# usamec/GAML

Measured on AMD Instinct MI355X. Metric: reads_per_sec_scored, higher is better.
Workload: dtype f64; 1 GPU; cfg3: 5 Mbp, 50x 2x150 paired, insert 300+-30; 833333 pairs in all, whole true genome as 1-2 walks, 8 rotating path sets, window cache warm; pairs_total=833333, pairs_per_gpu=833333, genome_bp=5000000, parallelism=reads sharded over 1 GPU(s)

## Files before the change

gaml_amd/api.py:

```python
from __future__ import annotations

import ctypes as C
import importlib.util
import os
import sys

import numpy as np

_HERE = os.path.dirname(os.path.abspath(__file__))
FLAVOUR = os.environ.get("GAML_HIP_FLAVOUR", "release")
LIB_PATH = os.environ.get("GAML_HIP_LIB") or os.path.join(_HERE, "libgaml_hip_dev.so" if FLAVOUR == "dev" else "libgaml_hip.so")

OK, EINVAL, ENODEVICE, EHIP, ESTATE = 0, -1, -2, -3, -4

_i32p = np.ctypeslib.ndpointer(np.int32, flags="C_CONTIGUOUS")
_i64p = np.ctypeslib.ndpointer(np.int64, flags="C_CONTIGUOUS")
_f64p = np.ctypeslib.ndpointer(np.float64, flags="C_CONTIGUOUS")
_u8p = np.ctypeslib.ndpointer(np.uint8, flags="C_CONTIGUOUS")

ALIGMENT = np.dtype([("position", np.int32), ("edit_dist", np.int32), ("read_id", np.int32), ("orientation", np.int32)])
PACBIO_ALIGMENT = np.dtype([("position", np.int32), ("position_end", np.int32), ("read_id", np.int32), ("pad_", np.int32),
                            ("logprob", np.float64)])


# ... 90 lines not shown
    L.gaml_hip_set_presharded.argtypes = [vp, C.c_int32]
    L.gaml_hip_put_window_records.argtypes = [vp, C.c_int, C.c_int, _i32p, C.c_int32, vp, C.c_int64]
    L.gaml_hip_put_pacbio_records.argtypes = [vp, C.c_int, _i32p, C.c_int32, vp, C.c_int64]
    L.gaml_hip_add_pacbio_reads.argtypes = [vp, C.POINTER(SingleCfg), C.c_int32, _u8p, _i64p, C.c_char_p]
    L.gaml_hip_pacbio_missing.argtypes = [vp, C.c_int, _i32p, C.c_int32, _i32p, C.c_int32]
    L.gaml_hip_pacbio_missing.restype = C.c_int32
    L.gaml_hip_pacbio_ingest_sam.argtypes = [vp, C.c_int, _i32p, C.c_int32, C.c_char_p, C.c_int64, C.POINTER(C.c_int64)]
    L.gaml_hip_pacbio_records.argtypes = [vp, C.c_int, _i32p, C.c_int32, vp, C.c_int64]
    L.gaml_hip_pacbio_records.restype = C.c_int64
    L.gaml_hip_pacbio_dp_stats.argtypes = [vp, C.c_int, _f64p]
    if hasattr(L, "gaml_hip_debug_sam_logprob"):
        L.gaml_hip_debug_sam_logprob.argtypes = [vp, C.c_char_p, C.c_int32, C.c_char_p, C.c_int32, C.c_char_p, C.c_int64, C.c_double, C.POINTER(C.c_double), vp, vp, C.c_int32]
    if hasattr(L, "gaml_hip_debug_sam_shape"):
        L.gaml_hip_debug_sam_shape.argtypes = [C.c_char_p, C.c_int64, C.c_int32, _i32p, C.c_void_p, C.c_int32]
    if hasattr(L, "gaml_hip_debug_sam_band"):
        L.gaml_hip_debug_sam_band.argtypes = [C.c_char_p, C.c_int64, C.c_int32, _i32p, _i32p, _i32p, _i32p, C.c_int32]
        L.gaml_hip_debug_sam_band.restype = C.c_int32
    L.gaml_hip_calc_prob.argtypes = [vp, _i32p, _i64p, C.c_int32, C.POINTER(C.c_double), _i32p, C.POINTER(C.c_int32)]
    L.gaml_hip_calc_prob_batch.argtypes = [vp, C.c_int32, _i32p, _i64p, _i32p, _f64p, vp, vp]
    L.gaml_hip_calc_partials.argtypes = [vp, _i32p, _i64p, C.c_int32, _f64p, C.POINTER(C.c_int32)]
    L.gaml_hip_combine_partials.argtypes = [vp, _f64p, C.c_int32, C.POINTER(C.c_double), _i32p]
    L.gaml_hip_calc_partials_async.argtypes = [vp, _i32p, _i64p, C.c_int32, vp, vp, C.POINTER(C.c_int32)]
    L.gaml_hip_eval_begin.argtypes = [vp, _i32p, _i64p, C.c_int32, C.POINTER(C.c_int64), C.POINTER(C.c_int32)]
    L.gaml_hip_eval_pending_maxpos.argtypes = [vp, vp, C.c_int64]
    L.gaml_hip_eval_pending_maxpos.restype = C.c_int64
    L.gaml_hip_eval_apply_maxpos.argtypes = [vp, _i32p, C.c_int64]
    L.gaml_hip_eval_finish.argtypes = [vp, _f64p]
    L.gaml_hip_eval_finish_async.argtypes = [vp, vp, vp]
    L.gaml_hip_sync.argtypes = [vp]
    L.gaml_hip_compact_tables.argtypes = [vp]
    L.gaml_hip_eval_score_async.argtypes = [vp, vp, vp]
    L.gaml_hip_eval_score_async.restype = C.c_int32
    L.gaml_hip_eval_coverage_export_async.argtypes = [vp, C.c_int32, vp, C.c_int64, C.POINTER(C.c_int64), vp]
    L.gaml_hip_eval_coverage_finish_async.argtypes = [vp, C.c_int32, vp, C.c_int32, C.c_int32, vp]
    L.gaml_hip_eval_pacbio_pending.argtypes = [vp]
    L.gaml_hip_eval_pacbio_pending.restype = C.c_int32
    L.gaml_hip_eval_pacbio_intervals.argtypes = [vp, C.c_int32]
    L.gaml_hip_eval_pacbio_intervals.restype = C.c_int64
    L.gaml_hip_eval_pacbio_export_async.argtypes = [vp, C.c_int32, vp, C.c_int64, vp]
    L.gaml_hip_eval_pacbio_finish_async.argtypes = [vp, C.c_int32, vp, C.c_int64, C.c_int32, vp]
    L.gaml_hip_num_readsets.argtypes = [vp]
    L.gaml_hip_readset_kind.argtypes = [vp, C.c_int]
    L.gaml_hip_readset_reads.argtypes = [vp, C.c_int]
    L.gaml_hip_readset_reads.restype = C.c_int64
    L.gaml_hip_num_nodes.argtypes = [vp]
    L.gaml_hip_node_len.argtypes = [vp, C.c_int32]
    L.gaml_hip_read_probs.argtypes = [vp, C.c_int, _f64p, C.c_int64]
    L.gaml_hip_bad_bases.argtypes = [vp, C.c_int, C.POINTER(C.c_int64)]
    L.gaml_hip_window_count.argtypes = [vp, C.c_int, C.c_int]
    L.gaml_hip_window_count.restype = C.c_int64
    L.gaml_hip_window_records.argtypes = [vp, C.c_int, C.c_int, _i32p, C.c_int32, vp, C.c_int64]
    L.gaml_hip_window_records.restype = C.c_int64
    L.gaml_hip_align_window.argtypes = [vp, C.c_int, C.c_int, _i32p, C.c_int32]
    L.gaml_hip_align_window.restype = C.c_int64
    if hasattr(L, "gaml_hip_debug_prepare"):
        L.gaml_hip_debug_prepare.argtypes = [vp, _i32p, _i64p, C.c_int32]
    if hasattr(L, "gaml_hip_debug_occurrences"):
        L.gaml_hip_debug_occurrences.argtypes = [vp, C.c_int, C.c_int, _i32p, C.c_int64]
    if hasattr(L, "gaml_hip_debug_occurrences"):
        L.gaml_hip_debug_occurrences.restype = C.c_int64
    if hasattr(L, "gaml_hip_debug_table_occurrences"):
        L.gaml_hip_debug_table_occurrences.argtypes = [vp, C.c_int, C.c_int, _i32p, C.c_int64, _i64p]
    if hasattr(L, "gaml_hip_debug_table_occurrences"):
        L.gaml_hip_debug_table_occurrences.restype = C.c_int64
    if hasattr(L, "gaml_hip_debug_window_walk"):
        L.gaml_hip_debug_window_walk.argtypes = [vp, C.c_int, C.c_int, C.c_int32, _i32p, C.c_int32]
    for new, old in (("gaml_hip_pair_classes", "gaml_hip_debug_class_counts"), ("gaml_hip_last_phases", "gaml_hip_debug_profile"),
                     ("gaml_hip_table_stats", "gaml_hip_debug_table_stats")):
        if not hasattr(L, new) and hasattr(L, old):
            setattr(L, new, getattr(L, old))
    L.gaml_hip_pair_classes.argtypes = [vp, C.c_int, _i64p]
    if hasattr(L, "gaml_hip_debug_fold_check"):
        L.gaml_hip_debug_fold_check.argtypes = [vp, C.c_int, _i64p]
    if hasattr(L, "gaml_hip_debug_radix_sort"):
        L.gaml_hip_debug_radix_sort.argtypes = [vp, C.c_void_p, C.c_void_p, C.c_int64, C.c_int, C.c_int, C.c_void_p]
    if hasattr(L, "gaml_hip_debug_tables_check"):
        L.gaml_hip_debug_tables_check.argtypes = [vp, C.c_int, _i64p]
    if hasattr(L, "gaml_hip_debug_static_check"):
        L.gaml_hip_debug_static_check.argtypes = [vp, C.c_int, _i64p]
    if hasattr(L, "gaml_hip_debug_set_knob"):
        L.gaml_hip_debug_set_knob.argtypes = [vp, C.c_int, C.c_int]
    if hasattr(L, "gaml_hip_debug_occ_route"):
        L.gaml_hip_debug_occ_route.argtypes = [vp, C.c_int, _i64p]
    if hasattr(L, "gaml_hip_debug_occ_check"):
        L.gaml_hip_debug_occ_check.argtypes = [vp, C.c_int, _i64p]
    if hasattr(L, "gaml_hip_shm_exchange_open"):
        L.gaml_hip_shm_exchange_open.argtypes = [vp, C.c_char_p, C.c_int32, C.c_int32, C.c_int32]
        L.gaml_hip_shm_allreduce_sum.argtypes = [vp, C.c_void_p, C.c_int32]
        L.gaml_hip_shm_exchange_close.argtypes = [vp, C.c_int32]
    if hasattr(L, "gaml_hip_fetch_async"):
        L.gaml_hip_fetch_async.argtypes = [vp, C.c_void_p, C.c_int32, C.c_void_p]
        L.gaml_hip_fetch_wait.argtypes = [vp, C.c_void_p, C.c_int32]
    if hasattr(L, "gaml_hip_advice_build"):
        L.gaml_hip_advice_build.argtypes = [vp, C.c_int, C.c_int32]
        L.gaml_hip_advice_index.argtypes = [vp, C.c_int, C.c_void_p, C.c_void_p, C.c_int64]
        L.gaml_hip_advice_index.restype = C.c_int64
        L.gaml_hip_advice_candidates.argtypes = [vp, C.c_int, _i32p, C.c_int32, _i32p, C.c_int32, C.c_int32, C.c_void_p, C.c_int64]
        L.gaml_hip_advice_candidates.restype = C.c_int64
    if hasattr(L, "gaml_hip_debug_timeline"):
        L.gaml_hip_debug_timeline.argtypes = [vp, C.c_int, C.c_void_p, C.c_int64]
    L.gaml_hip_last_phases.argtypes = [vp, _f64p]
    L.gaml_hip_table_stats.argtypes = [vp, C.c_int, _i64p]
    L.gaml_hip_aligner_stats.argtypes = [vp, C.POINTER(C.c_int64), C.POINTER(C.c_int64), C.POINTER(C.c_double)]
    L.gaml_hip_aligner_stages.argtypes = [vp, _f64p]
    L.gaml_hip_last_timing.argtypes = [vp, _f64p]
    L.gaml_hip_set_event_timing.argtypes = [vp, C.c_int]
    L.gaml_hip_kernel_stats.argtypes = [vp, C.c_int, C.POINTER(C.c_int64), C.POINTER(C.c_double), C.POINTER(C.c_double)]
    return L


_lib = _load()

def lib():
    return _lib


def version() -> str:
    return _lib.gaml_hip_version().decode()


class FlatPaths:

    def __init__(self, paths):
        self.flat, self.offs = _flat(paths)
        self.n = len(paths)
        self.flat_ptr, self.offs_ptr = self.flat.ctypes.data, self.offs.ctypes.data

    def __len__(self):
        return self.n


def _flat(paths):
    if isinstance(paths, FlatPaths):
        return paths.flat, paths.offs
    flat = np.array([x for p in paths for x in p], dtype=np.int32)
    if flat.size == 0:
        flat = np.zeros(1, np.int32)
    offs = np.zeros(len(paths) + 1, dtype=np.int64)
    offs[1:] = np.cumsum([len(p) for p in paths])
    return flat, offs


def comm_unique_id() -> bytes:
    buf = C.create_string_buffer(128)
    rc = _lib.gaml_hip_comm_unique_id(C.cast(buf, C.c_void_p))
    if rc != OK:
        raise GamlHipError(rc, "gaml_hip_comm_unique_id failed (RCCL not loadable?)")
    return buf.raw


class Context:

    def __init__(self, device: int = 0, rank: int = 0, world: int = 1, presharded: int = 1, devices=None):
        self._h = C.c_void_p()
        if devices is not None:
            devs = np.ascontiguousarray(devices, np.int32)
            rc = _lib.gaml_hip_create_multi(C.byref(self._h), devs, len(devs))
            if rc != OK:
                raise GamlHipError(rc, f"gaml_hip_create_multi(devices={list(devs)}) failed")
            device = int(devs[0])
        else:
            rc = _lib.gaml_hip_create(C.byref(self._h), device)
            if rc != OK:
                raise GamlHipError(rc, f"gaml_hip_create(device={device}) failed")
        self.device = device
        if world != 1:
# ... 365 lines not shown
        if n > len(out):
            out = self._adv_buf = np.zeros(n, np.int32)
            n = self._check(_lib.gaml_hip_advice_candidates(self._h, rs, path, len(path), reach, len(reach), flags, out.ctypes.data, len(out)))
        return out[:n].copy()

    def debug_prepare(self, paths):
        flat, offs = _flat(paths)
        self._check(_lib.gaml_hip_debug_prepare(self._h, flat, offs, len(paths)))

    def debug_occurrences(self, rs, mate=0) -> np.ndarray:
        n = _lib.gaml_hip_debug_occurrences(self._h, rs, mate, np.zeros(5, np.int32), 0)
        out = np.zeros(5 * max(1, n), np.int32)
        _lib.gaml_hip_debug_occurrences(self._h, rs, mate, out, n)
        return out.reshape(-1, 5)[:n]

    def debug_table_occurrences(self, rs, mate=0):
        info = np.zeros(3, np.int64)
        n = _lib.gaml_hip_debug_table_occurrences(self._h, rs, mate, np.zeros(5, np.int32), 0, info)
        out = np.zeros(5 * max(1, n), np.int32)
        _lib.gaml_hip_debug_table_occurrences(self._h, rs, mate, out, n, info)
        return out.reshape(-1, 5)[:n], {"incremental": bool(info[0]), "incremental_calls": int(info[1]), "full_calls": int(info[2])}

    def debug_window_walk(self, rs, mate, wid) -> list:
        buf = np.zeros(64, np.int32)
        n = _lib.gaml_hip_debug_window_walk(self._h, rs, mate, wid, buf, 64)
        if n > 64:
            buf = np.zeros(n, np.int32)
            _lib.gaml_hip_debug_window_walk(self._h, rs, mate, wid, buf, n)
        return [int(x) for x in buf[:n]]

    def table_stats(self, rs):
        out = np.zeros(10, np.int64)
        self._check(_lib.gaml_hip_table_stats(self._h, rs, out))
        return {"full_rebuilds": int(out[0]), "delta_updates": int(out[1]), "dirty_pairs": int(out[2]), "worker_rebuilds": int(out[3]), "side_stream_rebuilds": int(out[3]),
                "batches_patched": int(out[4]), "batches_full": int(out[5]), "records_left_out": [int(out[6]), int(out[7])], "delta_records_left_out": int(out[8]),
                "static_index_pairs": int(out[9])}

    def aligner_stats(self):
        w, k, us = C.c_int64(), C.c_int64(), C.c_double()
        _lib.gaml_hip_aligner_stats(self._h, C.byref(w), C.byref(k), C.byref(us))
        return {"windows": w.value, "candidates": k.value, "us": us.value}

    def aligner_stages(self):
        out = np.zeros(6, np.float64)
        self._check(_lib.gaml_hip_aligner_stages(self._h, out))
        return {"strings_upload": out[0], "spans_candidates": out[1], "extension": out[2], "hits_d2h": out[3], "sort_file": out[4], "batches": int(out[5])}

    def last_phases(self):
        out = np.zeros(8, np.float64)
        _lib.gaml_hip_last_phases(self._h, out)
        return out

    def debug_timeline(self, rs: int, cap_waves: int = 1 << 16) -> np.ndarray:
        out = np.zeros((cap_waves, 8), np.uint64)
        n = self._check(_lib.gaml_hip_debug_timeline(self._h, rs, out.ctypes.data, cap_waves))
        return out[:n]

    def debug_set_knob(self, knob, value):
        self._check(_lib.gaml_hip_debug_set_knob(self._h, knob, value))

    def debug_fold_check(self, rs):
        out = np.zeros(6, np.int64)
        self._check(_lib.gaml_hip_debug_fold_check(self._h, rs, out))
        return {"records_left_out": [int(out[0]), int(out[1])], "compact_pairs": [int(out[2]), int(out[3])], "records_checked": int(out[4]),
                "violations": int(out[5])}

    def debug_radix_sort(self, keys, vals=None, begin_bit=0, end_bit=64, running_max=False):
        k = np.ascontiguousarray(keys, np.uint64).copy()
        v = None if vals is None else np.ascontiguousarray(vals, np.uint64).copy()
        m = np.zeros(len(k), np.uint64) if running_max else None
        self._check(_lib.gaml_hip_debug_radix_sort(self._h, k.ctypes.data, None if v is None else v.ctypes.data, len(k), begin_bit, end_bit,
                                                   None if m is None else m.ctypes.data))
        return k, v, m

    def debug_static_check(self, rs):
        out = np.zeros(8, np.int64)
        self._check(_lib.gaml_hip_debug_static_check(self._h, rs, out))
        return {"static_pairs": int(out[0]), "other_pairs": int(out[1]), "violations": int(out[2]), "no_record": int(out[3]),
                "different_windows": int(out[4]), "orientation": int(out[5]), "distance": int(out[6]), "edits_or_code": int(out[7])}

    def debug_occ_route(self, rs):
        out = np.zeros(6, np.int64)
        self._check(_lib.gaml_hip_debug_occ_route(self._h, rs, out))
        return {"device": int(out[0]), "host": int(out[1]), "fallbacks": int(out[2]), "compactions": int(out[3]),
                "pool_entries": int(out[4]), "shared_combinations": int(out[5])}

    def debug_occ_check(self, rs):
        out = np.zeros(4, np.int64)
        rc = _lib.gaml_hip_debug_occ_check(self._h, rs, out)
        res = {"compared": int(out[0]), "present": int(out[1]), "mismatches": int(out[2]), "lists": int(out[3])}
        if rc != 0 and res["compared"] == 0:
            self._check(rc)
        return res

    def debug_tables_check(self, rs):
        out = np.zeros(8, np.int64)
        rc = _lib.gaml_hip_debug_tables_check(self._h, rs, out)
        res = {"pairs": int(out[0]), "compact": int(out[1]), "static": int(out[2]), "two": int(out[3]), "four": int(out[4]), "more": int(out[5]),
               "compared": int(out[6]), "mismatches": int(out[7])}
        if rc != 0 and res["compared"] == 0:
            self._check(rc)
        return res

    def debug_block_partials(self, rs, set_index=0):
        sums, zeros, lay = np.zeros(8192, np.float64), np.zeros(8192, np.int32), np.zeros(8, np.int32)
        _lib.gaml_hip_debug_block_partials.argtypes = [C.c_void_p, C.c_int, C.c_int32, _f64p, _i32p, C.c_int32, _i32p]
        n = _lib.gaml_hip_debug_block_partials(self._h, rs, set_index, sums, zeros, 8192, lay)
        return sums[:max(n, 0)].copy(), zeros[:max(n, 0)].copy(), lay.tolist()

    def pair_classes(self, rs):
        out = np.zeros(4, np.int64)
        self._check(_lib.gaml_hip_pair_classes(self._h, rs, out))
        return out

    debug_table_stats, debug_profile, debug_class_counts = table_stats, last_phases, pair_classes

    def last_timing(self):
        out = np.zeros(3, np.float64)
        _lib.gaml_hip_last_timing(self._h, out)
        return {"host_us": out[0], "device_wall_us": out[1], "kernel_us": out[2]}

    def set_event_timing(self, on):
        _lib.gaml_hip_set_event_timing(self._h, int(on))

    def kernel_stats(self, reset=False):
        n, us, b = C.c_int64(), C.c_double(), C.c_double()
        _lib.gaml_hip_kernel_stats(self._h, 1 if reset else 0, C.byref(n), C.byref(us), C.byref(b))
        return {"launches": n.value, "device_us": us.value, "algo_bytes": b.value}


def debug_sam_band(sam_line: str, total_len: int):
    raw = sam_line.encode()
    f = np.zeros(10, np.int32); r0 = np.zeros(1, np.int32)
    n = _lib.gaml_hip_debug_sam_band(raw, len(raw), total_len, f, r0, np.zeros(1, np.int32), np.zeros(1, np.int32), 0)
    if n < 0:
        raise GamlHipError(n, "malformed SAM line")
    lo = np.zeros(n, np.int32); hi = np.zeros(n, np.int32)
    _lib.gaml_hip_debug_sam_band(raw, len(raw), total_len, f, r0, lo, hi, n)
    keys = ["flags", "len", "posstart", "posend", "sstart", "send", "slen", "tstart", "tend", "edit_dist"]
    return dict(zip(keys, (int(x) for x in f))), int(r0[0]), lo, hi


def debug_sam_shape(sam_line: str, total_len: int):
    raw = sam_line.encode()
    f = np.zeros(6, np.int32)
    n = _lib.gaml_hip_debug_sam_shape(raw, len(raw), total_len, f, None, 0)
    if n < 0:
        raise GamlHipError(n, "malformed SAM line")
    ops = np.zeros(max(1, n), np.uint32)
    _lib.gaml_hip_debug_sam_shape(raw, len(raw), total_len, f, ops.ctypes.data, n)
    keys = ["n_ops", "row_f", "col_f", "bl", "el", "max_width"]
    return dict(zip(keys, (int(x) for x in f))), [(int(o) >> 2, "MID"[int(o) & 3]) for o in ops[:n]]
```

gaml_amd/csrc/ctx.hip.h:

```cpp
#pragma once
#include <hip/hip_runtime.h>
#include <hip/hip_ext.h>
#include "radix_sort.hip.h"

#include <algorithm>
#include <atomic>
#include <fcntl.h>
#include <sys/mman.h>
#include <unistd.h>
#include <chrono>
#include <climits>
#include <limits>
#include <cmath>
#include <cstdio>
#include <cstdlib>
#include <cstring>
#include <immintrin.h>
#include <memory>
#include <set>
#include <string>
#include <thread>
#include <vector>

#include "aligner.hip.h"
// ... 200 lines not shown
  int64_t class_count[4] = {0, 0, 0, 0};
  int64_t n0a = 0;
  std::vector<uint32_t> len_combo;
  int64_t dropped_records[2] = {0, 0};
};

struct AdviceDev {
  bool built = false;
  int32_t threshold = 0;
  int64_t n_ent = 0, queries = 0;
  std::vector<int64_t> h_offs;
  std::vector<int32_t> h_ent;
  DevBuf offs, ent;
  DevBuf scratch;
  DevBuf first, last, cnt, at, tiles;
  DevBuf in, mask, out;
  PinBuf h_in, h_out;
  uint32_t serial = 0;
  std::vector<AdviceStep> steps;
  std::vector<int32_t> list;
  void release() {
    offs.release(); ent.release(); scratch.release(); first.release(); last.release(); cnt.release(); at.release(); tiles.release();
    in.release(); mask.release(); out.release(); h_in.release(); h_out.release();
  }
};

struct PairedSet {
  gaml_paired_cfg cfg;
  ShortMate mate[2];
  PairInfo pt;
  MateDev dev[2];
  TableDev tab;
  TableRebuild rebuild;
  BuildScratch scratch;
  BuildPlan build_plan;
  int64_t async_rebuilds = 0, retired_windows = 0, eval_count = 0;
  DevBuf lcode, len_combo_dev, combo_tabs, memo;
  int memo_codes = 0;
  bool statics_uploaded = false, kernels_warm = false, prereserved = false;
  DevBuf dl_slot, dl_spill, dl_rec[2], sp_rng[2], sp_rec[2], sp_slot, dstate;
  DevBuf dl_bins, dl_bin_count, dl_blk_tot, dl_wlist, dl_stamps;
  PinBuf h_dstate;
  size_t delta_cap = 0, cap_spill = 0, cap_sprec = 0;
  int64_t nd_est = 0, ns_est = 0;
  bool spill_may_grow = false;
  int dl_seq = 0;
  int64_t full_rebuilds = 0, delta_updates = 0;
  int quiet_calls = 0;
  int64_t delta_left_out = 0, delta_left_out_base = 0;
  bool compact_requested = false;
  PinBuf h_timeline; int timeline_waves = 0;
  PinBuf h_part_sum, h_part_zero;
  size_t host_part_stride = 0;
  int last_total_blocks = 0, last_sets = 1;
  int last_blocks[8] = {0, 0, 0, 0, 0, 0, 0, 0};
  bool last_host_partials = false;
  DevBuf probs, tabs, cov_bits, bad;
  Arena arena;
  struct Persist {
    void* dev = nullptr; size_t bytes = 0;
    size_t cap_w[2] = {0, 0}, cap_lo[2] = {0, 0}, cap_m[2] = {0, 0};
    size_t off_tfloor = 0, off_occ[2] = {0, 0}, off_lo[2] = {0, 0}, off_m[2] = {0, 0};
    bool valid = false;
    void release() { if (dev) (void)hipFree(dev); dev = nullptr; bytes = 0; valid = false; }
  } persist;
  struct OccDev {
    DevBuf pool[2];
    size_t pool_cap[2] = {0, 0}, pool_used[2] = {0, 0};
    uint32_t pool_gen = 1;
    PinBuf stage;
    DevBuf tab[2][2], list[2][2];
    DevBuf stamp[2];
    size_t cap_w = 0, cap_list = 0;
    int32_t list_n[2][2] = {{0, 0}, {0, 0}};
    uint32_t serial = 0;
    PinBuf dup;
    bool taken = false;
    bool check_dup = false;
    bool image_stale = false;
    std::vector<std::vector<uint64_t>> shared;
    size_t shared_next = 0;
    std::vector<uint64_t> key;
    int64_t dev_calls = 0, host_calls = 0, fallbacks = 0, compactions = 0;
    void release() {
      for (int mt = 0; mt < 2; mt++) {
        pool[mt].release(); stamp[mt].release();
        for (int k = 0; k < 2; k++) { tab[mt][k].release(); list[mt][k].release(); }
      }
      stage.release(); dup.release();
    }
  } occdev;
  int64_t batches_patched = 0, batches_full = 0;
  size_t batch_slack = 0;
  hipEvent_t ev_tables = nullptr, ev_ovf = nullptr;
  PairedPlanner planner;
  OccImage image[2];
  std::vector<Occ> scratch_occ[2];
  Reducer red;
  Staging stage_pool;
  std::vector<double> ins_tab, floor_tab, logfloor_tab, covthr_tab;
  bool floor_positive = true;
  bool tabs_uploaded = false;
  int64_t last_bad_bases = 0;
  AdviceDev adv;
};

struct SingleSet {
  gaml_single_cfg cfg;
  ShortMate mate;
  ReadMajor rm;
  MateDev dev;
  DevBuf lens, probs, tabs, occ_arena;
  std::vector<Occ> last_occ;
  Reducer red;
  std::vector<double> floor_tab, logfloor_tab;
  bool tabs_uploaded = false;
  Staging stage;
};

struct DpDev {
  DevBuf path, jobs, ops, scratch, out, dbg;
  void release() { path.release(); jobs.release(); ops.release(); scratch.release(); out.release(); dbg.release(); }
};

struct PbSweepDev {
  DevBuf iv_off, iv;
  std::vector<int32_t> iv_off_host;
  uint64_t generation = ~0ull;
  DevBuf in, all;
  DevBuf key_begin, key_end, pos, key_begin_s, key_end_s, pos_s, end_max, tmp, bad;
  Staging stage;
  void release() {
    iv_off.release(); iv.release(); in.release(); all.release(); key_begin.release(); key_end.release(); pos.release();
    key_begin_s.release(); key_end_s.release(); pos_s.release(); end_max.release(); tmp.release(); bad.release();
    for (int k = 0; k < kRing; k++) { stage.host[k].release(); if (stage.done[k]) (void)hipEventDestroy(stage.done[k]); stage.done[k] = nullptr; stage.armed[k] = false; }
  }
};

struct PacbioSet {
  gaml_single_cfg cfg;
  int64_t n_global = 0, lo = 0, hi = 0;
  std::vector<int32_t> lens;
  double log_match = 0, log_mismatch = 0;
  std::unordered_map<Walk, int32_t, WalkHasher> walk_id;
  std::vector<std::vector<gaml_pacbio_aligment>> recs;
  uint64_t generation = 0, uploaded_generation = ~0ull;
  int32_t max_len = 0;
  int64_t misses = 0;
  DevBuf d_lens, rec_off, rec_walk, rec_logp, walk_count, logprobs;
  Reducer red;
  int64_t last_bad_bases = 0;
  Staging stage;
  PbSweepDev sweep;
  bool have_reads = false;
  std::string bases;
  std::vector<int64_t> base_off;
  std::unordered_map<std::string, int32_t> name_id;
  DevBuf d_bases;
  DpDev dp;
  bool bases_uploaded = false;
  double dp_stats[8] = {0, 0, 0, 0, 0, 0, 0, 0};
};

struct PairedPrep {
  int64_t assembled_records = 0;
  std::vector<int32_t> path_base, start_off, starts;
  int32_t total_bits = 0, n_paths = 0;
  bool general = false;
};
// ... 76 lines not shown
```

gaml_amd/csrc/debug_api.hip.h:

```cpp
#pragma once

int gaml_hip_debug_prepare(gaml_hip_ctx* c, const int32_t* flat, const int64_t* offs, int32_t n_paths) {
  if (!c || n_paths < 0 || (n_paths > 0 && (!flat || !offs))) return fail(c, GAML_HIP_EINVAL, "bad arguments");
  if (c->multi) {
    for (int k = 0; k < gaml::multi_num_shards(c->multi); k++)
      if (int e = gaml_hip_debug_prepare(gaml::multi_shard(c->multi, k), flat, offs, n_paths)) return fail(c, e, gaml_hip_last_error(gaml::multi_shard(c->multi, k)));
    return GAML_HIP_OK;
  }
  if (!c->have_graph) return fail(c, GAML_HIP_ESTATE, "no graph set");
  std::vector<Walk> paths = unflatten(flat, offs, n_paths);
  for (auto& h : scoring_order(c)) {
    if (h.kind == 0) { std::vector<Occ> occs; prepare_single_host(c, *c->singles[h.idx], paths, occs); }
    else if (h.kind == 1) {
      PairedPrep p;
      PairedSet& ps = *c->paireds[h.idx];
      if (int e = prepare_paired_structure(c, ps, flat, offs, n_paths)) return e;
      if (int e = align_pending_pair(c, ps)) return e;
      if (int e = prepare_paired_tables_host(c, ps, p)) return e;
    }
  }
  if (c->peers == 1) {
    for (ShortMate* m : filter_mates(c)) m->unsynced.clear();
  }
  return GAML_HIP_OK;
// ... 205 lines not shown
  }
  return n;
}



int gaml_hip_debug_tables_check(gaml_hip_ctx* c, int rs, int64_t* out8) {
  MULTI_SHARD0(c);
  if (!c || rs < 0 || rs >= (int)c->handles.size() || c->handles[rs].kind != 1 || !out8) return fail(c, GAML_HIP_EINVAL, "bad arguments");
  if (c->device < 0) return fail(c, GAML_HIP_ENODEVICE, "host-only context");
  PairedSet& s = *c->paireds[c->handles[rs].idx];
  HIP_TRY(c, hipSetDevice(c->device));
  if (s.rebuild.active) { if (int e = paired_build_continue(c, s, true)) return e; HIP_TRY(c, hipEventSynchronize(s.rebuild.done)); s.rebuild.active = false; s.rebuild.after.clear(); }
  if (int e = prepare_paired_tables(c, s)) return e;
  if (int e = pool_mirror(c, s, c->stream)) return e;
  if (int e = paired_upload_statics(c, s, c->stream)) return e;
  TableDev T;
  if (int e = paired_build_enqueue(c, s, T, c->stream)) return e;
  HIP_TRY(c, hipStreamSynchronize(c->stream));
  if (int e = paired_build_collect(c, s, T)) { T.release(); return e; }
  ShortMate hm[2];
  for (int mt = 0; mt < 2; mt++) {
    const ShortMate& m = s.mate[mt];
    hm[mt].n_global = m.n_global; hm[mt].lo = m.lo; hm[mt].hi = m.hi; hm[mt].lens = m.lens;
    hm[mt].wins = m.wins;
    std::vector<int4> dp((size_t)s.dev[mt].pool_n);
    if (!dp.empty()) HIP_TRY(c, hipMemcpy(dp.data(), s.dev[mt].pool.p, dp.size() * sizeof(int4), hipMemcpyDeviceToHost));
    hm[mt].pool.resize(dp.size());
    for (size_t k = 0; k < dp.size(); k++) hm[mt].pool[k] = gaml_aligment{dp[k].y, dp[k].z & 0xff, dp[k].w, (dp[k].z >> 8) & 1};
    for (Window& w : hm[mt].wins) w.first = w.dfirst < 0 ? 0 : w.dfirst;
    for (Window& w : hm[mt].wins) if (w.dfirst < 0) { w.count = 0; }
  }
  PairTables pt;
  build_pair_tables(hm[0], hm[1], pt, KNOB(c, 16) != 1, paired_static_ins_n(c, s));
  const int64_t n = s.mate[0].n_local();
  int64_t compared = 0, bad = 0;
  auto fetch = [&](const DevBuf& d, size_t bytes, std::vector<char>& out) -> int {
    out.resize(bytes);
    if (bytes) HIP_TRY(c, hipMemcpy(out.data(), d.p, bytes, hipMemcpyDeviceToHost));
    return 0;
  };
  auto cmp = [&](const DevBuf& d, const void* host, size_t bytes, size_t elem, const char* what) -> int {
    std::vector<char> v;
    if (int e = fetch(d, bytes, v)) return e;
    int64_t b0 = bad;
    for (size_t k = 0; k < bytes / elem; k++) { compared++; if (memcmp(v.data() + k * elem, (const char*)host + k * elem, elem) != 0) bad++; }
    if (bad != b0 && getenv("GAML_HIP_TRACE_HOST")) fprintf(stderr, "tables_check: %s differs in %lld of %zu entries\n", what, (long long)(bad - b0), bytes / elem);
    return 0;
  };
  for (int k = 0; k < 4; k++) { compared++; bad += T.class_count[k] != pt.class_count[k]; }
  compared++; bad += T.n0a != pt.n0a;
  if (bad == 0) {
    const int64_t n0 = pt.class_count[0], n16 = n - n0;
    if (int e = cmp(T.slot_of_read, pt.slot_of_read.data(), (size_t)n * 4, 4, "slot_of_read")) return e;
    if (int e = cmp(T.read_of_slot, pt.read_of_slot.data(), (size_t)n * 4, 4, "read_of_slot")) return e;
    for (int mt = 0; mt < 2; mt++) {
      if (int e = cmp(T.rec8[mt], pt.rec8[mt].data(), (size_t)n0 * 8, 8, "rec8")) return e;
      if (int e = cmp(T.first[mt], pt.rm[mt].first.data(), (size_t)n16 * 16, 16, "first")) return e;
      if (int e = cmp(T.extra[mt], pt.rm[mt].extra.data(), pt.rm[mt].extra.size() * 16, 16, "extra")) return e;
      if (int e = cmp(T.inl[mt], pt.inl[mt].data(), pt.inl[mt].size() * 16, 16, "inl")) return e;
      compared++; bad += T.extras[mt] != (int64_t)pt.rm[mt].extra.size();
      compared++; bad += T.dropped[mt] != pt.dropped_records[mt];
    }
    if (int e = cmp(T.len_code, pt.len_code.data(), (size_t)n0, 1, "len_code")) return e;
    if (int e = cmp(T.static_idx, pt.static_idx.data(), (size_t)pt.n0a * 4, 4, "static_idx")) return e;
    if (int e = cmp(T.len12, pt.len12.data(), (size_t)n16 * 4, 4, "len12")) return e;
    compared++; bad += pt.len_combo != s.pt.len_combo;
  }
  out8[0] = n; out8[1] = T.class_count[0]; out8[2] = T.n0a; out8[3] = T.class_count[1]; out8[4] = T.class_count[2]; out8[5] = T.class_count[3];
  out8[6] = compared; out8[7] = bad;
  T.release();
  return bad ? fail(c, GAML_HIP_ESTATE, "record tables: the device build differs from the host restatement") : GAML_HIP_OK;
}

int gaml_hip_debug_occ_route(gaml_hip_ctx* c, int rs, int64_t* out6) {
  MULTI_SHARD0(c);
  if (!c || !out6 || rs < 0 || rs >= (int)c->handles.size() || c->handles[rs].kind != 1) return fail(c, GAML_HIP_EINVAL, "bad arguments");
  const PairedSet::OccDev& D = c->paireds[c->handles[rs].idx]->occdev;
  out6[0] = D.dev_calls; out6[1] = D.host_calls; out6[2] = D.fallbacks; out6[3] = D.compactions;
  out6[4] = (int64_t)(D.pool_used[0] + D.pool_used[1]); out6[5] = (int64_t)D.shared.size();
  return GAML_HIP_OK;
}

int gaml_hip_debug_occ_check(gaml_hip_ctx* c, int rs, int64_t* out4) {
  MULTI_SHARD0(c);
  if (!c || !out4 || rs < 0 || rs >= (int)c->handles.size() || c->handles[rs].kind != 1) return fail(c, GAML_HIP_EINVAL, "bad arguments");
  PairedSet& ps = *c->paireds[c->handles[rs].idx];
  const PairedSet::OccDev& D = ps.occdev;
  out4[0] = out4[1] = out4[2] = out4[3] = 0;
  if (!D.image_stale) return GAML_HIP_OK;
  HIP_TRY(c, hipSetDevice(c->device));
  HIP_TRY(c, hipStreamSynchronize(c->stream));
  const PlanView& v = ps.planner.view();
  for (int mt = 0; mt < 2; mt++) {
    OccImage im;
    im.build(ps.mate[mt].wins.size(), v, mt);
    const size_t n = im.occ12.size();
    std::vector<Occ12> dev(n);
    if (n) HIP_TRY(c, hipMemcpy(dev.data(), occdev_table(ps, mt), n * sizeof(Occ12), hipMemcpyDeviceToHost));
    for (size_t w = 0; w < n; w++) {
      const Occ12& h = im.occ12[w];
      const Occ12& d = dev[w];
      const bool absent = h.lo == ~0u && h.hi == ~0u;
      out4[0]++;
      if (!absent) out4[1]++;
      if (absent ? (d.lo != ~0u || d.hi != ~0u) : (d.lo != h.lo || d.hi != h.hi || d.rank != h.rank)) out4[2]++;
    }
    if (!im.general_wids.empty()) out4[3]++;
  }
  if (out4[2] || out4[3]) return fail(c, GAML_HIP_ESTATE, "device occurrence tables differ from the host image");
  return GAML_HIP_OK;
}
```

gaml_amd/csrc/host_model.cc:

```cpp
#include "host_model.h"

#include <algorithm>
#include <chrono>
#include <cmath>
#include <cstdlib>
#include <cstring>
#include <fstream>
#include <thread>

namespace gaml {

void GraphStore::finish() {
  norm.resize(n());
  std::unordered_map<std::string, int32_t> tiny;
  for (int32_t i = 0; i < n(); i++) {
    norm[i] = i;
    if (len(i) > 3) continue;
    std::string s(seq(i), len(i));
    auto it = tiny.find(s);
    if (it == tiny.end()) tiny.emplace(s, i);
    else norm[i] = it->second;
  }
}

// ... 865 lines not shown
    }
    is_new_.assign((size_t)n_paths, 0);
    for (const Edit& e : edits_) for (int32_t k = e.c0; k < e.c1; k++) is_new_[k] = 1;
    for (const Edit& e : edits_) {
      int32_t chain_end = e.c1;
      while (chain_end < n_paths) { const bool has_node = memos_[cur_ids_[chain_end]]->final_last_end != -2; chain_end++; if (has_node) break; }
      registration_chain(g, mate, e.c0, chain_end);
    }
    std::vector<char>& redo = redo_;
    redo.assign(memos_.size(), 0);
    for (int32_t id : in_ids) redo[id] = 1;
    for (int32_t id : stale_) if (id < (int32_t)memos_.size() && memos_[id]->use_count > 0 && (!memos_[id]->valid[0] || !memos_[id]->valid[1] || !memos_[id]->occ_valid[0] || !memos_[id]->occ_valid[1])) redo[id] = 2;
    stale_.clear();
    drain(mate);
    size_t seen = stale_.size();
    for (int32_t k = 0; k < n_paths; k++) {
      const int32_t id = cur_ids_[k];
      if (!redo[id]) continue;
      PathMemo& pm = *memos_[id];
      bool built = false;
      for (int mt = 0; mt < 2; mt++)
        if (!pm.valid[mt]) { build_placements(g, mate[mt], mt, pm, id); built = true; }
      if (!built) continue;
      drain(mate);
      for (; seen < stale_.size(); seen++) {
        const int32_t sid = stale_[seen];
        if (sid >= (int32_t)redo.size() || redo[sid]) continue;
        for (int32_t q = k + 1; q < n_paths; q++) if (cur_ids_[q] == sid) { redo[sid] = 2; break; }
      }
    }
    for (int32_t k = 0; k < n_paths; k++) {
      const int32_t id = cur_ids_[k];
      if (!redo[id]) continue;
      if (!is_new_[k]) {
        const PathMemo& pm = *memos_[id];
        removed_.push_back(Removed{cur_slots_[k], {pm.assembled[0], pm.assembled[1]}, {pm.occ[0], pm.occ[1]}});
      }
      work_.push_back(k);
    }
    std::vector<int32_t> keep;
    for (int32_t sid : stale_) if (sid < (int32_t)memos_.size() && memos_[sid]->use_count > 0 && (!memos_[sid]->valid[0] || !memos_[sid]->valid[1])) keep.push_back(sid);
    stale_.swap(keep);
  }
  const int64_t total = n_paths > 0 ? offs[n_paths] - base : 0;
  prev_flat_.assign(flat + base, flat + base + total);
  prev_offs_.resize((size_t)n_paths + 1);
  for (int32_t k = 0; k <= n_paths; k++) prev_offs_[k] = (n_paths > 0 ? offs[k] : 0) - base;
  have_prev_ = true;
  return true;
}

static void occ_prepack(const std::vector<Occ>& occ, std::vector<OccPre>& pre) {
  pre.resize(occ.size());
  for (size_t k = 0; k < occ.size(); k++) {
    const Occ& o = occ[k];
    const int32_t mp = o.min_pos < -32768 ? -32768 : o.min_pos;
    pre[k] = OccPre{o.min_pos <= 32767 ? o.wid : ~o.wid, (uint32_t)o.shift, (uint32_t)(uint16_t)(int16_t)mp, o.rank};
  }
}

static bool occ_pre_plain(const std::vector<OccPre>& pre) {
  std::vector<int32_t> w(pre.size());
  for (size_t k = 0; k < pre.size(); k++) { if (pre[k].wid < 0) return false; w[k] = pre[k].wid; }
  std::sort(w.begin(), w.end());
  return std::adjacent_find(w.begin(), w.end()) == w.end();
}

void PairedPlanner::invalidate_thresholds() {
  for (auto& pm : memos_) pm->occ_valid[0] = pm->occ_valid[1] = false;
  have_prev_ = false;
}

void PairedPlanner::finish(ShortMate mate[2]) {
  auto redo_occ = [&](PathMemo& pm) {
    for (int mt = 0; mt < 2; mt++) {
      if (pm.occ_valid[mt]) continue;
      pm.occ[mt].clear();
      occurrences_from_placements(mate[mt], pm.pl[mt], pm.occ[mt]);
      pm.assembled[mt] = 0;
      for (const Occ& o : pm.occ[mt]) pm.assembled[mt] += mate[mt].wins[o.wid].count;
      occ_prepack(pm.occ[mt], pm.pre[mt]);
      pm.pre_plain[mt] = occ_pre_plain(pm.pre[mt]);
      pm.dev_off[mt] = -1;
      pm.occ_valid[mt] = true;
    }
  };
  if (!incremental_) {
    for (int32_t id : cur_ids_) redo_occ(*memos_[id]);
    assembled_[0] = assembled_[1] = 0;
    for (int32_t id : cur_ids_) { assembled_[0] += memos_[id]->assembled[0]; assembled_[1] += memos_[id]->assembled[1]; }
  } else {
    for (int32_t k : work_) redo_occ(*memos_[cur_ids_[k]]);
  }
}

const PlanView& PairedPlanner::view() {
  if (!view_valid_) {
    view_.paths.clear();
    for (int32_t id : cur_ids_) view_.paths.push_back(memos_[id].get());
    view_valid_ = true;
  }
  return view_;
}

void PairedPlanner::apply(ShortMate mate[2], OccImage image[2], bool build_image, bool image_stale) {
  if (!incremental_) {
    const PlanView& v = view();
    for (int32_t id : cur_ids_) {
      PathMemo& pm = *memos_[id];
      if (pm.touched_serial == retire_serial_) continue;
      for (int mt = 0; mt < 2; mt++) for (const Occ& o : pm.occ[mt]) mate[mt].touch(o.wid);
      pm.touched_serial = retire_serial_;
    }
    if (build_image) for (int mt = 0; mt < 2; mt++) image[mt].build(mate[mt].wins.size(), v, mt);
    return;
  }
  if (image_stale) {
    for (int mt = 0; mt < 2; mt++) {
      for (const Removed& r : removed_) assembled_[mt] -= r.assembled[mt];
      for (int32_t k : work_) assembled_[mt] += memos_[cur_ids_[k]]->assembled[mt];
    }
    for (int32_t id : cur_ids_) {
      PathMemo& pm = *memos_[id];
      if (pm.touched_serial == retire_serial_) continue;
      for (int mt = 0; mt < 2; mt++) for (const Occ& o : pm.occ[mt]) mate[mt].touch(o.wid);
      pm.touched_serial = retire_serial_;
    }
    rebuild_images(mate, image);
    return;
  }
  for (int32_t k : work_) {
    PathMemo& pm = *memos_[cur_ids_[k]];
    if (pm.touched_serial == retire_serial_) continue;
    for (int mt = 0; mt < 2; mt++) for (const Occ& o : pm.occ[mt]) mate[mt].touch(o.wid);
    pm.touched_serial = retire_serial_;
  }
  if ((int32_t)pos_of_slot_.size() < next_slot_) pos_of_slot_.resize((size_t)next_slot_ + 64, 0);
  for (int32_t k = 0; k < (int32_t)cur_slots_.size(); k++) pos_of_slot_[cur_slots_[k]] = k;
  for (int mt = 0; mt < 2; mt++) {
    OccImage& im = image[mt];
    for (const Removed& r : removed_) { im.remove_path(r.occ[mt], r.slot); assembled_[mt] -= r.assembled[mt]; }
    for (int32_t k : work_) {
      const PathMemo& pm = *memos_[cur_ids_[k]];
      im.add_path(mate[mt].wins.size(), pm.occ[mt], cur_slots_[k]);
      assembled_[mt] += pm.assembled[mt];
    }
    im.finalize(pos_of_slot_);
  }
}

void PairedPlanner::rebuild_images(ShortMate mate[2], OccImage image[2]) {
  if ((int32_t)pos_of_slot_.size() < next_slot_) pos_of_slot_.resize((size_t)next_slot_ + 64, 0);
  for (int32_t k = 0; k < (int32_t)cur_slots_.size(); k++) pos_of_slot_[cur_slots_[k]] = k;
  const PlanView& v = view();
  for (int mt = 0; mt < 2; mt++) image[mt].build(mate[mt].wins.size(), v, mt, &cur_slots_, &pos_of_slot_);
}

void PairedPlanner::mark_used(ShortMate mate[2], const OccImage image[2]) {
  for (int mt = 0; mt < 2; mt++) image[mt].for_each_present([&](int32_t w) { mate[mt].touch(w); });
  for (auto& pm : memos_)
    if (pm->last_used > rebuild_clock_ || pm->use_count > 0)
      for (int mt = 0; mt < 2; mt++) for (const Occ& o : pm->occ[mt]) if (o.wid < (int32_t)mate[mt].wins.size()) mate[mt].touch(o.wid);
}

void PairedPlanner::flat_occurrences(int mate, std::vector<Occ>& out) {
  out.clear();
// ... 646 lines not shown
```

gaml_amd/csrc/host_model.h:

```cpp
#pragma once
#include <climits>
#include <cstdint>
#include <memory>
#include <string>
#include <unordered_map>
#include <vector>

#include "../../include/gaml_hip.h"

namespace gaml {

constexpr int kTail = 300;
constexpr int kSeed = 15;

struct GraphStore {
  std::string bases;
  std::vector<int64_t> off;
  std::vector<int32_t> norm;
  int32_t n() const { return (int32_t)off.size() - 1; }
  int32_t len(int32_t node) const { return (int32_t)(off[node + 1] - off[node]); }
  const char* seq(int32_t node) const { return bases.data() + off[node]; }
  void finish();
  bool load_lastgraph(const std::string& file, std::string* err);
};
// ... 127 lines not shown
#ifndef GAML_FOLD_CLASS2_BELOW
#define GAML_FOLD_CLASS2_BELOW 1024
#endif
constexpr int64_t kFoldClass2Below = GAML_FOLD_CLASS2_BELOW;
constexpr int kMemoCodes = 4;
constexpr int32_t kStaticZero = -2;
constexpr size_t kMemoMaxEntries = (size_t)1 << 24;
#ifdef GAML_HIP_DEV
struct PairTables {
  std::vector<int32_t> slot_of_read, read_of_slot;
  int64_t class_count[4] = {0, 0, 0, 0};
  int64_t n0a = 0;
  std::vector<int32_t> static_idx;
  std::vector<uint64_t> rec8[2];
  std::vector<uint8_t> len_code;
  std::vector<uint32_t> len_combo;
  std::vector<uint32_t> len12;
  ReadMajor rm[2];
  std::vector<RecQuad> inl[2];
  int64_t dropped_records[2] = {0, 0};
};
void build_pair_tables(const ShortMate& a, const ShortMate& b, PairTables& out, bool fold = true, int ins_n = 0);
#endif
void link_mate_windows(ShortMate& a, ShortMate& b);
#ifdef GAML_HIP_DEV
int64_t undominated_records(const ShortMate& m, int32_t wid, std::vector<uint8_t>& keep);
#endif


struct OccQuad { int32_t shift, min_pos, path, rank; };
struct OccTable {
  std::vector<OccQuad> direct;
  std::vector<int32_t> multi_off;
  std::vector<OccQuad> multi;
};
void build_occ_table(size_t n_windows, const std::vector<Occ>& occs, OccTable& out);

void split_contigs(const Walk& path, std::vector<std::pair<int32_t, int32_t>>& ctg_ranges, std::vector<int32_t>& gaps);

struct PlanView;
struct Occ12 { uint32_t lo, hi; int32_t rank; };
struct OccImage {
  std::vector<Occ12> occ12;
  std::vector<int32_t> multi_off;
  std::vector<OccQuad> multi;
  std::vector<int32_t> general_wids;
  void build(size_t n_windows, const PlanView& view, int mate, const std::vector<int32_t>* slots = nullptr,
             const std::vector<int32_t>* pos_of_slot = nullptr);
  void add_path(size_t n_windows, const std::vector<Occ>& occ, int32_t slot);
  void remove_path(const std::vector<Occ>& occ, int32_t slot);
  void finalize(const std::vector<int32_t>& pos_of_slot);
  std::vector<int32_t> changed;
  bool changed_all = true, lists_changed = true;
  void dump(std::vector<Occ>& out) const;
  template <class F> void for_each_present(F f) const { for (int32_t w : touched_) if (cnt_[w] > 0) f(w); }
  void take_changed() { changed.clear(); changed_all = false; lists_changed = false; if (++mark_serial_ == 0) { std::fill(mark_.begin(), mark_.end(), 0); mark_serial_ = 1; } }
 private:
  void grow(size_t n_windows);
  void mark(int32_t w) { if (mark_[w] != mark_serial_) { mark_[w] = mark_serial_; changed.push_back(w); } }
  void set_direct(int32_t w, const OccQuad& q);
  std::vector<int32_t> touched_, stale_, cnt_, list_of_;
  std::vector<uint32_t> stamp_, mark_;
  uint32_t serial_ = 0, mark_serial_ = 1;
  struct Pending { int32_t wid; OccQuad q; };
  std::vector<Pending> pending_;
  std::unordered_map<int32_t, std::vector<OccQuad>> gen_;
  bool lists_dirty_ = false;
};

struct OccPre { int32_t wid; uint32_t lo, hi; int32_t rank; };

struct PathMemo {
  Walk path;
  bool registered[2] = {false, false};
  bool first_pending[2] = {false, false};
  bool valid[2] = {false, false};
  bool occ_valid[2] = {false, false};
  std::vector<Placement> pl[2];
  std::vector<Occ> occ[2];
  std::vector<OccPre> pre[2];
  bool pre_plain[2] = {false, false};
  int64_t dev_off[2] = {-1, -1};
  uint32_t dev_gen[2] = {0, 0};
  int64_t assembled[2] = {0, 0};
  std::vector<int32_t> starts;
  int32_t length = 0;
  int32_t first_idx = -1, first_end = -1;
  int32_t final_last_end = -2;
  int32_t use_count = 0;
  uint32_t touched_serial = 0;
  uint64_t last_used = 0;
  uint32_t serial = 0;
};

struct PlanView {
  std::vector<const PathMemo*> paths;
};

class PairedPlanner {
 public:
  bool begin(const GraphStore& g, ShortMate mate[2], const int32_t* flat, const int64_t* offs, int32_t n_paths,
             bool allow_incremental, std::string* err);
  void finish(ShortMate mate[2]);
  void apply(ShortMate mate[2], OccImage image[2], bool build_image = true, bool image_stale = false);
  void rebuild_images(ShortMate mate[2], OccImage image[2]);
  const std::vector<int32_t>& ids() const { return cur_ids_; }
  PathMemo& memo(int32_t id) { return *memos_[id]; }
  void mark_used(ShortMate mate[2], const OccImage image[2]);
  void note_rebuild(bool retired_some) { rebuild_clock_ = clock_; if (retired_some) retire_serial_++; }
  void invalidate_thresholds();
  void forget_previous() { have_prev_ = false; }
  const PlanView& view();
  void flat_occurrences(int mate, std::vector<Occ>& out);
  size_t memo_count() const { return memos_.size(); }
  int32_t total_len() const { return total_len_; }
  int64_t assembled(int mate) const { return assembled_[mate]; }
  int32_t n_paths() const { return (int32_t)cur_ids_.size(); }
  bool last_was_incremental() const { return incremental_; }
  const std::vector<int32_t>& slots() const { return cur_slots_; }
  uint64_t hits = 0, misses = 0, incremental_calls = 0, full_calls = 0;
 private:
  int32_t lookup_or_create(const GraphStore& g, const int32_t* p, int32_t len, std::string* err);
  void drain(ShortMate mate[2]);
  void build_placements(const GraphStore& g, ShortMate& m, int mt, PathMemo& pm, int32_t id);
  void registration_chain(const GraphStore& g, ShortMate mate[2], int32_t from, int32_t to);
  std::vector<std::unique_ptr<PathMemo>> memos_;
  std::unordered_map<Walk, int32_t, WalkHasher> by_path_;
  std::unordered_map<Walk, std::vector<std::pair<int32_t, uint32_t>>, WalkHasher> missed_[2];
  PlanView view_;
  bool view_valid_ = false;
  std::vector<int32_t> cur_ids_;
  std::vector<int32_t> cur_slots_;
  std::vector<int32_t> free_slots_, pos_of_slot_;
  int32_t next_slot_ = 0;
  std::vector<int32_t> prev_flat_;
  std::vector<int64_t> prev_offs_;
  bool have_prev_ = false;
  bool incremental_ = false;
  struct Removed { int32_t slot; int64_t assembled[2]; std::vector<Occ> occ[2]; };
  std::vector<Removed> removed_;
  std::vector<int32_t> work_;
  std::vector<int32_t> stale_;
  std::vector<char> redo_;
  struct Edit { int32_t p0, p1, c0, c1; };
  std::vector<Edit> edits_;
  std::vector<char> is_new_;
  int32_t total_len_ = 0;
  int64_t assembled_[2] = {0, 0};
  uint64_t clock_ = 0, rebuild_clock_ = 0;
  uint32_t retire_serial_ = 0;
  static constexpr size_t kMaxMemos = 2048;
};
int32_t walk_length(const GraphStore& g, const Walk& w);

bool read_fastq(const std::string& file, std::string& bases, std::vector<int64_t>& offs, std::string* err,
                std::vector<std::string>* names = nullptr);

struct SamRecord {
  std::string name;
  int32_t flags = 0, len = 0, posstart = 0, posend = 0, sstart = 0, send = 0, slen = 0, tstart = 0, tend = 0, edit_dist = 0;
  std::vector<std::pair<int32_t, char>> cigar;
};
bool parse_sam_record(const char* begin, const char* end, int32_t total_len, SamRecord& out);

struct DpBand {
  int32_t row0 = 0, max_width = 0;
// ... 11 lines not shown
```

gaml_amd/csrc/kernels.hip.h:

```cpp
#pragma once
#include <hip/hip_runtime.h>
#include <stdint.h>

namespace gaml {

constexpr int kBlock = 256;
constexpr int kMaxBlocks = 2048;
enum { kDsDirty = 0, kDsSpill = 1, kDsTop0 = 2, kDsTop1 = 3, kDsOverflow = 4, kDsSeq = 5, kDsInts = 8 };

__device__ __forceinline__ unsigned long long occ8_of(const Occ12* t, unsigned w) { const Occ12* e = t + w; return (unsigned long long)e->lo | ((unsigned long long)e->hi << 32); }

struct MateView {
  const int4* first;
  const int4* extra;
  const int4* occ;
  const Occ12* occ12;
  const int* multi_off;
  const int4* multi;
  const double* mism_pow;
  const double* match_pow;
};

struct PairedArgs {
  int total_blocks, blocks0a, n0a, n_codes;
  int blocks0;
  int blocks01, blocks012;
  int main_blocks;
  const double2* memo;
  uint32_t* cov_bits;
  const unsigned long long* rec8[2];
  const double2* static_val;
  const Occ12* occ12[2];
  double* probs;
  double* part_sum;
  int* part_zero;
  double log_two_T;
  double tfloor0, logfloor0;
  uint32_t len_combo0; int pad0_;
  MateView m[2];
  const uint32_t* len12;
  const double* ins_tab;
  int ins_n;
  const double* floor_tab;
  const double* logfloor_tab;
  const double* covthr_tab;
  double two_T;
  int n;
  const int* path_base;
  const unsigned char* len_code;
  const uint32_t* len_combo;
  const double* pe[2];
  const double* floor_c;
  const double* logfloor_c;
  const double* covthr_c;
  int lt_codes;
  const double* tfloor_c;
  const int4* inl[2];
  int n0;
  const int* static_idx;
  int n01;
  int n_main;
  unsigned long long* timeline;
  const int* dstate;
  const int* dirty_slots;
  const int4* dirty_recs[2];
  const int* dirty_spill;
  const int2* spill_rng[2];
  const int4* spill_recs[2];
  const int* spill_slot;
  unsigned* ticket;
  double* out;
  double n_reads;
  double* status_out;
  double status_a, status_b;
};

struct Cand { int path, pos, edit, orient, rank, k; bool valid; };

__device__ __forceinline__ int4 occ_from_compact(unsigned long long o, int rk) {
  const int4 e = make_int4((int)(unsigned)o, (int)(short)(o >> 32), (int)((o >> 48) & 0x7fff), rk);
  return o == ~0ull ? make_int4(0, 0, -1, 0) : e;
}
__device__ __forceinline__ int4 mate_occ(const MateView& v, int w) {
  if (v.occ) return v.occ[w];
  const Occ12 e = v.occ12[w];
  return occ_from_compact((unsigned long long)e.lo | ((unsigned long long)e.hi << 32), e.rank);
}

__device__ __forceinline__ Cand make_cand(const int4& r, const int4& o, int k) {
  Cand c;
  c.path = o.z; c.pos = r.y + o.x; c.edit = r.z & 0xff; c.orient = (r.z >> 8) & 1;
  c.rank = o.w; c.k = k; c.valid = r.y >= o.y;
  return c;
}

struct TableSrc {
  const MateView* v;
  int4 r0;
  __device__ __forceinline__ int count() const { return r0.x < 0 ? 0 : 1 + (int)((unsigned)r0.z >> 9); }
  __device__ __forceinline__ int4 get(int k) const { return k == 0 ? r0 : v->extra[r0.w + k - 1]; }
};
struct ListSrc {
  const int4* recs;
  int cnt;
  __device__ __forceinline__ int count() const { return cnt; }
  __device__ __forceinline__ int4 get(int k) const { return recs[k]; }
};

template <class Src, class F>
__device__ __forceinline__ void for_each_cand_src(const MateView& v, const Src& src, F f) {
  const int cnt = src.count();
  for (int k = 0; k < cnt; k++) {
    int4 r = src.get(k);
    if (r.x < 0) continue;
    int4 o = mate_occ(v, r.x);
    if (o.z < 0) continue;
    if (o.w >= 0) {
      f(make_cand(r, o, k));
    } else {
      const int s = -o.w - 1;
      for (int q = v.multi_off[s]; q < v.multi_off[s + 1]; q++) f(make_cand(r, v.multi[q], k));
    }
  }
}
template <class F>
__device__ __forceinline__ void for_each_cand(const MateView& v, const int4& r0, F f) {
  for_each_cand_src(v, TableSrc{&v, r0}, f);
}

template <class Src>
__device__ __forceinline__ bool is_live_src(const MateView& v, const Src& src, const Cand& c) {
  if (!c.valid) return false;
  bool live = true;
  for_each_cand_src(v, src, [&](const Cand& d) {
    if (d.valid && d.path == c.path && d.pos == c.pos && (d.rank > c.rank || (d.rank == c.rank && d.k > c.k))) live = false;
  });
  return live;
}
__device__ __forceinline__ bool is_live(const MateView& v, const int4& r0, const Cand& c) {
  return is_live_src(v, TableSrc{&v, r0}, c);
}

__device__ __forceinline__ void mark_bit(uint32_t* bits, int bit) {
  atomicOr(&bits[bit >> 5], 1u << (bit & 31));
}

__device__ __forceinline__ double pair_term(const PairedArgs& a, const Cand& x, const Cand& y, int L1, int L2) {
  if (x.orient == y.orient) return 0.0;
  int dist;
  if (x.pos < y.pos) {
    if (x.orient != 0 || y.orient != 1) return 0.0;
    dist = y.pos - x.pos + L2;
  } else {
    if (x.orient != 1 || y.orient != 0) return 0.0;
    dist = x.pos - y.pos + L1;
  }
  if ((unsigned)dist >= (unsigned)a.ins_n) return 0.0;
  double p1 = a.m[0].mism_pow[x.edit] * a.m[0].match_pow[L1 - x.edit];
  double p2 = a.m[1].mism_pow[y.edit] * a.m[1].match_pow[L2 - y.edit];
  double ip = a.ins_tab[dist];
  double t = p1 * p2 * ip;
  if (a.cov_bits && t > a.covthr_tab[L2]) {
    int base = a.path_base[x.path];
    mark_bit(a.cov_bits, base + max(x.pos, y.pos));
    mark_bit(a.cov_bits, base + min(x.pos, y.pos));
  }
  return t;
}

template <class Src>
__device__ __forceinline__ double paired_general_src_slow(const PairedArgs& a, const Src& s1, const Src& s2, int L1, int L2) {
  double acc = 0.0;
  for_each_cand_src(a.m[0], s1, [&](const Cand& x) {
    if (!is_live_src(a.m[0], s1, x)) return;
    for_each_cand_src(a.m[1], s2, [&](const Cand& y) {
      if (y.path != x.path) return;
      if (!is_live_src(a.m[1], s2, y)) return;
      acc += pair_term(a, x, y, L1, L2);
    });
  });
  return acc;
}
template <class Src>
__device__ __forceinline__ bool live_mask_src(const MateView& v, const Src& src, unsigned long long& mask) {
  mask = 0;
  int n = 0;
  for_each_cand_src(v, src, [&](const Cand& c) {
    if (n < 64 && is_live_src(v, src, c)) mask |= 1ull << n;
    n++;
  });
  return n <= 64;
}
template <class Src>
__device__ __forceinline__ double paired_general_src_masks(const PairedArgs& a, const Src& s1, const Src& s2, int L1, int L2) {
  unsigned long long live1, live2;
  if (!live_mask_src(a.m[0], s1, live1) || !live_mask_src(a.m[1], s2, live2)) return paired_general_src_slow(a, s1, s2, L1, L2);
  double acc = 0.0;
  if (!live1 || !live2) return acc;
  int ix = 0;
  for_each_cand_src(a.m[0], s1, [&](const Cand& x) {
    const bool lx = (live1 >> ix) & 1ull;
    ix++;
    if (!lx) return;
    int iy = 0;
    for_each_cand_src(a.m[1], s2, [&](const Cand& y) {
      const bool ly = (live2 >> iy) & 1ull;
      iy++;
      if (!ly || y.path != x.path) return;
      acc += pair_term(a, x, y, L1, L2);
    });
  });
  return acc;
}
template <class Src>
__device__ __forceinline__ double paired_general_src(const PairedArgs& a, const Src& s1, const Src& s2, int L1, int L2) {
  return paired_general_src_slow(a, s1, s2, L1, L2);
}
__device__ __forceinline__ double paired_general(const PairedArgs& a, const int4& r1, const int4& r2, int L1, int L2) {
  return paired_general_src_masks(a, TableSrc{&a.m[0], r1}, TableSrc{&a.m[1], r2}, L1, L2);
}

__device__ __forceinline__ void block_reduce(double& s, int& z, double* sh_s, int* sh_z) {
  for (int off = 32; off > 0; off >>= 1) {
    s += __shfl_down(s, off, 64);
    z += __shfl_down(z, off, 64);
  }
  const int lane = threadIdx.x & 63, wave = threadIdx.x >> 6;
  if (lane == 0) { sh_s[wave] = s; sh_z[wave] = z; }
  __syncthreads();
  if (threadIdx.x == 0) {
    double ts = 0; int tz = 0;
    for (int w = 0; w < kBlock / 64; w++) { ts += sh_s[w]; tz += sh_z[w]; }
    s = ts; z = tz;
  }
}

constexpr int kTicketWords = 17;
__device__ __forceinline__ void grid_finish(double s, int z, int my_slot, int n_partials, double* part_sum, int* part_zero,
                                            unsigned* ticket, double* out, double bad_bases, double n_reads, double* sh_s, int* sh_z,
                                            double* status_out = nullptr, double status_a = 0.0, double status_b = 0.0) {
  __shared__ bool is_last;
  if (threadIdx.x == 0) {
    __hip_atomic_store(&part_sum[my_slot], s, __ATOMIC_RELAXED, __HIP_MEMORY_SCOPE_AGENT);
    __hip_atomic_store(&part_zero[my_slot], z, __ATOMIC_RELAXED, __HIP_MEMORY_SCOPE_AGENT);
    asm volatile("s_waitcnt vmcnt(0)" ::: "memory");
    const int g = my_slot & 15;
    const unsigned in_group = (unsigned)((n_partials - g + 15) >> 4), groups = (unsigned)min(16, n_partials);
    bool last = false;
    if (__hip_atomic_fetch_add(&ticket[1 + g], 1u, __ATOMIC_RELAXED, __HIP_MEMORY_SCOPE_AGENT) == in_group - 1)
      last = __hip_atomic_fetch_add(&ticket[0], 1u, __ATOMIC_RELAXED, __HIP_MEMORY_SCOPE_AGENT) == groups - 1;
    is_last = last;
  }
  __syncthreads();
  if (!is_last) return;
  double ts = 0; int tz = 0;
  for (int b = threadIdx.x; b < n_partials; b += kBlock) {
    ts += __hip_atomic_load(&part_sum[b], __ATOMIC_RELAXED, __HIP_MEMORY_SCOPE_AGENT);
    tz += __hip_atomic_load(&part_zero[b], __ATOMIC_RELAXED, __HIP_MEMORY_SCOPE_AGENT);
  }
  __syncthreads();
  block_reduce(ts, tz, sh_s, sh_z);
  if (threadIdx.x < kTicketWords) __hip_atomic_store(&ticket[threadIdx.x], 0u, __ATOMIC_RELAXED, __HIP_MEMORY_SCOPE_AGENT);
  if (threadIdx.x == 0) {
    out[0] = ts;
    out[1] = (double)tz;
    if (bad_bases >= 0) out[2] = bad_bases;
    out[3] = n_reads;
    if (status_out) { status_out[0] = status_a; status_out[1] = status_b; }
  }
}

struct PairVal { double t, logt; int key, kind; };

__device__ __forceinline__ void finish_read(const PairedArgs& a, int i, double acc, int L1, int L2, double& lsum, int& zeros, PairVal* cap = nullptr) {
  if (cap) *cap = PairVal{acc, 0.0, L1 + L2, 3};
  a.probs[i] = acc;
  const double p = acc / a.two_T;
  const int s = L1 + L2;
  if (p < a.floor_tab[s]) { zeros++; lsum += a.logfloor_tab[s]; }
  else lsum += log(p);
}

template <int K>
struct RegCands {
  int path[K], pos[K], ef[K], rank[K];
  bool valid[K], live[K];
};

template <int K>
__device__ __forceinline__ bool cands_from_records(const MateView& v, const int4 (&r)[K], RegCands<K>& c) {
  int4 o[K];
  bool multi = false;
  Occ12 e[K];
#pragma unroll
  for (int k = 0; k < K; k++) e[k] = v.occ12[r[k].x >= 0 ? r[k].x : 0];
#pragma unroll
  for (int k = 0; k < K; k++) o[k] = occ_from_compact((unsigned long long)e[k].lo | ((unsigned long long)e[k].hi << 32), e[k].rank);
#pragma unroll
  for (int k = 0; k < K; k++) if (r[k].x < 0) o[k] = make_int4(0, 0, -1, 0);
#pragma unroll
  for (int k = 0; k < K; k++) {
    multi |= (o[k].z >= 0 && o[k].w < 0);
    c.path[k] = o[k].z; c.pos[k] = r[k].y + o[k].x; c.ef[k] = r[k].z & 0x1ff; c.rank[k] = o[k].w;
    c.valid[k] = r[k].x >= 0 && o[k].z >= 0 && r[k].y >= o[k].y;
  }
#pragma unroll
  for (int i = 0; i < K; i++) {
    bool lv = c.valid[i];
#pragma unroll
    for (int j = 0; j < K; j++)
      if (j != i) lv = lv && !(c.valid[j] && c.path[j] == c.path[i] && c.pos[j] == c.pos[i] &&
                               (c.rank[j] > c.rank[i] || (c.rank[j] == c.rank[i] && j > i)));
    c.live[i] = lv;
  }
  return multi;
}
template <int K>
__device__ __forceinline__ bool load_cands_inline(const MateView& v, const int4* rec, RegCands<K>& c) {
  int4 r[K];
#pragma unroll
  for (int k = 0; k < K; k++) r[k] = rec[k];
  return cands_from_records<K>(v, r, c);
}

template <int K>
__device__ __forceinline__ double score_regs(const PairedArgs& a, const RegCands<K>& c1, const RegCands<K>& c2, int L1, int L2) {
  int n1 = 0, n2 = 0;
  Cand x, y;
  x.path = -1; x.pos = 0; x.edit = 0; x.orient = 0; y = x;
#pragma unroll
  for (int i = 0; i < K; i++) {
    if (c1.live[i]) { n1++; x.path = c1.path[i]; x.pos = c1.pos[i]; x.edit = c1.ef[i] & 0xff; x.orient = c1.ef[i] >> 8; }
    if (c2.live[i]) { n2++; y.path = c2.path[i]; y.pos = c2.pos[i]; y.edit = c2.ef[i] & 0xff; y.orient = c2.ef[i] >> 8; }
  }
  if (n1 == 0 || n2 == 0) return 0.0;
  if (n1 == 1 && n2 == 1) return x.path == y.path ? pair_term(a, x, y, L1, L2) : 0.0;
  double acc = 0.0;
#pragma unroll
  for (int i = 0; i < K; i++) {
#pragma unroll
    for (int j = 0; j < K; j++) {
      if (c1.live[i] && c2.live[j] && c1.path[i] == c2.path[j]) {
        Cand x, y;
        x.path = c1.path[i]; x.pos = c1.pos[i]; x.edit = c1.ef[i] & 0xff; x.orient = c1.ef[i] >> 8;
        y.path = c2.path[j]; y.pos = c2.pos[j]; y.edit = c2.ef[j] & 0xff; y.orient = c2.ef[j] >> 8;
        acc += pair_term(a, x, y, L1, L2);
      }
    }
  }
  return acc;
}

constexpr unsigned long long kNone8 = ~0ull;
constexpr unsigned long long kDirty8 = ~0ull - 1;
constexpr int kDirtyWid = -2;

__device__ __forceinline__ int4 rec8_to_quad(unsigned long long r) {
  if (r == kNone8 || r == kDirty8) return make_int4(r == kDirty8 ? kDirtyWid : -1, 0, 0, 0);
  return make_int4((int)(r & 0xffffff), (int)((r >> 24) & 0xfffffff), (int)((r >> 52) & 63) | ((int)((r >> 58) & 1) << 8), 0);
}

struct Compact1 {
  unsigned long long r1, r2, o1, o2;
  int L1, L2, lc;
};

__global__ __launch_bounds__(kBlock) void logterm_kernel(const double* pe0, const double* pe1, const double* ins_tab, int ins_n, int codes,
                                                        double2* memo) {
  const int total = codes * 49 * ins_n;
  for (int idx = blockIdx.x * kBlock + threadIdx.x; idx < total; idx += gridDim.x * kBlock) {
    const int dist = idx % ins_n;
    const int q = idx / ins_n;
    const int e2 = q % 7, e1 = (q / 7) % 7, code = q / 49;
    const double t = pe0[code * 64 + e1] * pe1[code * 64 + e2] * ins_tab[dist];
    memo[idx] = make_double2(t, log(t));
  }
}

// ... 82 lines not shown
      for (int q = 0; q < K; q++) {
        const Cand y = make_cand(r2, e2[q], 0);
        if (q >= l2.n || !y.valid || y.path != x.path) continue;
        acc += pair_term(a, x, y, L1, L2);
      }
    }
  } else {
    for (int p = 0; p < l1.n; p++) {
      const Cand x = make_cand(r1, l1.e[p], 0);
      if (!x.valid) continue;
      for (int q = 0; q < l2.n; q++) {
        const Cand y = make_cand(r2, l2.e[q], 0);
        if (!y.valid || y.path != x.path) continue;
        acc += pair_term(a, x, y, L1, L2);
      }
    }
  }
  finish_read_compact(a, i, acc, lc, lsum, zeros);
}

struct GenOut { double add; int zeros; };
__device__ GenOut compact_general_call(unsigned long long kernargs, int i, int set);
__device__ GenOut general_pair_call(unsigned long long kernargs, int i, int dj, int set, int4* lds);
__device__ __forceinline__ unsigned long long kernel_args_address() {
#if defined(__HIP_DEVICE_COMPILE__)
  return (unsigned long long)__builtin_amdgcn_kernarg_segment_ptr();
#else
  return 0;
#endif
}

__device__ __forceinline__ void compact_finish(const PairedArgs& a, int i, const Compact1& c, const CompactPrep& q, double2 m,
                                               double& lsum, int& zeros, PairVal* cap = nullptr) {
  if (q.memo_idx >= 0) {
    const double t = m.x;
    if (cap) *cap = PairVal{t, m.y, c.lc, 1};
    compact_cover(a, c, q, t);
    __builtin_nontemporal_store(t, &a.probs[i]);
    const bool floored = t < a.tfloor_c[c.lc];
    lsum += floored ? a.logfloor_c[c.lc] : m.y - a.log_two_T;
    zeros += (int)floored;
    return;
  }
  double t = 0.0;
  if (q.scores) { t = compact_term_tables(a, c, q); compact_cover(a, c, q, t); }
  finish_read_compact(a, i, t, c.lc, lsum, zeros, cap);
}

__device__ __forceinline__ void finish_val(const PairedArgs& a, int i, const PairVal& v, bool store, double& lsum, int& zeros) {
  if (v.kind == 0) return;
  if (store) __builtin_nontemporal_store(v.t, &a.probs[i]);
  if (v.kind == 1) {
    const bool floored = v.t < a.tfloor_c[v.key];
    lsum += floored ? a.logfloor_c[v.key] : v.logt - a.log_two_T;
    zeros += (int)floored;
  } else if (v.kind == 2) {
    if (v.t == 0.0 && a.floor_c[v.key] > 0.0) { zeros++; lsum += a.logfloor_c[v.key]; return; }
    const double p = v.t / a.two_T;
    if (p < a.floor_c[v.key]) { zeros++; lsum += a.logfloor_c[v.key]; }
    else lsum += log(p);
  } else {
    const double p = v.t / a.two_T;
    if (p < a.floor_tab[v.key]) { zeros++; lsum += a.logfloor_tab[v.key]; }
    else lsum += log(p);
  }
}

__device__ __forceinline__ void compact_load(const PairedArgs& a, int i, bool ok, Compact1& c) {
  c.r1 = ok ? a.rec8[0][i] : kNone8;
  c.r2 = ok ? a.rec8[1][i] : kNone8;
  c.lc = ok ? a.len_code[i] : 0;
}

#if defined(GAML_HIP_DEV) && defined(GAML_GEN_X)
#define GAML_GEN_OFF(bit) ((GAML_GEN_X) & (bit))
#else
#define GAML_GEN_OFF(bit) 0
#endif
struct SlotRange { int lo, hi, lb, blocks; };
__device__ __forceinline__ SlotRange compact_range(const PairedArgs& a, int lb) {
  return lb < a.blocks0a ? SlotRange{0, a.n0a, lb, a.blocks0a} : SlotRange{a.n0a, a.n0, lb - a.blocks0a, a.blocks0 - a.blocks0a};
}

template <bool GEN>
__device__ __forceinline__ void paired_compact_body(const PairedArgs& a, const SlotRange rg, double& lsum, int& zeros) {
  const int stride = rg.blocks * kBlock, hi = rg.hi;
  int i0 = rg.lo + rg.lb * kBlock + threadIdx.x;
  if (i0 >= hi) return;
  Compact1 c0, c1;
  compact_load(a, i0, true, c0);
  compact_load(a, i0 + stride, i0 + stride < hi, c1);
  while (true) {
    const int i1 = i0 + stride;
    const bool two = i1 < hi;
    const int j0 = i0 + 2 * stride;
    const bool more = j0 < hi;
    Compact1 n0v, n1v;
    compact_load(a, j0, more, n0v);
    compact_load(a, j0 + stride, j0 + stride < hi, n1v);
    const uint32_t l0 = a.len_combo[c0.lc], l1 = a.len_combo[c1.lc];
    c0.L1 = l0 & 0xffff; c0.L2 = l0 >> 16; c1.L1 = l1 & 0xffff; c1.L2 = l1 >> 16;
    const bool d0 = c0.r1 == kDirty8, d1 = c1.r1 == kDirty8;
    if (d0) { c0.r1 = kNone8; c0.r2 = kNone8; }
    if (d1) { c1.r1 = kNone8; c1.r2 = kNone8; }
    c0.o1 = c0.r1 != kNone8 ? occ8_of(a.occ12[0], (unsigned)(c0.r1 & 0xffffff)) : kNone8;
    c0.o2 = c0.r2 != kNone8 ? occ8_of(a.occ12[1], (unsigned)(c0.r2 & 0xffffff)) : kNone8;
    c1.o1 = c1.r1 != kNone8 ? occ8_of(a.occ12[0], (unsigned)(c1.r1 & 0xffffff)) : kNone8;
    c1.o2 = c1.r2 != kNone8 ? occ8_of(a.occ12[1], (unsigned)(c1.r2 & 0xffffff)) : kNone8;
    CompactPrep q0, q1;
    compact_prep(a, c0, q0);
    compact_prep(a, c1, q1);
    const double2 m0 = q0.memo_idx >= 0 ? a.memo[q0.memo_idx] : make_double2(0.0, 0.0);
    const double2 m1 = q1.memo_idx >= 0 ? a.memo[q1.memo_idx] : make_double2(0.0, 0.0);
    if (!d0 && !q0.skip) compact_finish(a, i0, c0, q0, m0, lsum, zeros);
    else if (GEN && q0.skip) { const GenOut o = compact_general_call(kernel_args_address(), i0, -1); lsum += o.add; zeros += o.zeros; }
    if (two && !d1 && !q1.skip) compact_finish(a, i1, c1, q1, m1, lsum, zeros);
    else if (GEN && two && q1.skip) { const GenOut o = compact_general_call(kernel_args_address(), i1, -1); lsum += o.add; zeros += o.zeros; }
    if (!more) break;
    c0 = n0v; c1 = n1v;
    i0 = j0;
  }
}

constexpr int kPairZero = -1, kPairOther = -(1 << 20);
__device__ __forceinline__ int compact_state(const PairedArgs& a, uint2 r1, uint2 r2, uint2 o1, uint2 o2, unsigned lc, uint32_t l12,
                                             bool in_range, bool& skip) {
  const bool v1 = r1.y != ~0u, v2 = r2.y != ~0u;
  const bool w1 = v1 & (o1.y != ~0u), w2 = v2 & (o2.y != ~0u);
  const bool here = in_range & !(r1.y == ~0u && r1.x == 0xfffffffeu);
  skip = here & ((w1 & ((int)o1.y < 0)) | (w2 & ((int)o2.y < 0)));
  const int L1 = l12 & 0xffff, L2 = l12 >> 16;
  const int p1 = (int)(__funnelshift_r(r1.x, r1.y, 24) & 0xfffffffu), p2 = (int)(__funnelshift_r(r2.x, r2.y, 24) & 0xfffffffu);
  const int x = p1 + (int)o1.x, y = p2 + (int)o2.x;
  const unsigned or1 = (r1.y >> 26) & 1u, or2 = (r2.y >> 26) & 1u;
  const bool fwd = x < y;
  const int dist = fwd ? y - x + L2 : x - y + L1;
  const bool scores = w1 & w2 & !skip & (((o1.y ^ o2.y) >> 16) == 0)
                      & (p1 >= (int)(short)(o1.y & 0xffffu)) & (p2 >= (int)(short)(o2.y & 0xffffu))
                      & (or1 != or2) & (or1 == (fwd ? 0u : 1u));
  const unsigned e1 = (r1.y >> 20) & 63u, e2 = (r2.y >> 20) & 63u;
  const bool in_memo = scores & ((unsigned)dist < (unsigned)a.ins_n) & (lc < (unsigned)a.lt_codes) & (e1 < 7u) & (e2 < 7u);
  const int idx = (int)((lc * 7u + e1) * 7u + e2) * a.ins_n + dist;
  int state = in_memo ? idx : ((skip | scores) ? kPairOther : kPairZero - (int)lc);
  if (!here) state = kPairOther - 1;
  return state;
}

template <bool GEN, bool TL = false, bool ONE = false>
__device__ __forceinline__ void paired_compact4_body(const PairedArgs& a, const SlotRange rg, double& lsum, int& zeros) {
  const unsigned stride = (unsigned)rg.blocks * kBlock, n0 = (unsigned)rg.hi;
  unsigned long long* tl = TL ? a.timeline + ((size_t)blockIdx.x * (kBlock / 64) + (threadIdx.x >> 6)) * 8 : nullptr;
#define GAML_STAMP(slot, dep) if (TL) { asm volatile("s_waitcnt vmcnt(0)" ::: "memory"); if ((threadIdx.x & 63) == 0) tl[slot] = (unsigned long long)wall_clock64() + ((dep) == 0x12345u ? 1 : 0); }
  const char* const rec0 = (const char*)a.rec8[0];
  const char* const rec1 = (const char*)a.rec8[1];
  const char* const occ0 = (const char*)a.occ12[0];
  const char* const occ1 = (const char*)a.occ12[1];
  const char* const memo = (const char*)a.memo;
  char* const probs = (char*)a.probs;
  const uint32_t l12_one = ONE ? a.len_combo[0] : 0u;
  const double logfloor_one = ONE ? a.logfloor_c[0] : 0.0, tfloor_one = ONE ? a.tfloor_c[0] : 0.0, log2T = a.log_two_T;
  for (unsigned base = (unsigned)rg.lo + (unsigned)rg.lb * kBlock + threadIdx.x; base < n0; base += 4 * stride) {
    uint2 r1[4], r2[4], o1[4], o2[4];
    unsigned lc[4];
#pragma unroll
    for (int k = 0; k < 4; k++) {
      const unsigned ic = base + k * stride < n0 ? base + k * stride : base;
      r1[k] = *(const uint2*)(rec0 + ic * 8u); r2[k] = *(const uint2*)(rec1 + ic * 8u); lc[k] = ONE ? 0u : (unsigned)a.len_code[ic];
    }
    GAML_STAMP(2, r1[0].x ^ r1[1].x ^ r1[2].x ^ r1[3].x ^ r2[0].x ^ r2[3].x)
#pragma unroll
    for (int k = 0; k < 4; k++) {
      const Occ12* e1 = (const Occ12*)(occ0 + (r1[k].y != ~0u ? (r1[k].x & 0xffffffu) : 0u) * 12u);
      const Occ12* e2 = (const Occ12*)(occ1 + (r2[k].y != ~0u ? (r2[k].x & 0xffffffu) : 0u) * 12u);
      o1[k] = make_uint2(e1->lo, e1->hi); o2[k] = make_uint2(e2->lo, e2->hi);
    }
    GAML_STAMP(3, o1[0].x ^ o1[1].x ^ o1[2].x ^ o1[3].x ^ o2[0].x ^ o2[3].x)
    int state[4];
    unsigned skip_bits = 0;
#pragma unroll
    for (int k = 0; k < 4; k++) {
      bool skip;
      state[k] = compact_state(a, r1[k], r2[k], o1[k], o2[k], lc[k], ONE ? l12_one : a.len_combo[lc[k]], base + k * stride < n0, skip);
      skip_bits |= (unsigned)skip << k;
    }
    double2 m[4];
#pragma unroll
    for (int k = 0; k < 4; k++) m[k] = *(const double2*)(memo + (unsigned)max(state[k], 0) * 16u);
    GAML_STAMP(4, (unsigned)(__double2loint(m[0].x) ^ __double2loint(m[1].x) ^ __double2loint(m[2].x) ^ __double2loint(m[3].x)))
    bool other = false;
#pragma unroll
    for (int k = 0; k < 4; k++) {
      double* const out = (double*)(probs + (base + k * stride) * 8u);
      if (state[k] >= 0) {
        __builtin_nontemporal_store(m[k].x, out);
        const bool floored = m[k].x < (ONE ? tfloor_one : a.tfloor_c[lc[k]]);
        lsum += floored ? (ONE ? logfloor_one : a.logfloor_c[lc[k]]) : m[k].y - log2T;
        zeros += (int)floored;
      } else if (state[k] > kPairOther) {
        __builtin_nontemporal_store(0.0, out);
        zeros++;
        lsum += ONE ? logfloor_one : a.logfloor_c[kPairZero - state[k]];
      } else other |= state[k] == kPairOther && !((skip_bits >> k) & 1u);
    }
    GAML_STAMP(5, 0u)
    if (__any(other)) {
#pragma unroll 1
      for (int k = 0; k < 4; k++) {
        if (state[k] != kPairOther || ((skip_bits >> k) & 1u)) continue;
        const int i = (int)(base + k * stride);
        Compact1 d;
        compact_load(a, i, true, d);
        d.o1 = d.r1 != kNone8 ? occ8_of(a.occ12[0], (unsigned)(d.r1 & 0xffffff)) : kNone8;
        d.o2 = d.r2 != kNone8 ? occ8_of(a.occ12[1], (unsigned)(d.r2 & 0xffffff)) : kNone8;
        const uint32_t l = a.len_combo[d.lc];
        d.L1 = l & 0xffff; d.L2 = l >> 16;
        CompactPrep q;
        compact_prep(a, d, q);
        compact_finish(a, i, d, q, make_double2(0.0, 0.0), lsum, zeros);
      }
    }
    if (GEN && !GAML_GEN_OFF(8) && __any(skip_bits != 0)) {
#pragma unroll 1
      for (int k = 0; k < 4; k++)
        if ((skip_bits >> k) & 1u) { const GenOut o = compact_general_call(kernel_args_address(), (int)(base + k * stride), -1); lsum += o.add; zeros += o.zeros; }
    }
  }
#undef GAML_STAMP
}

#ifndef GAML_LEAN_ENTRY
#define GAML_LEAN_ENTRY 1
#endif
#if GAML_LEAN_ENTRY && defined(__HIP_DEVICE_COMPILE__)
#define GAML_FRESH_ARGS(name, fallback)                                                                                   \
  const __attribute__((address_space(4))) PairedArgs* name##_p =                                                          \
      (const __attribute__((address_space(4))) PairedArgs*)__builtin_amdgcn_kernarg_segment_ptr();                        \
  asm volatile("" : "+s"(name##_p));                                                                                      \
  const PairedArgs name = *name##_p;
#else
#define GAML_FRESH_ARGS(name, fallback) const PairedArgs& name = fallback;
#endif
#ifndef GAML_STATIC_P
#define GAML_STATIC_P 4
#endif
#ifndef GAML_STATIC_PIPE
#define GAML_STATIC_PIPE 0
#endif
#if defined(GAML_HIP_DEV) && defined(GAML_STATIC_X)
#define GAML_TIMING_X(bit) ((GAML_STATIC_X) & (bit))
#else
#define GAML_TIMING_X(bit) 0
#endif
__global__ __launch_bounds__(kBlock) void static_values_kernel(const int* static_idx, int n0a, const double2* memo, double2* static_val) {
  for (int i = blockIdx.x * kBlock + threadIdx.x; i < n0a; i += gridDim.x * kBlock) {
    const int mi = static_idx[i];
    static_val[i] = mi >= 0 ? memo[mi] : make_double2(0.0, 0.0);
  }
}

template <bool GEN, bool TL = false, bool ONE = false>
__device__ __forceinline__ void paired_static4_body(const PairedArgs& a, const SlotRange rg, double& lsum, int& zeros) {
  constexpr int P = GAML_STATIC_P;
  const unsigned stride = (unsigned)rg.blocks * kBlock, n0 = (unsigned)rg.hi;
  unsigned long long* tl = TL ? a.timeline + ((size_t)blockIdx.x * (kBlock / 64) + (threadIdx.x >> 6)) * 8 : nullptr;
#define GAML_STAMP(slot, dep) if (TL && first_round) { asm volatile("s_waitcnt vmcnt(0)" ::: "memory"); if ((threadIdx.x & 63) == 0) tl[slot] = (unsigned long long)wall_clock64() + ((dep) == 0x12345u ? 1 : 0); }
  const char* const rec0 = (const char*)a.rec8[0];
  const char* const rec1 = (const char*)a.rec8[1];
  const char* const sval = (const char*)a.static_val;
  const char* const occ0 = (const char*)a.occ12[0];
  const char* const occ1 = (const char*)a.occ12[1];
  char* const probs = (char*)a.probs;
  const double logfloor_one = ONE ? a.logfloor0 : 0.0, tfloor_one = ONE ? a.tfloor0 : 0.0, log2T = a.log_two_T;
  unsigned base = (unsigned)rg.lo + (unsigned)rg.lb * kBlock + threadIdx.x;
  if (base >= n0) return;
  uint2 r1[P], r2[P];
  double2 m[P];
  unsigned lc[P];
#pragma unroll
  for (int k = 0; k < P; k++) {
    const unsigned ic = base + k * stride < n0 ? base + k * stride : base;
    r1[k] = *(const uint2*)(rec0 + ic * 8u); r2[k] = *(const uint2*)(rec1 + ic * 8u); m[k] = GAML_TIMING_X(4) ? make_double2(1e-9 * (double)ic, -20.0) : *(const double2*)(sval + ic * 16u);
    lc[k] = ONE ? 0u : (unsigned)a.len_code[ic];
  }
  bool first_round = true;
  while (true) {
    GAML_STAMP(2, r1[0].x ^ r2[0].x ^ (unsigned)__double2loint(m[0].x))
    uint2 o1[P], o2[P];
#pragma unroll
    for (int k = 0; k < P; k++) {
      const unsigned w1 = (r1[k].x & 0xffffffu) & (0u - (unsigned)(r1[k].y != ~0u)), w2 = (r2[k].x & 0xffffffu) & (0u - (unsigned)(r2[k].y != ~0u));
      const Occ12* e1 = (const Occ12*)(occ0 + w1 * 12u);
      const Occ12* e2 = (const Occ12*)(occ1 + w2 * 12u);
      o1[k] = make_uint2(e1->lo, e1->hi); o2[k] = make_uint2(e2->lo, e2->hi);
      if (GAML_TIMING_X(1)) { o1[k] = make_uint2(r1[k].x >> 8, 0u); o2[k] = make_uint2(r1[k].x >> 8, 0u); }
    }
    const unsigned nbase = base + P * stride;
    const bool more = nbase < n0;
    uint2 nr1[P], nr2[P];
    double2 nm[P];
    unsigned nlc[P];
    if (GAML_STATIC_PIPE && __any(more)) {
#pragma unroll
      for (int k = 0; k < P; k++) {
        const unsigned ic = nbase + k * stride < n0 ? nbase + k * stride : base;
        nr1[k] = *(const uint2*)(rec0 + ic * 8u); nr2[k] = *(const uint2*)(rec1 + ic * 8u); nm[k] = *(const double2*)(sval + ic * 16u);
        nlc[k] = ONE ? 0u : (unsigned)a.len_code[ic];
      }
    }
    GAML_STAMP(3, o1[0].x ^ o2[0].x)
    GAML_STAMP(4, 0u)
    unsigned skip_bits = 0;
#pragma unroll
    for (int k = 0; k < P; k++) {
      const bool none1 = r1[k].y == ~0u, none2 = r2[k].y == ~0u;
      const bool here = (base + k * stride < n0) & !(none1 & (r1[k].x == 0xfffffffeu));
      const bool w1 = !none1 & (o1[k].y != ~0u), w2 = !none2 & (o2[k].y != ~0u);
      const bool gen = here & ((w1 & ((int)o1[k].y < 0)) | (w2 & ((int)o2[k].y < 0)));
      const bool same = (o1[k].x == o2[k].x) & (((o1[k].y ^ o2[k].y) >> 16) == 0);
      const int p1 = (int)(__funnelshift_r(r1[k].x, r1[k].y, 24) & 0xfffffffu), p2 = (int)(__funnelshift_r(r2[k].x, r2[k].y, 24) & 0xfffffffu);
      const bool kept = (p1 >= (int)(short)(o1[k].y & 0xffffu)) & (p2 >= (int)(short)(o2[k].y & 0xffffu));
      const bool both = here & !gen & w1 & w2;
      const bool scores = both & same & kept;
      const bool poison = both & !same;
      const bool counted = here & !gen;
      skip_bits |= (unsigned)gen << k;
      const double t = scores ? m[k].x : 0.0;
      const bool floored = counted & (!scores | (t < (ONE ? tfloor_one : a.tfloor_c[lc[k]])));
      const double lf = ONE ? logfloor_one : a.logfloor_c[lc[k]];
      double add = floored ? lf : m[k].y - log2T;
      add = counted ? add : 0.0;
      add = poison ? __builtin_nan("") : add;
      lsum += add;
      zeros += (int)floored;
      if (counted && !GAML_TIMING_X(2)) __builtin_nontemporal_store(t, (double*)(probs + (base + k * stride) * 8u));
    }
    if (GEN && !GAML_GEN_OFF(1) && __any(skip_bits != 0)) {
#pragma unroll 1
      for (int k = 0; k < P; k++)
        if ((skip_bits >> k) & 1u) { const GenOut o = compact_general_call(kernel_args_address(), (int)(base + k * stride), -1); lsum += o.add; zeros += o.zeros; }
    }
    GAML_STAMP(5, 0u)
    first_round = false;
    if (!more) break;
    base = nbase;
    if (GAML_STATIC_PIPE) {
#pragma unroll
      for (int k = 0; k < P; k++) { r1[k] = nr1[k]; r2[k] = nr2[k]; m[k] = nm[k]; lc[k] = nlc[k]; }
    } else {
#pragma unroll
      for (int k = 0; k < P; k++) {
        const unsigned ic = base + k * stride < n0 ? base + k * stride : base;
        r1[k] = *(const uint2*)(rec0 + ic * 8u); r2[k] = *(const uint2*)(rec1 + ic * 8u); m[k] = GAML_TIMING_X(4) ? make_double2(1e-9 * (double)ic, -20.0) : *(const double2*)(sval + ic * 16u);
        lc[k] = ONE ? 0u : (unsigned)a.len_code[ic];
      }
    }
  }
#undef GAML_STAMP
}

#ifndef GAML_GEN_CANDS
#define GAML_GEN_CANDS 32
#endif
constexpr int kGenCands = GAML_GEN_CANDS;
#ifdef GAML_GEN_STAMPS
__device__ unsigned long long g_gen_stamp[32];
#define GEN_STAMP(k) do { asm volatile("s_waitcnt vmcnt(0) lgkmcnt(0)" ::: "memory"); const unsigned long long now_ = wall_clock64(); \
  if (__ffsll((long long)__ballot(1)) - 1 == (int)(threadIdx.x & 63)) atomicAdd(&g_gen_stamp[k], now_ - gen_t_); atomicMax(&g_gen_stamp[16 + k], now_ - gen_t_); if (now_ - gen_t_ > 1000) atomicAdd(&g_gen_stamp[24 + k], 1ull); gen_t_ = now_; } while (0)
#define GEN_STAMP_BEGIN unsigned long long gen_t_ = wall_clock64(); const unsigned long long gen_t0_ = gen_t_; if (__ffsll((long long)__ballot(1)) - 1 == (int)(threadIdx.x & 63)) atomicAdd(&g_gen_stamp[15], 1ull);
#else
#define GEN_STAMP(k) do { } while (0)
#define GEN_STAMP_BEGIN
#endif
constexpr int kGenListBatch = 8;
template <int K>
__device__ __forceinline__ bool general_pair_staged(const PairedArgs& a, const int4 (&r1)[K], const int4 (&r2)[K], int L1, int L2, double& acc_out, int4* cand) {
  int n[2] = {0, 0};
  unsigned live[2] = {0, 0};
  Occ12 e[2][K];
  int lb[2][K], le[2][K];
  GEN_STAMP_BEGIN
#pragma unroll
  for (int m = 0; m < 2; m++)
#pragma unroll
    for (int k = 0; k < K; k++) { const int4& r = m == 0 ? r1[k] : r2[k]; e[m][k] = a.m[m].occ12[r.x >= 0 ? r.x : 0]; }
  GEN_STAMP(0);
#pragma unroll
  for (int m = 0; m < 2; m++)
#pragma unroll
    for (int k = 0; k < K; k++) {
      const int4& r = m == 0 ? r1[k] : r2[k];
      const bool occurs = r.x >= 0 && !(e[m][k].lo == ~0u && e[m][k].hi == ~0u);
      const bool list = occurs && e[m][k].rank < 0;
      lb[m][k] = le[m][k] = 0;
      if (list) { const int s = -e[m][k].rank - 1; lb[m][k] = a.m[m].multi_off[s]; le[m][k] = a.m[m].multi_off[s + 1]; }
      else if (occurs) le[m][k] = -1;
    }
  GEN_STAMP(1);
  bool fits = true;
#pragma unroll
  for (int m = 0; m < 2; m++) {
    int4* const cm = cand + m * kGenCands;
#pragma unroll
    for (int k = 0; k < K; k++) {
      const int4& r = m == 0 ? r1[k] : r2[k];
      const bool single = le[m][k] == -1;
      const int cnt = single ? 1 : le[m][k] - lb[m][k];
      if (!__any(cnt > 0)) continue;
      if (n[m] + cnt > kGenCands) fits = false;
      const int4 one = occ_from_compact((unsigned long long)e[m][k].lo | ((unsigned long long)e[m][k].hi << 32), e[m][k].rank);
      const int n_before = n[m];
      for (int c0 = 0; __any(fits && c0 < cnt); c0 += kGenListBatch) {
        const int left = fits ? cnt - c0 : 0;
        int4 t[kGenListBatch];
#pragma unroll
        for (int q = 0; q < kGenListBatch; q++) t[q] = (!single && left > 0) ? a.m[m].multi[lb[m][k] + c0 + min(q, left - 1)] : one;
        unsigned nl = 0;
        int pos[kGenListBatch];
#pragma unroll
// ... 11 lines not shown
          if (q < left) cm[n[m] + q] = make_int4(t[q].z, pos[q], (r.z & 0x1ff) | (((valid >> q) & 1u) ? 0x200 : 0) | (k << 10), t[q].w);
        if (left > 0) { live[m] |= nl << n[m]; n[m] += min(left, kGenListBatch); }
      }
    }
  }
  GEN_STAMP(2);
#ifdef GAML_GEN_STAMPS
  if (!fits) atomicAdd(&g_gen_stamp[12], 1ull);
#endif
  if (!fits) return false;
  GEN_STAMP(3);
  double acc = 0.0;
  for (int x = 0; x < n[0]; x++) {
    if (!((live[0] >> x) & 1u)) continue;
    const int4 cx = cand[x];
    Cand X; X.path = cx.x; X.pos = cx.y; X.edit = cx.z & 0xff; X.orient = (cx.z >> 8) & 1;
    for (int y = 0; y < n[1]; y++) {
      if (!((live[1] >> y) & 1u)) continue;
      const int4 cy = cand[kGenCands + y];
      if (cy.x != cx.x) continue;
      Cand Y; Y.path = cy.x; Y.pos = cy.y; Y.edit = cy.z & 0xff; Y.orient = (cy.z >> 8) & 1;
      acc += pair_term(a, X, Y, L1, L2);
    }
  }
  GEN_STAMP(4);
#ifdef GAML_GEN_STAMPS
  if (__ffsll((long long)__ballot(1)) - 1 == (int)(threadIdx.x & 63)) { atomicAdd(&g_gen_stamp[8], (unsigned long long)n[0]); atomicAdd(&g_gen_stamp[9], (unsigned long long)n[1]); atomicAdd(&g_gen_stamp[10], (unsigned long long)__popc(live[0])); atomicAdd(&g_gen_stamp[11], (unsigned long long)__popcll(__ballot(1))); }
  atomicMax(&g_gen_stamp[13], wall_clock64() - gen_t0_); atomicMax(&g_gen_stamp[14], (unsigned long long)(n[0] * 1000 + n[1])); atomicMax(&g_gen_stamp[7], (unsigned long long)(__popc(live[0]) * 1000 + __popc(live[1])));
#endif
  acc_out = acc;
  return true;
}
constexpr int kOvfCap = 128;
constexpr int kGenWaveSlots = 2 * kOvfCap / (2 * kGenCands);
__device__ __forceinline__ int4* gen_wave_slot(int4* wave_lds, bool mine) {
  const unsigned long long m = __ballot(mine);
  const int rank = __popcll(m & ((1ull << (threadIdx.x & 63)) - 1ull));
  return (wave_lds && mine && rank < kGenWaveSlots) ? wave_lds + rank * 2 * kGenCands : nullptr;
}

template <int K>
__device__ __forceinline__ void score_cands_and_finish(const PairedArgs& a, int i, uint32_t l12, const RegCands<K>& x, const RegCands<K>& y,
                                                       double& lsum, int& zeros, PairVal* cap = nullptr) {
  const int L1 = l12 & 0xffff, L2 = l12 >> 16;
    if (a.memo) {
      int n1 = 0, n2 = 0;
      Compact1 c;
      CompactPrep q;
      q.x.path = -1; q.x.pos = 0; q.x.edit = 0; q.x.orient = 0; q.y = q.x;
#pragma unroll
      for (int k = 0; k < K; k++) {
        if (x.live[k]) { n1++; q.x.path = x.path[k]; q.x.pos = x.pos[k]; q.x.edit = x.ef[k] & 0xff; q.x.orient = x.ef[k] >> 8; }
        if (y.live[k]) { n2++; q.y.path = y.path[k]; q.y.pos = y.pos[k]; q.y.edit = y.ef[k] & 0xff; q.y.orient = y.ef[k] >> 8; }
      }
      int code = (a.lt_codes > 0 && l12 == a.len_combo0) ? 0 : -1;
      if (code < 0 && a.n_codes > 1) {
#pragma unroll
        for (int k = 3; k >= 1; k--) if (k < a.lt_codes && a.len_combo[k] == l12) code = k;
      }
      if (n1 == 1 && n2 == 1 && q.x.path == q.y.path && code >= 0 && q.x.orient != q.y.orient && q.x.edit < 7 && q.y.edit < 7) {
        const bool fwd = q.x.pos < q.y.pos;
        const bool ok = fwd ? (q.x.orient == 0) : (q.x.orient == 1);
        const int dist = fwd ? q.y.pos - q.x.pos + L2 : q.x.pos - q.y.pos + L1;
        if (ok && dist >= 0 && dist < a.ins_n) {
          c.lc = code; c.L1 = L1; c.L2 = L2;
          q.dist = dist; q.scores = true; q.skip = false;
          q.memo_idx = ((code * 7 + q.x.edit) * 7 + q.y.edit) * a.ins_n + dist;
          const double tfl = code == 0 ? a.tfloor0 : a.tfloor_c[code], lfl = code == 0 ? a.logfloor0 : a.logfloor_c[code];
          const double2 m = a.memo[q.memo_idx];
          if (cap) *cap = PairVal{m.x, m.y, code, 1};
          compact_cover(a, c, q, m.x);
          __builtin_nontemporal_store(m.x, &a.probs[i]);
          const bool floored = m.x < tfl;
          lsum += floored ? lfl : m.y - a.log_two_T;
          zeros += (int)floored;
          return;
        }
      }
    }
    const double acc = score_regs<K>(a, x, y, L1, L2);
    finish_read(a, i, acc, L1, L2, lsum, zeros, cap);
}

template <int K, bool GEN>
__device__ __forceinline__ void paired_regs_body(const PairedArgs& a, int lb, int slot_lo, int slot_hi, int block_lo, int block_hi,
                                                 double& lsum, int& zeros, unsigned long long* tl = nullptr, int4* wave_lds = nullptr) {
  bool first_pair = true;
#ifdef GAML_GEN_STAMPS
  const unsigned long long tb_ = wall_clock64();
#endif
  for (int i = slot_lo + (lb - block_lo) * kBlock + threadIdx.x; i < slot_hi; i += (block_hi - block_lo) * kBlock) {
    const int t = i - a.n0;
    const uint32_t l12 = a.len12[t];
    const size_t at = K == 2 ? (size_t)2 * (i - a.n0) : (size_t)2 * (a.n01 - a.n0) + (size_t)4 * (i - a.n01);
    int4 r1[K], r2[K];
#pragma unroll
    for (int k = 0; k < K; k++) { r1[k] = a.inl[0][at + k]; r2[k] = a.inl[1][at + k]; }
    if (tl && first_pair) { asm volatile("s_waitcnt vmcnt(0)" ::: "memory"); if ((threadIdx.x & 63) == 0) tl[2] = (unsigned long long)wall_clock64() + (r1[0].x == 0x12345 ? 1 : 0); }
    RegCands<K> x, y;
    const bool m1 = cands_from_records<K>(a.m[0], r1, x), m2 = cands_from_records<K>(a.m[1], r2, y);
    if (tl && first_pair) { asm volatile("s_waitcnt vmcnt(0)" ::: "memory"); if ((threadIdx.x & 63) == 0) tl[3] = (unsigned long long)wall_clock64() + (x.pos[0] == 0x12345 ? 1 : 0); }
    const bool dirty = r1[0].x == kDirtyWid;
    const bool general = !dirty && (m1 || m2);
    if (!dirty && !general) score_cands_and_finish<K>(a, i, l12, x, y, lsum, zeros);
    if (tl && first_pair) { asm volatile("s_waitcnt vmcnt(0)" ::: "memory"); if ((threadIdx.x & 63) == 0) tl[5] = (unsigned long long)wall_clock64() + (lsum == 0.12345 ? 1 : 0); }
    first_pair = false;
    if (GEN && !GAML_GEN_OFF(2) && __any(general)) {
      int4* const slot = gen_wave_slot(wave_lds, general);
#ifdef GAML_GEN_STAMPS
      const unsigned long long tc0_ = wall_clock64();
#endif
      if (general) {
        double acc;
        const int L1 = l12 & 0xffff, L2 = l12 >> 16;
        int4 priv[K == 2 ? 2 * kGenCands : 1];
        if (K == 2 && general_pair_staged<K>(a, r1, r2, L1, L2, acc, slot ? slot : priv)) finish_read(a, i, acc, L1, L2, lsum, zeros);
        else { const GenOut o = general_pair_call(kernel_args_address(), i, -1, -1, slot); lsum += o.add; zeros += o.zeros; }
      }
#ifdef GAML_GEN_STAMPS
      if (general) { asm volatile("s_waitcnt vmcnt(0) lgkmcnt(0)" ::: "memory"); const unsigned long long tc1_ = wall_clock64(); atomicAdd(&g_gen_stamp[5], tc1_ - tc0_); atomicAdd(&g_gen_stamp[6], 1ull); atomicAdd(&g_gen_stamp[21], tc0_ - tb_); }
#endif
    }
  }
}

template <bool GEN>
__device__ __forceinline__ void paired_delta_body(const PairedArgs& a, int db, int delta_blocks, double& lsum, int& zeros, int4* wave_lds = nullptr) {
  for (int dj = db * kBlock + threadIdx.x; dj < a.dstate[kDsDirty]; dj += delta_blocks * kBlock) {
    const int i = a.dirty_slots[dj];
    const int sp = a.dirty_spill[dj];
    int4 r0[4], r1[4];
#pragma unroll
    for (int k = 0; k < 2; k++) { r0[k] = a.dirty_recs[0][4 * (size_t)dj + k]; r1[k] = a.dirty_recs[1][4 * (size_t)dj + k]; }
    const uint32_t l12 = (uint32_t)r0[0].w;
    const int c0 = r1[0].w & 0xff, c1 = (r1[0].w >> 8) & 0xff;
    bool general = false;
    if (__all(sp >= 0 || (c0 <= 2 && c1 <= 2))) {
      if (sp < 0) {
        RegCands<2> x, y;
        const int4 q0[2] = {r0[0], r0[1]}, q1[2] = {r1[0], r1[1]};
        const bool m0 = cands_from_records<2>(a.m[0], q0, x), m1 = cands_from_records<2>(a.m[1], q1, y);
        general = m0 || m1;
        if (!general) score_cands_and_finish<2>(a, i, l12, x, y, lsum, zeros);
      }
    } else if (sp < 0) {
#pragma unroll
      for (int k = 2; k < 4; k++) { r0[k] = a.dirty_recs[0][4 * (size_t)dj + k]; r1[k] = a.dirty_recs[1][4 * (size_t)dj + k]; }
      RegCands<4> x, y;
      const bool m0 = cands_from_records<4>(a.m[0], r0, x), m1 = cands_from_records<4>(a.m[1], r1, y);
      general = m0 || m1;
      if (!general) score_cands_and_finish<4>(a, i, l12, x, y, lsum, zeros);
    }
    if (GEN) {
      if (!GAML_GEN_OFF(4) && __any(general)) {
        int4* const slot = gen_wave_slot(wave_lds, general);
        if (general) { const GenOut o = general_pair_call(kernel_args_address(), i, dj, -1, slot); lsum += o.add; zeros += o.zeros; }
      }
    } else if (general) {
      lsum += __builtin_nan("");
    }
  }
}

struct DeltaPatch { int dj, slot, spill, pad; int4 rec[2][4]; };
struct DeltaPatch2 { int dj, slot, spill, pad; int4 rec[2][2]; };
__device__ __forceinline__ void mark_dirty_slot(int s, unsigned long long* rec8_0, int n0, int4* inl_0, int n01, int n_main, int4* first_0) {
  if (s < n0) rec8_0[s] = ~0ull - 1;
  else {
    if (s < n01) inl_0[(size_t)2 * (s - n0)].x = -2;
    else if (s < n_main) inl_0[(size_t)2 * (n01 - n0) + (size_t)4 * (s - n01)].x = -2;
    first_0[s - n0].x = -2;
  }
}
template <class Patch, int K>
__global__ __launch_bounds__(kBlock) void apply_delta_patch_kernel(const Patch* patch, int n, int* slots, int* spill, int4* rec0, int4* rec1, int mark_from,
                                                                   unsigned long long* rec8_0, int n0, int4* inl_0, int n01, int n_main, int4* first_0) {
  for (int t = blockIdx.x * kBlock + threadIdx.x; t < n; t += gridDim.x * kBlock) {
    const Patch p = patch[t];
    slots[p.dj] = p.slot;
    spill[p.dj] = p.spill;
#pragma unroll
    for (int k = 0; k < 4; k++) {
      rec0[4 * (size_t)p.dj + k] = k < K ? p.rec[0][k < K ? k : 0] : make_int4(-1, 0, 0, 0);
      rec1[4 * (size_t)p.dj + k] = k < K ? p.rec[1][k < K ? k : 0] : make_int4(-1, 0, 0, 0);
    }
    if (mark_from >= 0 && p.dj >= mark_from) mark_dirty_slot(p.slot, rec8_0, n0, inl_0, n01, n_main, first_0);
  }
}

template <bool TICKET, bool GEN, bool TL>
__device__ __forceinline__ void paired_main_body(const PairedArgs& a, int lb, double* sh_s, int* sh_z, int4* gen_lds) {
  double lsum = 0.0;
  int zeros = 0;
  unsigned long long* tl = TL ? a.timeline + ((size_t)blockIdx.x * (kBlock / 64) + (threadIdx.x >> 6)) * 8 : nullptr;
  if (TL && (threadIdx.x & 63) == 0) { tl[0] = wall_clock64(); tl[7] = lb < a.blocks0 ? 0 : (lb < a.blocks01 ? 1 : 2); }
  if (GAML_TIMING_X(8) && lb >= a.blocks0a) {
  } else if (GAML_TIMING_X(16) && lb < a.blocks0a) {
  } else if (lb < a.blocks0) {
    GAML_FRESH_ARGS(c, a)
    const bool wide = c.memo && !c.cov_bits;
    const SlotRange rg = compact_range(c, lb);
    const bool stat = wide && lb < c.blocks0a;
    if (!TL && wide && c.n_codes == 1) {
      if (stat) paired_static4_body<GEN, false, true>(c, rg, lsum, zeros);
      else paired_compact4_body<GEN, false, true>(c, rg, lsum, zeros);
    } else {
      __shared__ uint32_t sh_combo[256];
      __shared__ double sh_floor[256], sh_logfloor[256], sh_tfloor[256];
      for (int k = threadIdx.x; k < c.n_codes; k += kBlock) { sh_combo[k] = c.len_combo[k]; sh_floor[k] = c.floor_c[k]; sh_logfloor[k] = c.logfloor_c[k]; sh_tfloor[k] = c.tfloor_c ? c.tfloor_c[k] : 0.0; }
      __syncthreads();
      PairedArgs b = c;
      b.len_combo = sh_combo; b.floor_c = sh_floor; b.logfloor_c = sh_logfloor; b.tfloor_c = sh_tfloor;
      if (TL && (threadIdx.x & 63) == 0) tl[1] = wall_clock64();
      if (stat) paired_static4_body<GEN, TL>(b, rg, lsum, zeros);
      else if (wide) paired_compact4_body<GEN, TL>(b, rg, lsum, zeros);
      else paired_compact_body<GEN>(b, rg, lsum, zeros);
    }
  } else {
    int4* const wave_lds = GEN ? gen_lds + (threadIdx.x >> 6) * 2 * kOvfCap : nullptr;
    if (lb < a.blocks01) {
      GAML_FRESH_ARGS(c, a)
      paired_regs_body<2, GEN>(c, lb, c.n0, c.n01, c.blocks0, c.blocks01, lsum, zeros, tl, wave_lds);
    } else if (lb < a.blocks012) {
      GAML_FRESH_ARGS(c, a)
      paired_regs_body<4, GEN>(c, lb, c.n01, c.n_main, c.blocks01, c.blocks012, lsum, zeros, nullptr, wave_lds);
    } else {
      GAML_FRESH_ARGS(c, a)
      paired_delta_body<GEN>(c, lb - c.blocks012, c.main_blocks - c.blocks012, lsum, zeros, wave_lds);
    }
  }
  block_reduce(lsum, zeros, sh_s, sh_z);
  if (TL && (threadIdx.x & 63) == 0) tl[6] = wall_clock64();
  if (TICKET) {
    GAML_FRESH_ARGS(c, a)
    grid_finish(lsum, zeros, lb, c.total_blocks, c.part_sum, c.part_zero, c.ticket, c.out,
                c.cov_bits ? -1.0 : 0.0, c.n_reads, sh_s, sh_z, c.status_out, c.status_a, c.status_b);
  } else if (threadIdx.x == 0) {
    a.part_sum[lb] = lsum;
    a.part_zero[lb] = zeros;
  }
}

__global__ __launch_bounds__(kBlock) void finish_partials_kernel(const double* part_sum, const int* part_zero, int n_partials,
                                                                 double* out, double bad_bases, double n_reads,
                                                                 double* status_out = nullptr, double status_a = 0.0, double status_b = 0.0) {
  __shared__ double sh_s[kBlock / 64];
  __shared__ int sh_z[kBlock / 64];
  double ts = 0; int tz = 0;
  for (int b = threadIdx.x; b < n_partials; b += kBlock) { ts += part_sum[b]; tz += part_zero[b]; }
  block_reduce(ts, tz, sh_s, sh_z);
  if (threadIdx.x == 0) {
    out[0] = ts; out[1] = (double)tz; if (bad_bases >= 0) out[2] = bad_bases; out[3] = n_reads;
    if (status_out) { status_out[0] = status_a; status_out[1] = status_b; }
  }
}

constexpr int kOvfMaxBlocks = 1024;

template <class Src>
__device__ __forceinline__ int wave_gather(const MateView& v, const Src& src, int4* lds, int lane) {
  const int cnt = src.count();
  int total = 0;
  for (int base = 0; base < cnt; base += 64) {
    const int k = base + lane;
    int mine = 0;
    int4 r = make_int4(-1, 0, 0, 0), o = make_int4(0, 0, -1, 0);
    if (k < cnt) {
      r = src.get(k);
      if (r.x >= 0) { const Occ12 e = v.occ12[r.x]; o = occ_from_compact((unsigned long long)e.lo | ((unsigned long long)e.hi << 32), e.rank); }
      if (o.z >= 0) mine = o.w >= 0 ? 1 : v.multi_off[-o.w] - v.multi_off[-o.w - 1];
    }
    int incl = mine;
    for (int d = 1; d < 64; d <<= 1) { int t = __shfl_up(incl, d, 64); if (lane >= d) incl += t; }
    const int wave_total = __shfl(incl, 63, 64);
    const int at = total + incl - mine;
    if (total + wave_total > kOvfCap) return -1;
    if (mine == 1 && o.w >= 0) {
      lds[at] = make_int4(o.z, r.y + o.x, (r.z & 0x1ff) | ((r.y >= o.y) ? 0x200 : 0), o.w);
    } else if (mine > 0) {
      const int s = -o.w - 1;
      for (int q = 0; q < mine; q++) {
        const int4 oo = v.multi[v.multi_off[s] + q];
        lds[at + q] = make_int4(oo.z, r.y + oo.x, (r.z & 0x1ff) | ((r.y >= oo.y) ? 0x200 : 0), oo.w);
      }
    }
    total += wave_total;
  }
  return total;
}

template <class Src>
__device__ __forceinline__ double wave_score_pair(const PairedArgs& a, const Src& s1, const Src& s2, int L1, int L2, int4* c1, int4* c2, int lane) {
  const int n1 = wave_gather(a.m[0], s1, c1, lane);
  const int n2 = wave_gather(a.m[1], s2, c2, lane);
  double acc = 0.0;
  if (n1 < 0 || n2 < 0) {
    if (lane == 0) acc = paired_general_src(a, s1, s2, L1, L2);
    return acc;
  }
  __builtin_amdgcn_wave_barrier();
  for (int m = 0; m < 2; m++) {
    int4* c = m == 0 ? c1 : c2;
    const int n = m == 0 ? n1 : n2;
    for (int x = lane; x < n; x += 64) {
      int4 me = c[x];
      bool live = (me.z & 0x200) != 0;
      for (int y = 0; y < n && live; y++) {
        const int4 ot = c[y];
        if (y != x && (ot.z & 0x200) && ot.x == me.x && ot.y == me.y && (ot.w > me.w || (ot.w == me.w && y > x))) live = false;
      }
      if (live) me.z |= 0x400;
      c[x].z = me.z;
    }
  }
  __builtin_amdgcn_wave_barrier();
  const int pairs = n1 * n2;
  for (int idx = lane; idx < pairs; idx += 64) {
    const int4 xr = c1[idx / n2];
    const int4 yr = c2[idx % n2];
    if ((xr.z & 0x400) && (yr.z & 0x400) && xr.x == yr.x) {
      Cand x, y;
      x.path = xr.x; x.pos = xr.y; x.edit = xr.z & 0xff; x.orient = (xr.z >> 8) & 1;
      y.path = yr.x; y.pos = yr.y; y.edit = yr.z & 0xff; y.orient = (yr.z >> 8) & 1;
      acc += pair_term(a, x, y, L1, L2);
    }
  }
  for (int off = 32; off > 0; off >>= 1) acc += __shfl_xor(acc, off, 64);
  __builtin_amdgcn_wave_barrier();
  return acc;
}

template <bool TICKET>
__device__ __forceinline__ void paired_overflow_body(const PairedArgs& a, int ovf_block, int ovf_blocks, double* sh_s, int* sh_z,
                                                     int4 (*cand)[2][kOvfCap]) {
  const int lane = threadIdx.x & 63, wave = threadIdx.x >> 6;
  const int wave_global = ovf_block * (kBlock / 64) + wave;
  const int n_waves = ovf_blocks * (kBlock / 64);
  const int n_table = a.n - a.n_main;
  const int n_items = n_table + a.dstate[kDsSpill];
  double lsum = 0.0;
  int zeros = 0;
  int4* c1 = cand[wave][0];
  int4* c2 = cand[wave][1];
  for (int item = wave_global; item < n_items; item += n_waves) {
    if (item < n_table) {
      const int i = a.n_main + item;
      const int4 r1 = a.m[0].first[i - a.n0], r2 = a.m[1].first[i - a.n0];
      const uint32_t l12 = a.len12[i - a.n0];
      if (r1.x == kDirtyWid) continue;
      const int L1 = l12 & 0xffff, L2 = l12 >> 16;
      const double acc = wave_score_pair(a, TableSrc{&a.m[0], r1}, TableSrc{&a.m[1], r2}, L1, L2, c1, c2, lane);
      if (lane == 0) finish_read(a, i, acc, L1, L2, lsum, zeros);
    } else {
      const int sp = item - n_table;
      const int i = a.spill_slot[sp];
      const uint32_t l12 = i < a.n0 ? a.len_combo[a.len_code[i]] : a.len12[i - a.n0];
      const int L1 = l12 & 0xffff, L2 = l12 >> 16;
      const int2 g0 = a.spill_rng[0][sp], g1 = a.spill_rng[1][sp];
      const double acc = wave_score_pair(a, ListSrc{a.spill_recs[0] + g0.x, g0.y}, ListSrc{a.spill_recs[1] + g1.x, g1.y}, L1, L2, c1, c2, lane);
      if (lane == 0) finish_read(a, i, acc, L1, L2, lsum, zeros);
    }
  }
  block_reduce(lsum, zeros, sh_s, sh_z);
  if (TICKET) {
    grid_finish(lsum, zeros, a.main_blocks + ovf_block, a.total_blocks, a.part_sum, a.part_zero, a.ticket, a.out,
                a.cov_bits ? -1.0 : 0.0, a.n_reads, sh_s, sh_z, a.status_out, a.status_a, a.status_b);
  } else if (threadIdx.x == 0) {
    a.part_sum[a.main_blocks + ovf_block] = lsum;
    a.part_zero[a.main_blocks + ovf_block] = zeros;
  }
}

#ifndef GAML_GEN_WAVES
#define GAML_GEN_WAVES 4
#endif
template <bool TICKET, bool GEN = false, bool TL = false>
__global__ __launch_bounds__(kBlock, GEN ? GAML_GEN_WAVES : 5) void paired_score_kernel(PairedArgs a) {
  __shared__ double sh_s[kBlock / 64];
  __shared__ int sh_z[kBlock / 64];
  __shared__ int4 cand[kBlock / 64][2][kOvfCap];
  const int lb = a.total_blocks - 1 - (int)blockIdx.x;
#if GAML_LEAN_ENTRY && defined(__HIP_DEVICE_COMPILE__)
  if (!TL && lb < a.blocks0a && a.memo && !a.cov_bits && a.n_codes == 1) {
    double lsum = 0.0;
    int zeros = 0;
    if (!GAML_TIMING_X(16))
    paired_static4_body<GEN, false, true>(a, SlotRange{0, a.n0a, lb, a.blocks0a}, lsum, zeros);
    block_reduce(lsum, zeros, sh_s, sh_z);
    if (TICKET) grid_finish(lsum, zeros, lb, a.total_blocks, a.part_sum, a.part_zero, a.ticket, a.out, 0.0, a.n_reads, sh_s, sh_z, a.status_out, a.status_a, a.status_b);
    else if (threadIdx.x == 0) { a.part_sum[lb] = lsum; a.part_zero[lb] = zeros; }
    return;
  }
  if (lb < a.main_blocks) paired_main_body<TICKET, GEN, TL>(a, lb, sh_s, sh_z, &cand[0][0][0]);
  else if (GAML_GEN_OFF(16)) { if (threadIdx.x == 0) { a.part_sum[lb] = 0.0; a.part_zero[lb] = 0; } }
  else {
    GAML_FRESH_ARGS(c, a)
    paired_overflow_body<TICKET>(c, lb - c.main_blocks, c.total_blocks - c.main_blocks, sh_s, sh_z, cand);
  }
#else
  if (lb < a.main_blocks) paired_main_body<TICKET, GEN, TL>(a, lb, sh_s, sh_z, &cand[0][0][0]);
  else paired_overflow_body<TICKET>(a, lb - a.main_blocks, a.total_blocks - a.main_blocks, sh_s, sh_z, cand);
#endif
}

constexpr int kMaxSets = 8;
struct SetDev {
  const Occ12* occ12[2];
  const int* multi_off[2];
  const int4* multi[2];
  const double* tfloor_c;
  double tfloor0;
  double two_T, log_two_T;
  double* part_sum;
  int* part_zero;
};
struct MultiSets { int n; int pad_; const unsigned char* chg[2]; SetDev set[kMaxSets]; };

constexpr int kTfCodes = 16;
__device__ __forceinline__ PairedArgs with_set(const PairedArgs& a, const SetDev& sd, const double* tfloor_lds = nullptr) {
  PairedArgs b = a;
#pragma unroll
  for (int mt = 0; mt < 2; mt++) { b.m[mt].occ12 = sd.occ12[mt]; b.occ12[mt] = sd.occ12[mt]; b.m[mt].multi_off = sd.multi_off[mt]; b.m[mt].multi = sd.multi[mt]; }
  b.tfloor_c = tfloor_lds ? tfloor_lds : sd.tfloor_c; b.tfloor0 = sd.tfloor0; b.two_T = sd.two_T; b.log_two_T = sd.log_two_T;
  b.part_sum = sd.part_sum; b.part_zero = sd.part_zero;
  return b;
}

struct MultiKernArgs { PairedArgs a; MultiSets ms; };
#if defined(__HIP_DEVICE_COMPILE__)
#define GAML_CALLEE_ARGS(name, set)                                                                                                  \
  const unsigned long long name##_u = ((unsigned long long)(unsigned)__builtin_amdgcn_readfirstlane((int)(kernargs >> 32)) << 32) |  \
                                      (unsigned)__builtin_amdgcn_readfirstlane((int)kernargs);          \
  const __attribute__((address_space(4))) MultiKernArgs* name##_p = (const __attribute__((address_space(4))) MultiKernArgs*)name##_u; \
  const PairedArgs name##_0 = name##_p->a;                                                                                           \
  const PairedArgs name = (set) >= 0 ? with_set(name##_0, name##_p->ms.set[set]) : name##_0;
#else
#define GAML_CALLEE_ARGS(name, set) const PairedArgs& name = *(const PairedArgs*)nullptr;
#endif
__device__ __noinline__ GenOut compact_general_call(unsigned long long kernargs, int i, int set) {
  GAML_CALLEE_ARGS(a, set)
  GenOut o{0.0, 0};
  compact_general(a, i, o.add, o.zeros);
  return o;
}
__device__ __noinline__ GenOut general_pair_call(unsigned long long kernargs, int i, int dj, int set, int4* lds) {
  GAML_CALLEE_ARGS(a, set)
  GenOut o{0.0, 0};
  int4 priv[2 * kGenCands];
  int4* const cand = lds ? lds : priv;
  const int4 none = make_int4(-1, 0, 0, 0);
  int4 r1[4], r2[4];
  double acc;
  if (dj < 0) {
    const bool four = i >= a.n01;
    const size_t at = four ? (size_t)2 * (a.n01 - a.n0) + (size_t)4 * (i - a.n01) : (size_t)2 * (i - a.n0);
#pragma unroll
    for (int k = 0; k < 4; k++) { const bool has = four || k < 2; r1[k] = has ? a.inl[0][at + (has ? k : 0)] : none; r2[k] = has ? a.inl[1][at + (has ? k : 0)] : none; }
    const uint32_t l12 = a.len12[i - a.n0];
    const int L1 = l12 & 0xffff, L2 = l12 >> 16;
    if (!general_pair_staged<4>(a, r1, r2, L1, L2, acc, cand)) acc = paired_general(a, a.m[0].first[i - a.n0], a.m[1].first[i - a.n0], L1, L2);
    finish_read(a, i, acc, L1, L2, o.add, o.zeros);
  } else {
#pragma unroll
    for (int k = 0; k < 4; k++) { r1[k] = a.dirty_recs[0][4 * (size_t)dj + k]; r2[k] = a.dirty_recs[1][4 * (size_t)dj + k]; }
    const uint32_t l12 = (uint32_t)r1[0].w;
    const int L1 = l12 & 0xffff, L2 = l12 >> 16;
    const int c0 = r2[0].w & 0xff, c1 = (r2[0].w >> 8) & 0xff;
    if (!general_pair_staged<4>(a, r1, r2, L1, L2, acc, cand))
      acc = paired_general_src_masks(a, ListSrc{a.dirty_recs[0] + 4 * (size_t)dj, c0}, ListSrc{a.dirty_recs[1] + 4 * (size_t)dj, c1}, L1, L2);
    finish_read(a, i, acc, L1, L2, o.add, o.zeros);
  }
  return o;
}

template <bool GEN, bool ONE>
__device__ __forceinline__ void paired_compact4_multi_body(const PairedArgs& a, const MultiSets& ms, const SlotRange rg, double* acc_s, int* acc_z, const double* tf) {
  const unsigned stride = (unsigned)rg.blocks * kBlock, n0 = (unsigned)rg.hi;
  const char* const rec0 = (const char*)a.rec8[0];
  const char* const rec1 = (const char*)a.rec8[1];
  const char* const memo = (const char*)a.memo;
  char* const probs = (char*)a.probs;
  const uint32_t l12_one = ONE ? a.len_combo[0] : 0u;
  const double logfloor_one = ONE ? a.logfloor_c[0] : 0.0;
  for (unsigned base = (unsigned)rg.lo + (unsigned)rg.lb * kBlock + threadIdx.x; base < n0; base += 4 * stride) {
// ... 571 lines not shown
```

gaml_amd/csrc/occ_device.hip.h:

```cpp
#pragma once

namespace {

constexpr int kOccMaxDesc = 32;

struct OccDesc { long long off; int slot, start; };
struct OccScatterArgs {
  const OccPre* pool[2];
  Occ12* dst[2];
  int* dst_list[2];
  Occ12* clr[2];
  const int* clr_list[2];
  unsigned* stamp[2];
  int* dup;
  int n_desc, total[2], n_clr[2];
  unsigned serial;
  OccDesc desc[2][kOccMaxDesc];
};

__global__ void __launch_bounds__(kBlock) occ_scatter_kernel(const OccScatterArgs a) {
  const int t0 = a.total[0], t01 = t0 + a.total[1], c0 = t01 + a.n_clr[0], n = c0 + a.n_clr[1];
  for (int i = blockIdx.x * blockDim.x + threadIdx.x; i < n; i += gridDim.x * blockDim.x) {
    if (i < t01) {
      const int mt = i < t0 ? 0 : 1;
      const int j = mt ? i - t0 : i;
      int d = 0;
      while (d + 1 < a.n_desc && a.desc[mt][d + 1].start <= j) d++;
      const OccDesc& D = a.desc[mt][d];
      const OccPre e = a.pool[mt][D.off + (j - D.start)];
      Occ12* o = a.dst[mt] + e.wid;
      o->lo = e.lo; o->hi = e.hi | ((unsigned)D.slot << 16); o->rank = e.rank;
      a.dst_list[mt][j] = e.wid;
      if (atomicExch(a.stamp[mt] + e.wid, a.serial) == a.serial) *(volatile int*)a.dup = 1;
    } else {
      const int mt = i < c0 ? 0 : 1;
      const int j = mt ? i - c0 : i - t01;
      Occ12* o = a.clr[mt] + a.clr_list[mt][j];
      o->lo = ~0u; o->hi = ~0u; o->rank = -1;
    }
  }
}

bool paired_resident_route(const gaml_hip_ctx* c, const PairedSet& s) {
  return c->host_results && c->direct_write && KNOB(c, 8) == 0 && KNOB(c, 13) == 0 && !(s.cfg.penalty_constant > 0);
}

bool occdev_route_ok(const gaml_hip_ctx* c, PairedSet& s) {
  PairedSet::OccDev& D = s.occdev;
  if (!c->occ_route || KNOB(c, 17) != 0 || !paired_resident_route(c, s) || !s.persist.valid) return false;
  if (s.planner.last_was_incremental()) return false;
  const std::vector<int32_t>& ids = s.planner.ids();
  if (ids.empty() || ids.size() > (size_t)kOccMaxDesc) return false;
  D.key.clear();
  for (int32_t id : ids) {
    const PathMemo& pm = s.planner.memo(id);
    if (!pm.pre_plain[0] || !pm.pre_plain[1]) return false;
    D.key.push_back((uint64_t)(uint32_t)id << 32 | pm.serial);
  }
  for (const auto& k : D.shared) if (k == D.key) return false;
  return true;
}

void occdev_note_shared(PairedSet::OccDev& D) {
  constexpr size_t kShared = 16;
  if (D.shared.size() < kShared) D.shared.push_back(D.key);
  else { D.shared[D.shared_next] = D.key; D.shared_next = (D.shared_next + 1) % kShared; }
}

int occdev_reserve(gaml_hip_ctx* c, PairedSet& s, size_t n_windows, size_t n_occ, hipStream_t st) {
  PairedSet::OccDev& D = s.occdev;
  if (D.cap_w > 0 && n_windows <= D.cap_w && n_occ <= D.cap_list) return 0;
  HIP_TRY(c, hipStreamSynchronize(st));
  D.cap_w = std::max(std::max<size_t>(4 * n_windows, (size_t)1 << 18), D.cap_w);
  D.cap_list = std::max(std::max<size_t>(2 * n_occ, (size_t)1 << 16), D.cap_list);
  for (int mt = 0; mt < 2; mt++) {
    for (int k = 0; k < 2; k++) {
      HIP_TRY(c, D.tab[mt][k].reserve(D.cap_w * sizeof(Occ12)));
      HIP_TRY(c, hipMemsetAsync(D.tab[mt][k].p, 0xff, D.cap_w * sizeof(Occ12), st));
      HIP_TRY(c, D.list[mt][k].reserve(D.cap_list * sizeof(int32_t)));
      D.list_n[mt][k] = 0;
    }
    HIP_TRY(c, D.stamp[mt].reserve(D.cap_w * sizeof(uint32_t)));
    HIP_TRY(c, hipMemsetAsync(D.stamp[mt].p, 0, D.cap_w * sizeof(uint32_t), st));
  }
  D.serial = 0;
  return 0;
}

int occdev_upload(gaml_hip_ctx* c, PairedSet& s, hipStream_t st, size_t* bytes) {
  PairedSet::OccDev& D = s.occdev;
  const std::vector<int32_t>& ids = s.planner.ids();
  auto missing = [&](const PathMemo& pm, int mt) { return pm.dev_off[mt] < 0 || pm.dev_gen[mt] != D.pool_gen; };
  size_t need[2] = {0, 0}, whole[2] = {0, 0};
  for (int32_t id : ids)
    for (int mt = 0; mt < 2; mt++) { const PathMemo& pm = s.planner.memo(id); whole[mt] += pm.pre[mt].size(); if (missing(pm, mt)) need[mt] += pm.pre[mt].size(); }
  if (D.pool_used[0] + need[0] > D.pool_cap[0] || D.pool_used[1] + need[1] > D.pool_cap[1]) {
    HIP_TRY(c, hipStreamSynchronize(st));
    for (int mt = 0; mt < 2; mt++) {
      if (2 * whole[mt] > D.pool_cap[mt]) {
        D.pool_cap[mt] = std::max<size_t>(8 * whole[mt], 2 * D.pool_cap[mt]);
        HIP_TRY(c, D.pool[mt].reserve(D.pool_cap[mt] * sizeof(OccPre)));
      }
      D.pool_used[mt] = 0;
      need[mt] = whole[mt];
    }
    D.pool_gen++;
    D.compactions++;
  }
  *bytes = (need[0] + need[1]) * sizeof(OccPre);
  if (need[0] + need[1] == 0) return 0;
  HIP_TRY(c, D.stage.reserve(*bytes));
  OccPre* sp = (OccPre*)D.stage.p;
  for (int mt = 0; mt < 2; mt++) {
    const size_t at = D.pool_used[mt];
    size_t k = 0;
    for (int32_t id : ids) {
      PathMemo& pm = s.planner.memo(id);
      if (!missing(pm, mt)) continue;
      pm.dev_off[mt] = (int64_t)(at + k);
      pm.dev_gen[mt] = D.pool_gen;
      if (!pm.pre[mt].empty()) memcpy(sp + k, pm.pre[mt].data(), pm.pre[mt].size() * sizeof(OccPre));
      k += pm.pre[mt].size();
    }
    if (k) HIP_TRY(c, hipMemcpyAsync(D.pool[mt].as<OccPre>() + at, sp, k * sizeof(OccPre), hipMemcpyHostToDevice, st));
    D.pool_used[mt] = at + k;
    sp += k;
  }
  return 0;
}

int occdev_launch(gaml_hip_ctx* c, PairedSet& s, hipStream_t st, size_t* bytes) {
  PairedSet::OccDev& D = s.occdev;
  const std::vector<int32_t>& ids = s.planner.ids();
  if (D.pool_cap[0] == 0 || D.pool_cap[1] == 0) {
    for (int mt = 0; mt < 2; mt++) {
      size_t all = 0;
      for (int32_t id : ids) all += s.planner.memo(id).pre[mt].size();
      D.pool_cap[mt] = std::max<size_t>(16 * all, (size_t)1 << 10);
      HIP_TRY(c, D.pool[mt].reserve(D.pool_cap[mt] * sizeof(OccPre)));
      D.pool_used[mt] = 0;
    }
    D.pool_gen++;
  }
  size_t n_occ[2] = {0, 0};
  for (int32_t id : ids) for (int mt = 0; mt < 2; mt++) n_occ[mt] += s.planner.memo(id).pre[mt].size();
  const size_t n_windows = std::max(s.mate[0].wins.size(), s.mate[1].wins.size());
  if (int e = occdev_reserve(c, s, n_windows, std::max(n_occ[0], n_occ[1]), st)) return e;
  if (int e = occdev_upload(c, s, st, bytes)) return e;
  HIP_TRY(c, D.dup.reserve(sizeof(int)));
  *(volatile int*)D.dup.p = 0;
  if (++D.serial == 0) {
    for (int mt = 0; mt < 2; mt++) HIP_TRY(c, hipMemsetAsync(D.stamp[mt].p, 0, D.cap_w * sizeof(uint32_t), st));
    D.serial = 1;
  }
  const int cur = (int)(D.serial & 1), other = cur ^ 1;
  OccScatterArgs a;
  memset(&a, 0, sizeof(a));
  a.n_desc = (int)ids.size();
  for (int mt = 0; mt < 2; mt++) {
    a.pool[mt] = D.pool[mt].as<OccPre>();
    a.dst[mt] = D.tab[mt][cur].as<Occ12>();
    a.dst_list[mt] = D.list[mt][cur].as<int>();
    a.clr[mt] = D.tab[mt][other].as<Occ12>();
    a.clr_list[mt] = D.list[mt][other].as<int>();
    a.stamp[mt] = D.stamp[mt].as<unsigned>();
    int start = 0;
    for (size_t k = 0; k < ids.size(); k++) {
      const PathMemo& pm = s.planner.memo(ids[k]);
      a.desc[mt][k] = OccDesc{(long long)pm.dev_off[mt], (int)k, start};
      start += (int)pm.pre[mt].size();
    }
    a.total[mt] = start;
    a.n_clr[mt] = D.list_n[mt][other];
    D.list_n[mt][cur] = start;
    D.list_n[mt][other] = 0;
  }
  a.dup = (int*)D.dup.dev;
  a.serial = D.serial;
  const int items = a.total[0] + a.total[1] + a.n_clr[0] + a.n_clr[1];
  if (items > 0) {
    hipLaunchKernelGGL(occ_scatter_kernel, dim3((unsigned)std::min(512, (items + kBlock - 1) / kBlock)), dim3(kBlock), 0, st, a);
    HIP_TRY(c, hipGetLastError());
  }
  return 0;
}

const Occ12* occdev_table(const PairedSet& s, int mt) { return s.occdev.tab[mt][s.occdev.serial & 1].as<Occ12>(); }

void paired_images_refresh(PairedSet& s) {
  if (!s.occdev.image_stale) return;
  s.planner.rebuild_images(s.mate, s.image);
  s.occdev.image_stale = false;
}

}
```

gaml_amd/csrc/paired_launch.hip.h:

```cpp
#pragma once

namespace {

int paired_host_tabs(gaml_hip_ctx* c, PairedSet& s) {
  if (!s.ins_tab.empty() || !s.floor_tab.empty()) return 0;
  const double c0 = s.cfg.min_prob_start, k0 = s.cfg.min_prob_per_base;
  auto ins = [&](int d) {
    double z = ((double)d - s.cfg.insert_mean) / s.cfg.insert_std;
    return std::exp(-z * z / 2.0) / (std::sqrt(2 * M_PI) * s.cfg.insert_std);
  };
  const int kInsCap = 1 << 22;
  s.ins_tab.clear();
  for (int d = 0; d < kInsCap; d++) {
    double v = ins(d);
    if (v == 0.0 && (double)d > s.cfg.insert_mean) break;
    s.ins_tab.push_back(v);
  }
  if ((int)s.ins_tab.size() >= kInsCap)
    return fail(c, GAML_HIP_EINVAL, "insert_std too large: the insert-size table would exceed 4M entries");
  int smax = s.mate[0].max_len + s.mate[1].max_len;
  s.floor_tab.resize(smax + 1);
  s.logfloor_tab.resize(smax + 1);
  for (int v = 0; v <= smax; v++) {
    s.floor_tab[v] = std::exp(c0 + k0 * v);
    s.logfloor_tab[v] = std::log(s.floor_tab[v]);
    if (!(s.floor_tab[v] > 0.0)) s.floor_positive = false;
  }
  s.covthr_tab.resize(s.mate[1].max_len + 1);
  for (int v = 0; v <= s.mate[1].max_len; v++) s.covthr_tab[v] = std::exp(c0 + k0 * (v + v));
  return 0;
}

int prepare_paired_tables(gaml_hip_ctx* c, PairedSet& s) {
  if (s.tabs_uploaded) return 0;
  if (int e = paired_host_tabs(c, s)) return e;
  size_t total = s.ins_tab.size() + s.floor_tab.size() + s.logfloor_tab.size() + s.covthr_tab.size();
  HIP_TRY(c, s.tabs.reserve(std::max<size_t>(1, total) * sizeof(double)));
  double* d = s.tabs.as<double>();
  size_t at = 0;
  auto up = [&](const std::vector<double>& v) -> hipError_t {
    hipError_t e = v.empty() ? hipSuccess : hipMemcpy(d + at, v.data(), v.size() * sizeof(double), hipMemcpyHostToDevice);
    at += v.size();
    return e;
  };
  HIP_TRY(c, up(s.ins_tab));
  HIP_TRY(c, up(s.floor_tab));
  HIP_TRY(c, up(s.logfloor_tab));
  HIP_TRY(c, up(s.covthr_tab));
  const int64_t n = s.mate[0].n_local();
  HIP_TRY(c, s.probs.reserve(std::max<size_t>(1, n) * sizeof(double)));
  HIP_TRY(c, s.red.init());
  HIP_TRY(c, s.bad.reserve(sizeof(unsigned long long)));
  s.tabs_uploaded = true;
  return 0;
}

int prepare_paired_structure(gaml_hip_ctx* c, PairedSet& s, const int32_t* flat, const int64_t* offs, int32_t n_paths) {
  const bool incremental = !(s.cfg.penalty_constant > 0) && KNOB(c, 12) == 0;
  std::string err;
  if (!s.planner.begin(c->g, s.mate, flat, offs, n_paths, incremental, &err)) return fail(c, GAML_HIP_EINVAL, err);
  return 0;
}

int prepare_paired_tables_host(gaml_hip_ctx* c, PairedSet& s, PairedPrep& p, hipStream_t st = nullptr, bool device_route = false) {
  static const bool trace = getenv("GAML_HIP_TRACE_HOST") != nullptr;
  const double q0 = now_us();
  s.planner.finish(s.mate);
  PairedSet::OccDev& D = s.occdev;
  D.taken = device_route && occdev_route_ok(c, s);
  size_t up_bytes = 0;
  if (D.taken) { if (int e = occdev_launch(c, s, st, &up_bytes)) return e; }
  c->prof[6] = (double)up_bytes;
  const double q1 = now_us();
  const bool cov = s.cfg.penalty_constant > 0;
  p.path_base.assign(1, 0);
  p.start_off.assign(1, 0);
  p.starts.clear();
  if (cov) {
    const PlanView& v = s.planner.view();
    p.path_base.reserve(v.paths.size() + 1);
    p.start_off.reserve(v.paths.size() + 1);
    for (const PathMemo* pm : v.paths) {
      p.starts.insert(p.starts.end(), pm->starts.begin(), pm->starts.end());
      p.start_off.push_back((int32_t)p.starts.size());
      int32_t bits = ((pm->length + 64 + 31) / 32) * 32;
      p.path_base.push_back(p.path_base.back() + bits);
    }
  }
  p.total_bits = p.path_base.back();
  p.n_paths = s.planner.n_paths();
  const double q2 = now_us();
  s.planner.apply(s.mate, s.image, !D.taken, D.image_stale);
  D.image_stale = D.taken;
  if (D.taken) D.dev_calls++; else D.host_calls++;
  p.assembled_records = s.planner.assembled(0) + s.planner.assembled(1);
  p.general = !D.taken && (!s.image[0].general_wids.empty() || !s.image[1].general_wids.empty());
  if (trace) fprintf(stderr, "pass2: finish %.1f us, starts %.1f us, images %.1f us\n", q1 - q0, q2 - q1, now_us() - q2);
  return 0;
}

}
#include "paired_tables.hip.h"
namespace {

double tfloor_for(double floor, double two_T) {
  if (!(floor > 0.0)) return 0.0;
  double x = floor * two_T;
  for (int k = 0; k < 64 && x > 0.0 && (std::nextafter(x, 0.0) / two_T) >= floor; k++) x = std::nextafter(x, 0.0);
  for (int k = 0; k < 64 && (x / two_T) < floor; k++) x = std::nextafter(x, std::numeric_limits<double>::infinity());
  return x;
}

struct PairedLayout { size_t tfloor_off; OccLayout l0, l1; size_t pb_off, so_off, st_off, total; };

PairedLayout paired_layout(const PairedSet& s, const PairedPrep& p, const size_t* pad_to = nullptr) {
  PairedLayout L;
  L.tfloor_off = 0;
  const size_t hdr = align16(256 * sizeof(double));
  L.l0 = layout_image(s.image[0], hdr, pad_to ? pad_to[0] : 0);
  L.l1 = layout_image(s.image[1], L.l0.end, pad_to ? pad_to[1] : 0);
  L.pb_off = L.l1.end; L.so_off = L.st_off = 0; L.total = L.l1.end;
  if (s.cfg.penalty_constant > 0) {
    L.so_off = align16(L.pb_off + p.path_base.size() * sizeof(int32_t));
    L.st_off = align16(L.so_off + p.start_off.size() * sizeof(int32_t));
    L.total = align16(L.st_off + p.starts.size() * sizeof(int32_t));
  }
  return L;
}

void paired_pack_thresholds(const PairedSet& s, const PairedLayout& L, double two_T, char* dst) {
  double tf[256];
  const size_t nc = std::min<size_t>(256, s.pt.len_combo.size());
  for (size_t ci = 0; ci < nc; ci++) {
    const int L0 = (int)(s.pt.len_combo[ci] & 0xffff), L1 = (int)(s.pt.len_combo[ci] >> 16);
    tf[ci] = tfloor_for(s.floor_tab[L0 + L1], two_T);
  }
  if (nc) memcpy(dst + L.tfloor_off, tf, nc * sizeof(double));
}

void paired_pack(const PairedSet& s, const PairedPrep& p, const PairedLayout& L, char* dst) {
  pack_image(s.image[0], L.l0, dst);
  pack_image(s.image[1], L.l1, dst);
  if (s.cfg.penalty_constant > 0) {
    memcpy(dst + L.pb_off, p.path_base.data(), p.path_base.size() * sizeof(int32_t));
    memcpy(dst + L.so_off, p.start_off.data(), p.start_off.size() * sizeof(int32_t));
    memcpy(dst + L.st_off, p.starts.data(), p.starts.size() * sizeof(int32_t));
  }
}

int arena_acquire(gaml_hip_ctx* c, Arena& A, size_t bytes, hipStream_t st, int* slot_out, char** write_ptr) {
  const int k = A.next;
  A.next = (A.next + 1) % kRing;
  if (A.armed[k]) { HIP_TRY(c, hipEventSynchronize(A.done[k])); A.armed[k] = false; }
  if (!A.done[k]) HIP_TRY(c, hipEventCreateWithFlags(&A.done[k], hipEventDisableTiming));
  const bool direct = c->direct_write && KNOB(c, 8) == 0;
  if (bytes > A.cap[k] || A.direct[k] != direct) {
    HIP_TRY(c, hipStreamSynchronize(st));
    if (A.dev[k]) { HIP_TRY(c, hipFree(A.dev[k])); A.dev[k] = nullptr; A.cap[k] = 0; }
    const size_t want = std::max<size_t>(bytes + bytes / 2, (size_t)1 << 20);
    if (direct) HIP_TRY(c, hipExtMallocWithFlags(&A.dev[k], want, hipDeviceMallocFinegrained));
    else HIP_TRY(c, hipMalloc(&A.dev[k], want));
    A.cap[k] = want; A.direct[k] = direct;
  }
  if (direct) *write_ptr = (char*)A.dev[k];
  else { HIP_TRY(c, A.host[k].reserve(bytes)); *write_ptr = (char*)A.host[k].p; }
  *slot_out = k;
  return 0;
}

int arena_commit(gaml_hip_ctx* c, Arena& A, int k, size_t bytes, hipStream_t st) {
  if (A.direct[k]) { _mm_sfence(); return 0; }
  if (bytes == 0) return 0;
  if (KNOB(c, 8) == 1 || (bytes & 15)) { HIP_TRY(c, hipMemcpyAsync(A.dev[k], A.host[k].p, bytes, hipMemcpyHostToDevice, st)); return 0; }
  const int n16 = (int)(bytes / 16);
  hipLaunchKernelGGL(stage_copy_kernel, dim3((unsigned)std::min(64, (n16 + kBlock - 1) / kBlock)), dim3(kBlock), 0, st,
                     (const int4*)A.host[k].dev, (int4*)A.dev[k], n16);
  HIP_TRY(c, hipGetLastError());
// ... 194 lines not shown
  HIP_TRY(c, s.h_part_zero.reserve(per * sizeof(int) * kMaxSets));
  *d_sum = (double*)s.h_part_sum.dev;
  *d_zero = (int*)s.h_part_zero.dev;
  double* hs = (double*)s.h_part_sum.p;
  int* hz = (int*)s.h_part_zero.p;
  for (int k = first_set; k < first_set + n_sets; k++) {
    for (int b2 = 0; b2 < n_partials; b2++) { hs[(size_t)k * per + b2] = std::numeric_limits<double>::quiet_NaN(); hz[(size_t)k * per + b2] = INT_MIN; }
    s.last_blocks[k] = n_partials;
  }
  s.host_part_stride = per;
  return 0;
}

int launch_paired(gaml_hip_ctx* c, PairedSet& s, PairedPrep& p, int32_t total_len, hipStream_t st, double* out4) {
  const double tpp = now_us();
  if (int e = prepare_paired_tables(c, s)) return e;
  const double tp0 = now_us();
  if (int e = prepare_paired_tables_host(c, s, p, st, true)) return e;
  const double t_after_host = now_us();
  c->prof[1] = t_after_host - tp0;
  gpu_probe(st, c->warm_buf.p, "before table sync");
  if (int e = paired_sync_tables(c, s, st)) return e;
  const double tp1 = now_us();
  c->prof[4] = tp1 - t_after_host;
  if (tp1 - t_after_host > 1000.0 && getenv("GAML_HIP_TRACE_HOST")) fprintf(stderr, "table sync took %.0f us (evaluation %lld of the set, rebuild active %d slice %d)\n", tp1 - t_after_host, (long long)s.eval_count, (int)s.rebuild.active, s.rebuild.next_slice);

  const bool cov = s.cfg.penalty_constant > 0;
  const int tl = total_len == 0 ? 1 : total_len;
  const bool resident = paired_resident_route(c, s);
  PairedLayout L;
  memset(&L, 0, sizeof(L));
  int slot = -1;
  const char* arena = nullptr;
  SetDev sd;
  s.occdev.check_dup = s.occdev.taken;
  if (s.occdev.taken) {
    PairedLayout Lt;
    Lt.tfloor_off = s.persist.off_tfloor;
    paired_pack_thresholds(s, Lt, (double)(2 * tl), (char*)s.persist.dev);
    _mm_sfence();
    paired_persist_view(s, total_len, sd);
    for (int mt = 0; mt < 2; mt++) sd.occ12[mt] = occdev_table(s, mt);
    c->prof[6] += 256.0 * sizeof(double);
  } else if (resident) {
    c->prof[6] = (double)((s.image[0].changed_all || s.image[1].changed_all || !s.persist.valid) ? (s.image[0].occ12.size() + s.image[1].occ12.size()) * sizeof(Occ12)
                                                                                            : (s.image[0].changed.size() + s.image[1].changed.size()) * sizeof(Occ12));
    if (int e = paired_persist_update(c, s, (double)(2 * tl), st)) return e;
    paired_persist_view(s, total_len, sd);
  } else {
    L = paired_layout(s, p);
    char* wp = nullptr;
    if (int e = arena_acquire(c, s.arena, L.total, st, &slot, &wp)) return e;
    paired_pack(s, p, L, wp);
    paired_pack_thresholds(s, L, (double)(2 * tl), wp);
    if (int e = arena_commit(c, s.arena, slot, L.total, st)) return e;
    arena = (const char*)s.arena.dev[slot];
    paired_set_view(s, L, arena, total_len, sd);
    c->prof[6] = (double)L.total;
  }
  const double tp2 = now_us();
  c->prof[3] = tp2 - tp1;

  PairedArgs a;
  GridPlan gp;
  paired_base_args(c, s, a, gp);
  const int64_t n = s.mate[0].n_local();
  if (cov) {
    size_t words = (size_t)p.total_bits / 32;
    if (words * 4 > s.cov_bits.cap) { HIP_TRY(c, hipStreamSynchronize(st)); HIP_TRY(c, s.cov_bits.reserve(std::max<size_t>(4, words * 4))); }
    HIP_TRY(c, hipMemsetAsync(s.cov_bits.p, 0, std::max<size_t>(4, words * 4), st));
    HIP_TRY(c, hipMemsetAsync(s.bad.p, 0, sizeof(unsigned long long), st));
    a.cov_bits = s.cov_bits.as<uint32_t>();
    a.path_base = (const int*)(arena + L.pb_off);
  }
  const bool gen_set = a.n_main > 0 && p.general;
  const int n_partials = gp.total_blocks;
  sd.part_sum = s.red.part_sum.as<double>();
  sd.part_zero = s.red.part_zero.as<int>();
  if (c->host_results && n > 0) { if (int e = paired_host_partials(c, s, 0, 1, n_partials, &sd.part_sum, &sd.part_zero)) return e; }
  s.last_blocks[0] = n > 0 ? n_partials : 0;
  s.last_host_partials = c->host_results;
  s.last_sets = 1;
  paired_apply_set(a, sd);
  a.out = out4;
  a.timeline = nullptr;
  const bool timeline = KNOB(c, 3) == 8;
  if (timeline) {
    HIP_TRY(c, s.h_timeline.reserve((size_t)(4 * kMaxBlocks + kOvfMaxBlocks + 256) * (kBlock / 64) * 8 * sizeof(unsigned long long)));
    memset(s.h_timeline.p, 0, s.h_timeline.cap);
    a.timeline = (unsigned long long*)s.h_timeline.dev;
    s.timeline_waves = a.total_blocks * (kBlock / 64);
  }

  std::pair<hipEvent_t, hipEvent_t>* ev = nullptr;
  if (n > 0) {
    if (c->event_timing && (c->event_tick++ % c->event_every) == 0) { if (int e = take_events(c, &ev)) return e; }
    int fin_mode = c->host_results ? 2 : (KNOB(c, 2) ? KNOB(c, 2) - 1 : 1);
    double* status_out = nullptr;
    if (fin_mode != 2 && c->status_dst && !c->status_done) { status_out = c->status_dst; c->status_done = true; }
    if (fin_mode == 0) { a.status_out = status_out; a.status_a = c->status_a; a.status_b = c->status_b; }
    s.last_total_blocks = n_partials;
    const dim3 grid(a.total_blocks), block(kBlock);
    hipEvent_t e0 = ev ? ev->first : nullptr, e1 = ev ? ev->second : nullptr;
#define GAML_LAUNCH_SCORE(...) hipExtLaunchKernelGGL((paired_score_kernel<__VA_ARGS__>), grid, block, KNOB(c, 1), st, e0, e1, 0, a)
#ifdef GAML_HIP_DEV
    if (timeline) GAML_LAUNCH_SCORE(false, false, true);
    else
#endif
    if (gen_set) { if (fin_mode) GAML_LAUNCH_SCORE(false, true); else GAML_LAUNCH_SCORE(true, true); }
    else if (fin_mode) GAML_LAUNCH_SCORE(false, false);
    else GAML_LAUNCH_SCORE(true, false);
#undef GAML_LAUNCH_SCORE
    HIP_TRY(c, hipGetLastError());
    if (fin_mode == 1) {
      hipLaunchKernelGGL(finish_partials_kernel, dim3(1), dim3(kBlock), 0, st, a.part_sum, a.part_zero, n_partials, out4, cov ? -1.0 : 0.0, (double)n, status_out, c->status_a, c->status_b);
      HIP_TRY(c, hipGetLastError());
    }
  } else {
    s.last_total_blocks = 0;
    if (!c->host_results) HIP_TRY(c, hipMemsetAsync(out4, 0, 4 * sizeof(double), st));
  }
  if (cov && c->defer_cov) {
    int idx = 0;
    for (size_t i = 0; i < c->paireds.size(); i++) if (c->paireds[i].get() == &s) idx = (int)i;
    c->pending_cov.push_back(gaml_hip_ctx::PendingCov{idx, paired_cov_args(s, p, L, arena), out4});
  } else if (cov && n > 0 && p.total_bits > 0) {
    const CovArgs ca = paired_cov_args(s, p, L, arena);
    hipLaunchKernelGGL(coverage_sweep_kernel, dim3(grid_for(ca.total_words)), dim3(kBlock), 0, st, ca);
    HIP_TRY(c, hipGetLastError());
  }
  if (cov && n > 0 && !c->defer_cov) {
    hipLaunchKernelGGL(store_bad_bases_kernel, dim3(1), dim3(64), 0, st, s.bad.as<unsigned long long>(), out4, 1.0);
    HIP_TRY(c, hipGetLastError());
  }
  if (slot >= 0) { if (int e = arena_release(c, s.arena, slot, st)) return e; }
  c->prof[5] = now_us() - tp2;
  if (now_us() - tpp > 5000.0 && getenv("GAML_HIP_TRACE_HOST"))
    fprintf(stderr, "launch_paired: fixed tables %.2f ms, pass 2 %.2f, table sync %.2f, per-call tables %.2f, launches %.2f\n", (tp0 - tpp) * 1e-3, (t_after_host - tp0) * 1e-3,
            (tp1 - t_after_host) * 1e-3, (tp2 - tp1) * 1e-3, (now_us() - tp2) * 1e-3);
  if (!c->event_timing || ev) {
    c->stat_algo_bytes += 16.0 * (double)p.assembled_records + 16.0 * (double)n;
    c->stat_launches++;
  }
  c->t_host_us += t_after_host;
  return 0;
}

bool paired_multi_capable(const gaml_hip_ctx* c, const PairedSet& s) {
  return !(s.cfg.penalty_constant > 0) && KNOB(c, 3) == 0 && KNOB(c, 4) == 0 && s.floor_positive;
}

int launch_paired_multi(gaml_hip_ctx* c, PairedSet& s, int first, int n_sets, const PairedLayout* L, const PairedPrep* preps, const int32_t* total_lens,
                        const char* arena, size_t stride, hipStream_t st, const unsigned char* const* chg = nullptr) {
  PairedArgs a;
  GridPlan gp;
  paired_base_args(c, s, a, gp);
  if (!a.memo) return fail(c, GAML_HIP_ESTATE, "multi-set launch without a memo (caller must check paired_multi_capable)");
  const int64_t n = s.mate[0].n_local();
  bool any_set = false;
  for (int k = first; k < first + n_sets; k++) any_set = any_set || (a.n_main > 0 && preps[k].general);
  const int n_partials = gp.total_blocks;
  double* d_sum = nullptr;
  int* d_zero = nullptr;
  s.last_total_blocks = n > 0 ? n_partials : 0;
  s.last_host_partials = true;
  s.last_sets = first + n_sets;
  if (n == 0) { for (int k = first; k < first + n_sets; k++) s.last_blocks[k] = 0; return 0; }
  if (int e = paired_host_partials(c, s, first, n_sets, n_partials, &d_sum, &d_zero)) return e;
  MultiSets ms;
  memset(&ms, 0, sizeof(ms));
  ms.n = n_sets;
  if (KNOB(c, 11) >= 32) ms.pad_ = (KNOB(c, 11) - 32) & 31;
  if (chg && KNOB(c, 11) < 64) { ms.chg[0] = chg[0]; ms.chg[1] = chg[1]; }
  for (int k = 0; k < n_sets; k++) {
    const int g = first + k;
    paired_set_view(s, L[g], arena + (size_t)g * stride, total_lens[g], ms.set[k]);
    ms.set[k].part_sum = d_sum + (size_t)g * s.host_part_stride;
    ms.set[k].part_zero = d_zero + (size_t)g * s.host_part_stride;
  }
  paired_apply_set(a, ms.set[0]);
  std::pair<hipEvent_t, hipEvent_t>* ev = nullptr;
  if (c->event_timing && (c->event_tick++ % c->event_every) == 0) { if (int e = take_events(c, &ev)) return e; }
  hipEvent_t e0 = ev ? ev->first : nullptr, e1 = ev ? ev->second : nullptr;
  const dim3 grid(a.total_blocks), block(kBlock);
  if (any_set) hipExtLaunchKernelGGL((paired_score_multi_kernel<true>), grid, block, 0, st, e0, e1, 0, a, ms);
  else hipExtLaunchKernelGGL((paired_score_multi_kernel<false>), grid, block, 0, st, e0, e1, 0, a, ms);
  HIP_TRY(c, hipGetLastError());
  if (!c->event_timing || ev) {
    double rec = 0;
    for (int k = first; k < first + n_sets; k++) rec += (double)preps[k].assembled_records;
    c->stat_algo_bytes += 16.0 * rec + 16.0 * (double)n * n_sets;
    c->stat_launches++;
// ... 6 lines not shown
```

include/gaml_hip_debug.h:

```cpp
#ifndef GAML_HIP_DEBUG_H_
#define GAML_HIP_DEBUG_H_

#include "gaml_hip.h"

#ifdef __cplusplus
extern "C" {
#endif

int gaml_hip_debug_sam_logprob(gaml_hip_ctx* ctx, const char* target, int32_t target_len, const char* read, int32_t read_len,
                               const char* sam_line, int64_t sam_len, double mismatch_prob, double* logprob_out,
                               int32_t* band_lo, int32_t* band_hi, int32_t band_cap);
int gaml_hip_debug_sam_shape(const char* sam_line, int64_t len, int32_t total_len, int32_t* out6, uint32_t* ops, int32_t cap);
int32_t gaml_hip_debug_sam_band(const char* sam_line, int64_t len, int32_t total_len, int32_t* fields10, int32_t* row0,
                                int32_t* lo, int32_t* hi, int32_t cap);

int gaml_hip_debug_prepare(gaml_hip_ctx* ctx, const int32_t* paths, const int64_t* path_offs, int32_t n_paths);
int64_t gaml_hip_debug_occurrences(gaml_hip_ctx* ctx, int readset, int mate, int32_t* out5, int64_t cap);
int64_t gaml_hip_debug_table_occurrences(gaml_hip_ctx* ctx, int readset, int mate, int32_t* out5, int64_t cap, int64_t* info3);
int32_t gaml_hip_debug_window_walk(gaml_hip_ctx* ctx, int readset, int mate, int32_t window_id, int32_t* out, int32_t cap);
int gaml_hip_debug_timeline(gaml_hip_ctx* ctx, int rs, unsigned long long* out, int64_t cap_waves);

int gaml_hip_debug_set_knob(gaml_hip_ctx* ctx, int knob, int value);
int gaml_hip_debug_fold_check(gaml_hip_ctx* ctx, int readset, int64_t* out6);
int gaml_hip_debug_radix_sort(gaml_hip_ctx* ctx, uint64_t* keys, uint64_t* vals, int64_t n, int begin_bit, int end_bit, uint64_t* run_max);
int gaml_hip_debug_static_check(gaml_hip_ctx* ctx, int readset, int64_t* out8);
int gaml_hip_debug_tables_check(gaml_hip_ctx* ctx, int readset, int64_t* out8);
int32_t gaml_hip_debug_block_partials(gaml_hip_ctx* ctx, int readset, int32_t set, double* sums, int32_t* zeros, int32_t cap, int32_t* layout8);

int gaml_hip_debug_occ_route(gaml_hip_ctx* ctx, int readset, int64_t* out6);
int gaml_hip_debug_occ_check(gaml_hip_ctx* ctx, int readset, int64_t* out4);

#ifdef __cplusplus
}
#endif
#endif
```

Measured before the change: 61.68 billion reads/s.

## Memoize per-path dense occurrence tables on device and merge at score time

Adds a memo route for calls with at most two paths. Each path's occurrence prepack is expanded once into a dense per-window table that stays on the device and is reused across calls, keyed by path memo and generation. The scoring kernel then merges the two path tables per lookup instead of rebuilding a combined table every call. The cost is two loads per lookup, a flag store when a window occurs on both paths, a device memory budget that can force restarts, and an error path for call modes the memo route does not serve.

After: 70.11 billion reads/s (median of 6 runs). +13.7%, better.

```diff
diff --git a/gaml_amd/api.py b/gaml_amd/api.py
--- a/gaml_amd/api.py
+++ b/gaml_amd/api.py
@@ -196,6 +196,8 @@
         L.gaml_hip_debug_set_knob.argtypes = [vp, C.c_int, C.c_int]
     if hasattr(L, "gaml_hip_debug_occ_route"):
         L.gaml_hip_debug_occ_route.argtypes = [vp, C.c_int, _i64p]
+    if hasattr(L, "gaml_hip_debug_occ_memo"):
+        L.gaml_hip_debug_occ_memo.argtypes = [vp, C.c_int, _i64p]
     if hasattr(L, "gaml_hip_debug_occ_check"):
         L.gaml_hip_debug_occ_check.argtypes = [vp, C.c_int, _i64p]
     if hasattr(L, "gaml_hip_shm_exchange_open"):
@@ -727,8 +729,13 @@
     def debug_occ_route(self, rs):
         out = np.zeros(6, np.int64)
         self._check(_lib.gaml_hip_debug_occ_route(self._h, rs, out))
-        return {"device": int(out[0]), "host": int(out[1]), "fallbacks": int(out[2]), "compactions": int(out[3]),
-                "pool_entries": int(out[4]), "shared_combinations": int(out[5])}
+        res = {"device": int(out[0]), "host": int(out[1]), "fallbacks": int(out[2]), "compactions": int(out[3]),
+               "pool_entries": int(out[4]), "shared_combinations": int(out[5])}
+        if hasattr(_lib, "gaml_hip_debug_occ_memo"):
+            m = np.zeros(4, np.int64)
+            self._check(_lib.gaml_hip_debug_occ_memo(self._h, rs, m))
+            res.update({"memo": int(m[0]), "dense_restarts": int(m[1]), "dense_bytes_used": int(m[2]), "dense_bytes_held": int(m[3])})
+        return res
 
     def debug_occ_check(self, rs):
         out = np.zeros(4, np.int64)
diff --git a/gaml_amd/csrc/ctx.hip.h b/gaml_amd/csrc/ctx.hip.h
--- a/gaml_amd/csrc/ctx.hip.h
+++ b/gaml_amd/csrc/ctx.hip.h
@@ -306,9 +306,16 @@
     size_t shared_next = 0;
     std::vector<uint64_t> key;
     int64_t dev_calls = 0, host_calls = 0, fallbacks = 0, compactions = 0;
+    DevBuf dense[2];
+    size_t dense_cap[2] = {0, 0}, dense_used[2] = {0, 0};
+    uint32_t dense_gen = 1;
+    bool memo = false;
+    const Occ12* memo_tab[2][2] = {{nullptr, nullptr}, {nullptr, nullptr}};
+    uint32_t memo_n[2][2] = {{0, 0}, {0, 0}};
+    int64_t memo_calls = 0, dense_restarts = 0;
     void release() {
       for (int mt = 0; mt < 2; mt++) {
-        pool[mt].release(); stamp[mt].release();
+        pool[mt].release(); stamp[mt].release(); dense[mt].release();
         for (int k = 0; k < 2; k++) { tab[mt][k].release(); list[mt][k].release(); }
       }
       stage.release(); dup.release();
diff --git a/gaml_amd/csrc/debug_api.hip.h b/gaml_amd/csrc/debug_api.hip.h
--- a/gaml_amd/csrc/debug_api.hip.h
+++ b/gaml_amd/csrc/debug_api.hip.h
@@ -311,6 +311,16 @@
   return GAML_HIP_OK;
 }
 
+int gaml_hip_debug_occ_memo(gaml_hip_ctx* c, int rs, int64_t* out4) {
+  MULTI_SHARD0(c);
+  if (!c || !out4 || rs < 0 || rs >= (int)c->handles.size() || c->handles[rs].kind != 1) return fail(c, GAML_HIP_EINVAL, "bad arguments");
+  const PairedSet::OccDev& D = c->paireds[c->handles[rs].idx]->occdev;
+  out4[0] = D.memo_calls; out4[1] = D.dense_restarts;
+  out4[2] = (int64_t)((D.dense_used[0] + D.dense_used[1]) * sizeof(Occ12));
+  out4[3] = (int64_t)(D.dense[0].cap + D.dense[1].cap);
+  return GAML_HIP_OK;
+}
+
 int gaml_hip_debug_occ_check(gaml_hip_ctx* c, int rs, int64_t* out4) {
   MULTI_SHARD0(c);
   if (!c || !out4 || rs < 0 || rs >= (int)c->handles.size() || c->handles[rs].kind != 1) return fail(c, GAML_HIP_EINVAL, "bad arguments");
@@ -326,7 +336,21 @@
     im.build(ps.mate[mt].wins.size(), v, mt);
     const size_t n = im.occ12.size();
     std::vector<Occ12> dev(n);
-    if (n) HIP_TRY(c, hipMemcpy(dev.data(), occdev_table(ps, mt), n * sizeof(Occ12), hipMemcpyDeviceToHost));
+    if (n && D.memo) {
+      std::vector<Occ12> t[2];
+      for (int k = 0; k < 2; k++) {
+        t[k].resize((size_t)D.memo_n[mt][k] + 1);
+        HIP_TRY(c, hipMemcpy(t[k].data(), D.memo_tab[mt][k], t[k].size() * sizeof(Occ12), hipMemcpyDeviceToHost));
+      }
+      for (size_t w = 0; w < n; w++) {
+        const Occ12& ea = t[0][std::min<size_t>(w, D.memo_n[mt][0])];
+        Occ12 eb = t[1][std::min<size_t>(w, D.memo_n[mt][1])];
+        const bool in_a = ea.hi != ~0u, in_b = eb.hi != ~0u;
+        eb.hi |= 0x10000u;
+        dev[w] = in_a ? ea : eb;
+        if (in_a && in_b) out4[2]++;
+      }
+    } else if (n) HIP_TRY(c, hipMemcpy(dev.data(), occdev_table(ps, mt), n * sizeof(Occ12), hipMemcpyDeviceToHost));
     for (size_t w = 0; w < n; w++) {
       const Occ12& h = im.occ12[w];
       const Occ12& d = dev[w];
diff --git a/gaml_amd/csrc/host_model.cc b/gaml_amd/csrc/host_model.cc
--- a/gaml_amd/csrc/host_model.cc
+++ b/gaml_amd/csrc/host_model.cc
@@ -971,6 +971,7 @@
       occ_prepack(pm.occ[mt], pm.pre[mt]);
       pm.pre_plain[mt] = occ_pre_plain(pm.pre[mt]);
       pm.dev_off[mt] = -1;
+      pm.dense_off[mt] = -1;
       pm.occ_valid[mt] = true;
     }
   };
diff --git a/gaml_amd/csrc/host_model.h b/gaml_amd/csrc/host_model.h
--- a/gaml_amd/csrc/host_model.h
+++ b/gaml_amd/csrc/host_model.h
@@ -233,6 +233,9 @@
   bool pre_plain[2] = {false, false};
   int64_t dev_off[2] = {-1, -1};
   uint32_t dev_gen[2] = {0, 0};
+  int64_t dense_off[2] = {-1, -1};
+  uint32_t dense_gen[2] = {0, 0};
+  int32_t dense_n[2] = {0, 0};
   int64_t assembled[2] = {0, 0};
   std::vector<int32_t> starts;
   int32_t length = 0;
diff --git a/gaml_amd/csrc/kernels.hip.h b/gaml_amd/csrc/kernels.hip.h
--- a/gaml_amd/csrc/kernels.hip.h
+++ b/gaml_amd/csrc/kernels.hip.h
@@ -20,6 +20,7 @@
   const double* mism_pow;
   const double* match_pow;
 };
+struct OccMemo { const Occ12* tb; uint32_t na, nb; };
 
 struct PairedArgs {
   int total_blocks, blocks0a, n0a, n_codes;
@@ -73,7 +74,24 @@
   double n_reads;
   double* status_out;
   double status_a, status_b;
+  OccMemo om[2];
+  int* occ_dup;
 };
+__device__ __forceinline__ OccMemo occ_memo_of(int mt) {
+#if defined(__HIP_DEVICE_COMPILE__)
+  const __attribute__((address_space(4))) PairedArgs* ka = (const __attribute__((address_space(4))) PairedArgs*)__builtin_amdgcn_kernarg_segment_ptr();
+  return OccMemo{ka->om[mt].tb, ka->om[mt].na, ka->om[mt].nb};
+#else
+  return OccMemo{nullptr, 0u, 0u};
+#endif
+}
+__device__ __forceinline__ void occ_flag_shared() {
+#if defined(__HIP_DEVICE_COMPILE__)
+  const __attribute__((address_space(4))) PairedArgs* ka = (const __attribute__((address_space(4))) PairedArgs*)__builtin_amdgcn_kernarg_segment_ptr();
+  int* const dup = ka->occ_dup;
+  asm volatile("global_store_dword %0, %1, off sc0 sc1\n\ts_waitcnt vmcnt(0)" ::"v"(dup), "v"(1));
+#endif
+}
 
 struct Cand { int path, pos, edit, orient, rank, k; bool valid; };
 
@@ -81,9 +99,40 @@
   const int4 e = make_int4((int)(unsigned)o, (int)(short)(o >> 32), (int)((o >> 48) & 0x7fff), rk);
   return o == ~0ull ? make_int4(0, 0, -1, 0) : e;
 }
-__device__ __forceinline__ int4 mate_occ(const MateView& v, int w) {
-  if (v.occ) return v.occ[w];
-  const Occ12 e = v.occ12[w];
+template <bool MEMO, bool RANK, bool WIDE = false>
+__device__ __forceinline__ Occ12 occ_entry(const Occ12* ta, const Occ12* tb, unsigned na, unsigned nb, unsigned w, bool& both) {
+  Occ12 e;
+  if (!MEMO) {
+    const Occ12* p = WIDE ? (const Occ12*)((const char*)ta + w * 12u) : ta + w;
+    e.lo = p->lo; e.hi = p->hi; e.rank = RANK ? p->rank : 0;
+    return e;
+  }
+  const Occ12* pa = (const Occ12*)((const char*)ta + min(w, na) * 12u);
+  const Occ12* pb = (const Occ12*)((const char*)tb + min(w, nb) * 12u);
+  const unsigned alo = pa->lo, ahi = pa->hi, blo = pb->lo, bhi = pb->hi;
+  const int ark = RANK ? pa->rank : 0, brk = RANK ? pb->rank : 0;
+  const bool in_a = ahi != ~0u;
+  both |= in_a & (bhi != ~0u);
+  e.lo = in_a ? alo : blo; e.hi = in_a ? ahi : (bhi | 0x10000u); e.rank = in_a ? ark : brk;
+  return e;
+}
+template <bool MEMO>
+__device__ __forceinline__ Occ12 occ_entry_of(const MateView& v, int mt, unsigned w, bool& both) {
+  OccMemo om = OccMemo{nullptr, 0u, 0u};
+  if (MEMO) om = occ_memo_of(mt);
+  return occ_entry<MEMO, true>(v.occ12, om.tb, om.na, om.nb, w, both);
+}
+template <bool MEMO>
+__device__ __forceinline__ unsigned long long occ8_at(const PairedArgs& a, int mt, unsigned w, bool& both) {
+  const Occ12 e = occ_entry<MEMO, false>(a.occ12[mt], a.om[mt].tb, a.om[mt].na, a.om[mt].nb, w, both);
+  return (unsigned long long)e.lo | ((unsigned long long)e.hi << 32);
+}
+template <bool MEMO = false>
+__device__ __forceinline__ int4 mate_occ(const MateView& v, int w, int mt = 0) {
+  if (!MEMO && v.occ) return v.occ[w];
+  bool both = false;
+  const Occ12 e = occ_entry_of<MEMO>(v, mt, (unsigned)w, both);
+  if (MEMO && both) occ_flag_shared();
   return occ_from_compact((unsigned long long)e.lo | ((unsigned long long)e.hi << 32), e.rank);
 }
 
@@ -107,13 +156,13 @@
   __device__ __forceinline__ int4 get(int k) const { return recs[k]; }
 };
 
-template <class Src, class F>
-__device__ __forceinline__ void for_each_cand_src(const MateView& v, const Src& src, F f) {
+template <bool MEMO = false, class Src, class F>
+__device__ __forceinline__ void for_each_cand_src(const MateView& v, const Src& src, F f, int mt = 0) {
   const int cnt = src.count();
   for (int k = 0; k < cnt; k++) {
     int4 r = src.get(k);
     if (r.x < 0) continue;
-    int4 o = mate_occ(v, r.x);
+    int4 o = mate_occ<MEMO>(v, r.x, mt);
     if (o.z < 0) continue;
     if (o.w >= 0) {
       f(make_cand(r, o, k));
@@ -128,13 +177,13 @@
   for_each_cand_src(v, TableSrc{&v, r0}, f);
 }
 
-template <class Src>
-__device__ __forceinline__ bool is_live_src(const MateView& v, const Src& src, const Cand& c) {
+template <bool MEMO = false, class Src>
+__device__ __forceinline__ bool is_live_src(const MateView& v, const Src& src, const Cand& c, int mt = 0) {
   if (!c.valid) return false;
   bool live = true;
-  for_each_cand_src(v, src, [&](const Cand& d) {
+  for_each_cand_src<MEMO>(v, src, [&](const Cand& d) {
     if (d.valid && d.path == c.path && d.pos == c.pos && (d.rank > c.rank || (d.rank == c.rank && d.k > c.k))) live = false;
-  });
+  }, mt);
   return live;
 }
 __device__ __forceinline__ bool is_live(const MateView& v, const int4& r0, const Cand& c) {
@@ -168,17 +217,17 @@
   return t;
 }
 
-template <class Src>
+template <bool MEMO = false, class Src>
 __device__ __forceinline__ double paired_general_src_slow(const PairedArgs& a, const Src& s1, const Src& s2, int L1, int L2) {
   double acc = 0.0;
-  for_each_cand_src(a.m[0], s1, [&](const Cand& x) {
-    if (!is_live_src(a.m[0], s1, x)) return;
-    for_each_cand_src(a.m[1], s2, [&](const Cand& y) {
+  for_each_cand_src<MEMO>(a.m[0], s1, [&](const Cand& x) {
+    if (!is_live_src<MEMO>(a.m[0], s1, x, 0)) return;
+    for_each_cand_src<MEMO>(a.m[1], s2, [&](const Cand& y) {
       if (y.path != x.path) return;
-      if (!is_live_src(a.m[1], s2, y)) return;
+      if (!is_live_src<MEMO>(a.m[1], s2, y, 1)) return;
       acc += pair_term(a, x, y, L1, L2);
-    });
-  });
+    }, 1);
+  }, 0);
   return acc;
 }
 template <class Src>
@@ -212,9 +261,9 @@
   });
   return acc;
 }
-template <class Src>
+template <bool MEMO = false, class Src>
 __device__ __forceinline__ double paired_general_src(const PairedArgs& a, const Src& s1, const Src& s2, int L1, int L2) {
-  return paired_general_src_slow(a, s1, s2, L1, L2);
+  return paired_general_src_slow<MEMO>(a, s1, s2, L1, L2);
 }
 __device__ __forceinline__ double paired_general(const PairedArgs& a, const int4& r1, const int4& r2, int L1, int L2) {
   return paired_general_src_masks(a, TableSrc{&a.m[0], r1}, TableSrc{&a.m[1], r2}, L1, L2);
@@ -287,13 +336,14 @@
   bool valid[K], live[K];
 };
 
-template <int K>
-__device__ __forceinline__ bool cands_from_records(const MateView& v, const int4 (&r)[K], RegCands<K>& c) {
+template <int K, bool MEMO = false>
+__device__ __forceinline__ bool cands_from_records(const MateView& v, const int4 (&r)[K], RegCands<K>& c, int mt = 0) {
   int4 o[K];
-  bool multi = false;
+  bool multi = false, both = false;
   Occ12 e[K];
 #pragma unroll
-  for (int k = 0; k < K; k++) e[k] = v.occ12[r[k].x >= 0 ? r[k].x : 0];
+  for (int k = 0; k < K; k++) e[k] = occ_entry_of<MEMO>(v, mt, (unsigned)(r[k].x >= 0 ? r[k].x : 0), both);
+  if (MEMO && both) occ_flag_shared();
 #pragma unroll
   for (int k = 0; k < K; k++) o[k] = occ_from_compact((unsigned long long)e[k].lo | ((unsigned long long)e[k].hi << 32), e[k].rank);
 #pragma unroll
@@ -542,7 +592,7 @@
   return lb < a.blocks0a ? SlotRange{0, a.n0a, lb, a.blocks0a} : SlotRange{a.n0a, a.n0, lb - a.blocks0a, a.blocks0 - a.blocks0a};
 }
 
-template <bool GEN>
+template <bool GEN, bool MEMO = false>
 __device__ __forceinline__ void paired_compact_body(const PairedArgs& a, const SlotRange rg, double& lsum, int& zeros) {
   const int stride = rg.blocks * kBlock, hi = rg.hi;
   int i0 = rg.lo + rg.lb * kBlock + threadIdx.x;
@@ -563,10 +613,12 @@
     const bool d0 = c0.r1 == kDirty8, d1 = c1.r1 == kDirty8;
     if (d0) { c0.r1 = kNone8; c0.r2 = kNone8; }
     if (d1) { c1.r1 = kNone8; c1.r2 = kNone8; }
-    c0.o1 = c0.r1 != kNone8 ? occ8_of(a.occ12[0], (unsigned)(c0.r1 & 0xffffff)) : kNone8;
-    c0.o2 = c0.r2 != kNone8 ? occ8_of(a.occ12[1], (unsigned)(c0.r2 & 0xffffff)) : kNone8;
-    c1.o1 = c1.r1 != kNone8 ? occ8_of(a.occ12[0], (unsigned)(c1.r1 & 0xffffff)) : kNone8;
-    c1.o2 = c1.r2 != kNone8 ? occ8_of(a.occ12[1], (unsigned)(c1.r2 & 0xffffff)) : kNone8;
+    bool both = false;
+    c0.o1 = c0.r1 != kNone8 ? occ8_at<MEMO>(a, 0, (unsigned)(c0.r1 & 0xffffff), both) : kNone8;
+    c0.o2 = c0.r2 != kNone8 ? occ8_at<MEMO>(a, 1, (unsigned)(c0.r2 & 0xffffff), both) : kNone8;
+    c1.o1 = c1.r1 != kNone8 ? occ8_at<MEMO>(a, 0, (unsigned)(c1.r1 & 0xffffff), both) : kNone8;
+    c1.o2 = c1.r2 != kNone8 ? occ8_at<MEMO>(a, 1, (unsigned)(c1.r2 & 0xffffff), both) : kNone8;
+    if (MEMO && both) occ_flag_shared();
     CompactPrep q0, q1;
     compact_prep(a, c0, q0);
     compact_prep(a, c1, q1);
@@ -606,7 +658,7 @@
   return state;
 }
 
-template <bool GEN, bool TL = false, bool ONE = false>
+template <bool GEN, bool TL = false, bool ONE = false, bool MEMO = false>
 __device__ __forceinline__ void paired_compact4_body(const PairedArgs& a, const SlotRange rg, double& lsum, int& zeros) {
   const unsigned stride = (unsigned)rg.blocks * kBlock, n0 = (unsigned)rg.hi;
   unsigned long long* tl = TL ? a.timeline + ((size_t)blockIdx.x * (kBlock / 64) + (threadIdx.x >> 6)) * 8 : nullptr;
@@ -622,6 +674,7 @@
   for (unsigned base = (unsigned)rg.lo + (unsigned)rg.lb * kBlock + threadIdx.x; base < n0; base += 4 * stride) {
     uint2 r1[4], r2[4], o1[4], o2[4];
     unsigned lc[4];
+    bool both = false;
 #pragma unroll
     for (int k = 0; k < 4; k++) {
       const unsigned ic = base + k * stride < n0 ? base + k * stride : base;
@@ -630,9 +683,9 @@
     GAML_STAMP(2, r1[0].x ^ r1[1].x ^ r1[2].x ^ r1[3].x ^ r2[0].x ^ r2[3].x)
 #pragma unroll
     for (int k = 0; k < 4; k++) {
-      const Occ12* e1 = (const Occ12*)(occ0 + (r1[k].y != ~0u ? (r1[k].x & 0xffffffu) : 0u) * 12u);
-      const Occ12* e2 = (const Occ12*)(occ1 + (r2[k].y != ~0u ? (r2[k].x & 0xffffffu) : 0u) * 12u);
-      o1[k] = make_uint2(e1->lo, e1->hi); o2[k] = make_uint2(e2->lo, e2->hi);
+      const Occ12 e1 = occ_entry<MEMO, false, true>((const Occ12*)occ0, a.om[0].tb, a.om[0].na, a.om[0].nb, r1[k].y != ~0u ? (r1[k].x & 0xffffffu) : 0u, both);
+      const Occ12 e2 = occ_entry<MEMO, false, true>((const Occ12*)occ1, a.om[1].tb, a.om[1].na, a.om[1].nb, r2[k].y != ~0u ? (r2[k].x & 0xffffffu) : 0u, both);
+      o1[k] = make_uint2(e1.lo, e1.hi); o2[k] = make_uint2(e2.lo, e2.hi);
     }
     GAML_STAMP(3, o1[0].x ^ o1[1].x ^ o1[2].x ^ o1[3].x ^ o2[0].x ^ o2[3].x)
     int state[4];
@@ -663,6 +716,7 @@
       } else other |= state[k] == kPairOther && !((skip_bits >> k) & 1u);
     }
     GAML_STAMP(5, 0u)
+    if (MEMO && both) occ_flag_shared();
     if (__any(other)) {
 #pragma unroll 1
       for (int k = 0; k < 4; k++) {
@@ -670,8 +724,9 @@
         const int i = (int)(base + k * stride);
         Compact1 d;
         compact_load(a, i, true, d);
-        d.o1 = d.r1 != kNone8 ? occ8_of(a.occ12[0], (unsigned)(d.r1 & 0xffffff)) : kNone8;
-        d.o2 = d.r2 != kNone8 ? occ8_of(a.occ12[1], (unsigned)(d.r2 & 0xffffff)) : kNone8;
+        bool again = false;
+        d.o1 = d.r1 != kNone8 ? occ8_at<MEMO>(a, 0, (unsigned)(d.r1 & 0xffffff), again) : kNone8;
+        d.o2 = d.r2 != kNone8 ? occ8_at<MEMO>(a, 1, (unsigned)(d.r2 & 0xffffff), again) : kNone8;
         const uint32_t l = a.len_combo[d.lc];
         d.L1 = l & 0xffff; d.L2 = l >> 16;
         CompactPrep q;
@@ -718,7 +773,7 @@
   }
 }
 
-template <bool GEN, bool TL = false, bool ONE = false>
+template <bool GEN, bool TL = false, bool ONE = false, bool MEMO = false>
 __device__ __forceinline__ void paired_static4_body(const PairedArgs& a, const SlotRange rg, double& lsum, int& zeros) {
   constexpr int P = GAML_STATIC_P;
   const unsigned stride = (unsigned)rg.blocks * kBlock, n0 = (unsigned)rg.hi;
@@ -746,12 +801,13 @@
   while (true) {
     GAML_STAMP(2, r1[0].x ^ r2[0].x ^ (unsigned)__double2loint(m[0].x))
     uint2 o1[P], o2[P];
+    bool both_paths = false;
 #pragma unroll
     for (int k = 0; k < P; k++) {
       const unsigned w1 = (r1[k].x & 0xffffffu) & (0u - (unsigned)(r1[k].y != ~0u)), w2 = (r2[k].x & 0xffffffu) & (0u - (unsigned)(r2[k].y != ~0u));
-      const Occ12* e1 = (const Occ12*)(occ0 + w1 * 12u);
-      const Occ12* e2 = (const Occ12*)(occ1 + w2 * 12u);
-      o1[k] = make_uint2(e1->lo, e1->hi); o2[k] = make_uint2(e2->lo, e2->hi);
+      const Occ12 e1 = occ_entry<MEMO, false, true>((const Occ12*)occ0, a.om[0].tb, a.om[0].na, a.om[0].nb, w1, both_paths);
+      const Occ12 e2 = occ_entry<MEMO, false, true>((const Occ12*)occ1, a.om[1].tb, a.om[1].na, a.om[1].nb, w2, both_paths);
+      o1[k] = make_uint2(e1.lo, e1.hi); o2[k] = make_uint2(e2.lo, e2.hi);
       if (GAML_TIMING_X(1)) { o1[k] = make_uint2(r1[k].x >> 8, 0u); o2[k] = make_uint2(r1[k].x >> 8, 0u); }
     }
     const unsigned nbase = base + P * stride;
@@ -794,6 +850,7 @@
       zeros += (int)floored;
       if (counted && !GAML_TIMING_X(2)) __builtin_nontemporal_store(t, (double*)(probs + (base + k * stride) * 8u));
     }
+    if (MEMO && both_paths) occ_flag_shared();
     if (GEN && !GAML_GEN_OFF(1) && __any(skip_bits != 0)) {
 #pragma unroll 1
       for (int k = 0; k < P; k++)
@@ -971,7 +1028,7 @@
     finish_read(a, i, acc, L1, L2, lsum, zeros, cap);
 }
 
-template <int K, bool GEN>
+template <int K, bool GEN, bool MEMO = false>
 __device__ __forceinline__ void paired_regs_body(const PairedArgs& a, int lb, int slot_lo, int slot_hi, int block_lo, int block_hi,
                                                  double& lsum, int& zeros, unsigned long long* tl = nullptr, int4* wave_lds = nullptr) {
   bool first_pair = true;
@@ -987,7 +1044,7 @@
     for (int k = 0; k < K; k++) { r1[k] = a.inl[0][at + k]; r2[k] = a.inl[1][at + k]; }
     if (tl && first_pair) { asm volatile("s_waitcnt vmcnt(0)" ::: "memory"); if ((threadIdx.x & 63) == 0) tl[2] = (unsigned long long)wall_clock64() + (r1[0].x == 0x12345 ? 1 : 0); }
     RegCands<K> x, y;
-    const bool m1 = cands_from_records<K>(a.m[0], r1, x), m2 = cands_from_records<K>(a.m[1], r2, y);
+    const bool m1 = cands_from_records<K, MEMO>(a.m[0], r1, x, 0), m2 = cands_from_records<K, MEMO>(a.m[1], r2, y, 1);
     if (tl && first_pair) { asm volatile("s_waitcnt vmcnt(0)" ::: "memory"); if ((threadIdx.x & 63) == 0) tl[3] = (unsigned long long)wall_clock64() + (x.pos[0] == 0x12345 ? 1 : 0); }
     const bool dirty = r1[0].x == kDirtyWid;
     const bool general = !dirty && (m1 || m2);
@@ -1013,7 +1070,7 @@
   }
 }
 
-template <bool GEN>
+template <bool GEN, bool MEMO = false>
 __device__ __forceinline__ void paired_delta_body(const PairedArgs& a, int db, int delta_blocks, double& lsum, int& zeros, int4* wave_lds = nullptr) {
   for (int dj = db * kBlock + threadIdx.x; dj < a.dstate[kDsDirty]; dj += delta_blocks * kBlock) {
     const int i = a.dirty_slots[dj];
@@ -1028,7 +1085,7 @@
       if (sp < 0) {
         RegCands<2> x, y;
         const int4 q0[2] = {r0[0], r0[1]}, q1[2] = {r1[0], r1[1]};
-        const bool m0 = cands_from_records<2>(a.m[0], q0, x), m1 = cands_from_records<2>(a.m[1], q1, y);
+        const bool m0 = cands_from_records<2, MEMO>(a.m[0], q0, x, 0), m1 = cands_from_records<2, MEMO>(a.m[1], q1, y, 1);
         general = m0 || m1;
         if (!general) score_cands_and_finish<2>(a, i, l12, x, y, lsum, zeros);
       }
@@ -1036,7 +1093,7 @@
 #pragma unroll
       for (int k = 2; k < 4; k++) { r0[k] = a.dirty_recs[0][4 * (size_t)dj + k]; r1[k] = a.dirty_recs[1][4 * (size_t)dj + k]; }
       RegCands<4> x, y;
-      const bool m0 = cands_from_records<4>(a.m[0], r0, x), m1 = cands_from_records<4>(a.m[1], r1, y);
+      const bool m0 = cands_from_records<4, MEMO>(a.m[0], r0, x, 0), m1 = cands_from_records<4, MEMO>(a.m[1], r1, y, 1);
       general = m0 || m1;
       if (!general) score_cands_and_finish<4>(a, i, l12, x, y, lsum, zeros);
     }
@@ -1077,7 +1134,7 @@
   }
 }
 
-template <bool TICKET, bool GEN, bool TL>
+template <bool TICKET, bool GEN, bool TL, bool MEMO = false>
 __device__ __forceinline__ void paired_main_body(const PairedArgs& a, int lb, double* sh_s, int* sh_z, int4* gen_lds) {
   double lsum = 0.0;
   int zeros = 0;
@@ -1091,8 +1148,10 @@
     const SlotRange rg = compact_range(c, lb);
     const bool stat = wide && lb < c.blocks0a;
     if (!TL && wide && c.n_codes == 1) {
-      if (stat) paired_static4_body<GEN, false, true>(c, rg, lsum, zeros);
-      else paired_compact4_body<GEN, false, true>(c, rg, lsum, zeros);
+      if (stat) paired_static4_body<GEN, false, true, MEMO>(c, rg, lsum, zeros);
+      else paired_compact4_body<GEN, false, true, MEMO>(c, rg, lsum, zeros);
+    } else if (MEMO) {
+      paired_compact_body<GEN, MEMO>(c, rg, lsum, zeros);
     } else {
       __shared__ uint32_t sh_combo[256];
       __shared__ double sh_floor[256], sh_logfloor[256], sh_tfloor[256];
@@ -1109,13 +1168,13 @@
     int4* const wave_lds = GEN ? gen_lds + (threadIdx.x >> 6) * 2 * kOvfCap : nullptr;
     if (lb < a.blocks01) {
       GAML_FRESH_ARGS(c, a)
-      paired_regs_body<2, GEN>(c, lb, c.n0, c.n01, c.blocks0, c.blocks01, lsum, zeros, tl, wave_lds);
+      paired_regs_body<2, GEN, MEMO>(c, lb, c.n0, c.n01, c.blocks0, c.blocks01, lsum, zeros, tl, wave_lds);
     } else if (lb < a.blocks012) {
       GAML_FRESH_ARGS(c, a)
-      paired_regs_body<4, GEN>(c, lb, c.n01, c.n_main, c.blocks01, c.blocks012, lsum, zeros, nullptr, wave_lds);
+      paired_regs_body<4, GEN, MEMO>(c, lb, c.n01, c.n_main, c.blocks01, c.blocks012, lsum, zeros, nullptr, wave_lds);
     } else {
       GAML_FRESH_ARGS(c, a)
-      paired_delta_body<GEN>(c, lb - c.blocks012, c.main_blocks - c.blocks012, lsum, zeros, wave_lds);
+      paired_delta_body<GEN, MEMO>(c, lb - c.blocks012, c.main_blocks - c.blocks012, lsum, zeros, wave_lds);
     }
   }
   block_reduce(lsum, zeros, sh_s, sh_z);
@@ -1146,8 +1205,8 @@
 
 constexpr int kOvfMaxBlocks = 1024;
 
-template <class Src>
-__device__ __forceinline__ int wave_gather(const MateView& v, const Src& src, int4* lds, int lane) {
+template <bool MEMO = false, class Src>
+__device__ __forceinline__ int wave_gather(const MateView& v, const Src& src, int4* lds, int lane, int mt = 0) {
   const int cnt = src.count();
   int total = 0;
   for (int base = 0; base < cnt; base += 64) {
@@ -1156,7 +1215,12 @@
     int4 r = make_int4(-1, 0, 0, 0), o = make_int4(0, 0, -1, 0);
     if (k < cnt) {
       r = src.get(k);
-      if (r.x >= 0) { const Occ12 e = v.occ12[r.x]; o = occ_from_compact((unsigned long long)e.lo | ((unsigned long long)e.hi << 32), e.rank); }
+      if (r.x >= 0) {
+        bool both = false;
+        const Occ12 e = occ_entry_of<MEMO>(v, mt, (unsigned)r.x, both);
+        if (MEMO && both) occ_flag_shared();
+        o = occ_from_compact((unsigned long long)e.lo | ((unsigned long long)e.hi << 32), e.rank);
+      }
       if (o.z >= 0) mine = o.w >= 0 ? 1 : v.multi_off[-o.w] - v.multi_off[-o.w - 1];
     }
     int incl = mine;
@@ -1178,13 +1242,13 @@
   return total;
 }
 
-template <class Src>
+template <bool MEMO = false, class Src>
 __device__ __forceinline__ double wave_score_pair(const PairedArgs& a, const Src& s1, const Src& s2, int L1, int L2, int4* c1, int4* c2, int lane) {
-  const int n1 = wave_gather(a.m[0], s1, c1, lane);
-  const int n2 = wave_gather(a.m[1], s2, c2, lane);
+  const int n1 = wave_gather<MEMO>(a.m[0], s1, c1, lane, 0);
+  const int n2 = wave_gather<MEMO>(a.m[1], s2, c2, lane, 1);
   double acc = 0.0;
   if (n1 < 0 || n2 < 0) {
-    if (lane == 0) acc = paired_general_src(a, s1, s2, L1, L2);
+    if (lane == 0) acc = paired_general_src<MEMO>(a, s1, s2, L1, L2);
     return acc;
   }
   __builtin_amdgcn_wave_barrier();
@@ -1219,7 +1283,7 @@
   return acc;
 }
 
-template <bool TICKET>
+template <bool TICKET, bool MEMO = false>
 __device__ __forceinline__ void paired_overflow_body(const PairedArgs& a, int ovf_block, int ovf_blocks, double* sh_s, int* sh_z,
                                                      int4 (*cand)[2][kOvfCap]) {
   const int lane = threadIdx.x & 63, wave = threadIdx.x >> 6;
@@ -1238,7 +1302,7 @@
       const uint32_t l12 = a.len12[i - a.n0];
       if (r1.x == kDirtyWid) continue;
       const int L1 = l12 & 0xffff, L2 = l12 >> 16;
-      const double acc = wave_score_pair(a, TableSrc{&a.m[0], r1}, TableSrc{&a.m[1], r2}, L1, L2, c1, c2, lane);
+      const double acc = wave_score_pair<MEMO>(a, TableSrc{&a.m[0], r1}, TableSrc{&a.m[1], r2}, L1, L2, c1, c2, lane);
       if (lane == 0) finish_read(a, i, acc, L1, L2, lsum, zeros);
     } else {
       const int sp = item - n_table;
@@ -1246,7 +1310,7 @@
       const uint32_t l12 = i < a.n0 ? a.len_combo[a.len_code[i]] : a.len12[i - a.n0];
       const int L1 = l12 & 0xffff, L2 = l12 >> 16;
       const int2 g0 = a.spill_rng[0][sp], g1 = a.spill_rng[1][sp];
-      const double acc = wave_score_pair(a, ListSrc{a.spill_recs[0] + g0.x, g0.y}, ListSrc{a.spill_recs[1] + g1.x, g1.y}, L1, L2, c1, c2, lane);
+      const double acc = wave_score_pair<MEMO>(a, ListSrc{a.spill_recs[0] + g0.x, g0.y}, ListSrc{a.spill_recs[1] + g1.x, g1.y}, L1, L2, c1, c2, lane);
       if (lane == 0) finish_read(a, i, acc, L1, L2, lsum, zeros);
     }
   }
@@ -1263,7 +1327,7 @@
 #ifndef GAML_GEN_WAVES
 #define GAML_GEN_WAVES 4
 #endif
-template <bool TICKET, bool GEN = false, bool TL = false>
+template <bool TICKET, bool GEN = false, bool TL = false, bool MEMO = false>
 __global__ __launch_bounds__(kBlock, GEN ? GAML_GEN_WAVES : 5) void paired_score_kernel(PairedArgs a) {
   __shared__ double sh_s[kBlock / 64];
   __shared__ int sh_z[kBlock / 64];
@@ -1274,21 +1338,21 @@
     double lsum = 0.0;
     int zeros = 0;
     if (!GAML_TIMING_X(16))
-    paired_static4_body<GEN, false, true>(a, SlotRange{0, a.n0a, lb, a.blocks0a}, lsum, zeros);
+    paired_static4_body<GEN, false, true, MEMO>(a, SlotRange{0, a.n0a, lb, a.blocks0a}, lsum, zeros);
     block_reduce(lsum, zeros, sh_s, sh_z);
     if (TICKET) grid_finish(lsum, zeros, lb, a.total_blocks, a.part_sum, a.part_zero, a.ticket, a.out, 0.0, a.n_reads, sh_s, sh_z, a.status_out, a.status_a, a.status_b);
     else if (threadIdx.x == 0) { a.part_sum[lb] = lsum; a.part_zero[lb] = zeros; }
     return;
   }
-  if (lb < a.main_blocks) paired_main_body<TICKET, GEN, TL>(a, lb, sh_s, sh_z, &cand[0][0][0]);
+  if (lb < a.main_blocks) paired_main_body<TICKET, GEN, TL, MEMO>(a, lb, sh_s, sh_z, &cand[0][0][0]);
   else if (GAML_GEN_OFF(16)) { if (threadIdx.x == 0) { a.part_sum[lb] = 0.0; a.part_zero[lb] = 0; } }
   else {
     GAML_FRESH_ARGS(c, a)
-    paired_overflow_body<TICKET>(c, lb - c.main_blocks, c.total_blocks - c.main_blocks, sh_s, sh_z, cand);
+    paired_overflow_body<TICKET, MEMO>(c, lb - c.main_blocks, c.total_blocks - c.main_blocks, sh_s, sh_z, cand);
   }
 #else
-  if (lb < a.main_blocks) paired_main_body<TICKET, GEN, TL>(a, lb, sh_s, sh_z, &cand[0][0][0]);
-  else paired_overflow_body<TICKET>(a, lb - a.main_blocks, a.total_blocks - a.main_blocks, sh_s, sh_z, cand);
+  if (lb < a.main_blocks) paired_main_body<TICKET, GEN, TL, MEMO>(a, lb, sh_s, sh_z, &cand[0][0][0]);
+  else paired_overflow_body<TICKET, MEMO>(a, lb - a.main_blocks, a.total_blocks - a.main_blocks, sh_s, sh_z, cand);
 #endif
 }
 
diff --git a/gaml_amd/csrc/occ_device.hip.h b/gaml_amd/csrc/occ_device.hip.h
--- a/gaml_amd/csrc/occ_device.hip.h
+++ b/gaml_amd/csrc/occ_device.hip.h
@@ -47,7 +47,7 @@
 
 bool occdev_route_ok(const gaml_hip_ctx* c, PairedSet& s) {
   PairedSet::OccDev& D = s.occdev;
-  if (!c->occ_route || KNOB(c, 17) != 0 || !paired_resident_route(c, s) || !s.persist.valid) return false;
+  if (!c->occ_route || KNOB(c, 17) == 1 || !paired_resident_route(c, s) || !s.persist.valid) return false;
   if (s.planner.last_was_incremental()) return false;
   const std::vector<int32_t>& ids = s.planner.ids();
   if (ids.empty() || ids.size() > (size_t)kOccMaxDesc) return false;
@@ -129,7 +129,7 @@
   return 0;
 }
 
-int occdev_launch(gaml_hip_ctx* c, PairedSet& s, hipStream_t st, size_t* bytes) {
+int occdev_pool_init(gaml_hip_ctx* c, PairedSet& s) {
   PairedSet::OccDev& D = s.occdev;
   const std::vector<int32_t>& ids = s.planner.ids();
   if (D.pool_cap[0] == 0 || D.pool_cap[1] == 0) {
@@ -142,6 +142,106 @@
     }
     D.pool_gen++;
   }
+  return 0;
+}
+
+constexpr int kMemoMaxPaths = 2;
+constexpr size_t kDenseBudget = (size_t)64 << 20;
+
+bool occmemo_route_ok(const gaml_hip_ctx* c, PairedSet& s) {
+  const PairedSet::OccDev& D = s.occdev;
+  const bool thrashing = D.dense_restarts >= 8 && D.dense_restarts * 16 > D.memo_calls;
+  return KNOB(c, 17) == 0 && KNOB(c, 3) == 0 && s.planner.ids().size() <= (size_t)kMemoMaxPaths && !thrashing;
+}
+
+struct OccDenseJob { const OccPre* src; Occ12* dst; int n_pre, n_win, start; };
+struct OccDenseArgs { int n_jobs, total; OccDenseJob job[2 * kMemoMaxPaths]; };
+
+__global__ void __launch_bounds__(kBlock) occ_dense_kernel(const OccDenseArgs a) {
+  for (int i = blockIdx.x * blockDim.x + threadIdx.x; i < a.total; i += gridDim.x * blockDim.x) {
+    int j = 0;
+    while (j + 1 < a.n_jobs && a.job[j + 1].start <= i) j++;
+    const OccDenseJob& J = a.job[j];
+    const OccPre e = J.src[i - J.start];
+    if ((unsigned)e.wid >= (unsigned)J.n_win) continue;
+    Occ12* o = J.dst + e.wid;
+    o->lo = e.lo; o->hi = e.hi; o->rank = e.rank;
+  }
+}
+
+int occmemo_prepare(gaml_hip_ctx* c, PairedSet& s, hipStream_t st, size_t* bytes) {
+  PairedSet::OccDev& D = s.occdev;
+  const std::vector<int32_t>& ids = s.planner.ids();
+  if (int e = occdev_pool_init(c, s)) return e;
+  if (int e = occdev_upload(c, s, st, bytes)) return e;
+  auto missing = [&](const PathMemo& pm, int mt) { return pm.dense_off[mt] < 0 || pm.dense_gen[mt] != D.dense_gen; };
+  size_t n_win[2], need[2] = {0, 0}, whole[2];
+  for (int mt = 0; mt < 2; mt++) {
+    n_win[mt] = s.mate[mt].wins.size();
+    whole[mt] = ids.size() * (n_win[mt] + 1);
+    for (size_t k = 0; k < ids.size(); k++)
+      if (missing(s.planner.memo(ids[k]), mt) && !(k == 1 && ids[1] == ids[0])) need[mt] += n_win[mt] + 1;
+  }
+  if (D.dense_used[0] + need[0] > D.dense_cap[0] || D.dense_used[1] + need[1] > D.dense_cap[1]) {
+    HIP_TRY(c, hipStreamSynchronize(st));
+    const size_t budget = (KNOB(c, 23) > 0 ? (size_t)KNOB(c, 23) << 10 : kDenseBudget) / sizeof(Occ12);
+    for (int mt = 0; mt < 2; mt++) {
+      const size_t want = std::max(2 * whole[mt], std::min(budget, 32 * whole[mt]));
+      if (D.dense_cap[mt] < 2 * whole[mt] || D.dense_cap[mt] == 0) {
+        D.dense_cap[mt] = std::max(want, D.dense_cap[mt]);
+        HIP_TRY(c, D.dense[mt].reserve(D.dense_cap[mt] * sizeof(Occ12)));
+      }
+      D.dense_used[mt] = 0;
+      need[mt] = (ids.size() == 2 && ids[1] == ids[0] ? 1 : ids.size()) * (n_win[mt] + 1);
+    }
+    D.dense_gen++;
+    D.dense_restarts++;
+  }
+  if (need[0] + need[1] > 0) {
+    OccDenseArgs a;
+    memset(&a, 0, sizeof(a));
+    for (int mt = 0; mt < 2; mt++) {
+      if (!need[mt]) continue;
+      HIP_TRY(c, hipMemsetAsync(D.dense[mt].as<Occ12>() + D.dense_used[mt], 0xff, need[mt] * sizeof(Occ12), st));
+      for (int32_t id : ids) {
+        PathMemo& pm = s.planner.memo(id);
+        if (!missing(pm, mt)) continue;
+        pm.dense_off[mt] = (int64_t)D.dense_used[mt];
+        pm.dense_gen[mt] = D.dense_gen;
+        pm.dense_n[mt] = (int32_t)n_win[mt];
+        D.dense_used[mt] += n_win[mt] + 1;
+        a.job[a.n_jobs++] = OccDenseJob{D.pool[mt].as<OccPre>() + pm.dev_off[mt], D.dense[mt].as<Occ12>() + pm.dense_off[mt], (int)pm.pre[mt].size(), (int)n_win[mt], a.total};
+        a.total += (int)pm.pre[mt].size();
+      }
+    }
+    *bytes += (need[0] + need[1]) * sizeof(Occ12);
+    if (a.total > 0) {
+      hipLaunchKernelGGL(occ_dense_kernel, dim3((unsigned)std::min(256, (a.total + kBlock - 1) / kBlock)), dim3(kBlock), 0, st, a);
+      HIP_TRY(c, hipGetLastError());
+    }
+  }
+  for (int mt = 0; mt < 2; mt++) {
+    const PathMemo& A = s.planner.memo(ids[0]);
+    D.memo_tab[mt][0] = D.dense[mt].as<Occ12>() + A.dense_off[mt];
+    D.memo_n[mt][0] = (uint32_t)A.dense_n[mt];
+    if (ids.size() == 2) {
+      const PathMemo& B = s.planner.memo(ids[1]);
+      D.memo_tab[mt][1] = D.dense[mt].as<Occ12>() + B.dense_off[mt];
+      D.memo_n[mt][1] = (uint32_t)B.dense_n[mt];
+    } else {
+      D.memo_tab[mt][1] = D.memo_tab[mt][0] + A.dense_n[mt];
+      D.memo_n[mt][1] = 0;
+    }
+  }
+  HIP_TRY(c, D.dup.reserve(sizeof(int)));
+  *(volatile int*)D.dup.p = 0;
+  return 0;
+}
+
+int occdev_launch(gaml_hip_ctx* c, PairedSet& s, hipStream_t st, size_t* bytes) {
+  PairedSet::OccDev& D = s.occdev;
+  const std::vector<int32_t>& ids = s.planner.ids();
+  if (int e = occdev_pool_init(c, s)) return e;
   size_t n_occ[2] = {0, 0};
   for (int32_t id : ids) for (int mt = 0; mt < 2; mt++) n_occ[mt] += s.planner.memo(id).pre[mt].size();
   const size_t n_windows = std::max(s.mate[0].wins.size(), s.mate[1].wins.size());
@@ -185,7 +285,7 @@
   return 0;
 }
 
-const Occ12* occdev_table(const PairedSet& s, int mt) { return s.occdev.tab[mt][s.occdev.serial & 1].as<Occ12>(); }
+const Occ12* occdev_table(const PairedSet& s, int mt) { return s.occdev.memo ? s.occdev.memo_tab[mt][0] : s.occdev.tab[mt][s.occdev.serial & 1].as<Occ12>(); }
 
 void paired_images_refresh(PairedSet& s) {
   if (!s.occdev.image_stale) return;
diff --git a/gaml_amd/csrc/paired_launch.hip.h b/gaml_amd/csrc/paired_launch.hip.h
--- a/gaml_amd/csrc/paired_launch.hip.h
+++ b/gaml_amd/csrc/paired_launch.hip.h
@@ -68,8 +68,10 @@
   s.planner.finish(s.mate);
   PairedSet::OccDev& D = s.occdev;
   D.taken = device_route && occdev_route_ok(c, s);
+  D.memo = D.taken && occmemo_route_ok(c, s);
   size_t up_bytes = 0;
-  if (D.taken) { if (int e = occdev_launch(c, s, st, &up_bytes)) return e; }
+  if (D.memo) { if (int e = occmemo_prepare(c, s, st, &up_bytes)) return e; }
+  else if (D.taken) { if (int e = occdev_launch(c, s, st, &up_bytes)) return e; }
   c->prof[6] = (double)up_bytes;
   const double q1 = now_us();
   const bool cov = s.cfg.penalty_constant > 0;
@@ -93,6 +95,7 @@
   s.planner.apply(s.mate, s.image, !D.taken, D.image_stale);
   D.image_stale = D.taken;
   if (D.taken) D.dev_calls++; else D.host_calls++;
+  if (D.memo) D.memo_calls++;
   p.assembled_records = s.planner.assembled(0) + s.planner.assembled(1);
   p.general = !D.taken && (!s.image[0].general_wids.empty() || !s.image[1].general_wids.empty());
   if (trace) fprintf(stderr, "pass2: finish %.1f us, starts %.1f us, images %.1f us\n", q1 - q0, q2 - q1, now_us() - q2);
@@ -453,6 +456,11 @@
   s.last_host_partials = c->host_results;
   s.last_sets = 1;
   paired_apply_set(a, sd);
+  const bool memo_set = s.occdev.taken && s.occdev.memo;
+  if (memo_set) {
+    for (int mt = 0; mt < 2; mt++) a.om[mt] = OccMemo{s.occdev.memo_tab[mt][1], s.occdev.memo_n[mt][0], s.occdev.memo_n[mt][1]};
+    a.occ_dup = (int*)s.occdev.dup.dev;
+  }
   a.out = out4;
   a.timeline = nullptr;
   const bool timeline = KNOB(c, 3) == 8;
@@ -478,7 +486,10 @@
     if (timeline) GAML_LAUNCH_SCORE(false, false, true);
     else
 #endif
-    if (gen_set) { if (fin_mode) GAML_LAUNCH_SCORE(false, true); else GAML_LAUNCH_SCORE(true, true); }
+    if (memo_set) {
+      if (gen_set || !fin_mode || timeline) return fail(c, GAML_HIP_ESTATE, "memo route taken by a call it does not serve");
+      GAML_LAUNCH_SCORE(false, false, false, true);
+    } else if (gen_set) { if (fin_mode) GAML_LAUNCH_SCORE(false, true); else GAML_LAUNCH_SCORE(true, true); }
     else if (fin_mode) GAML_LAUNCH_SCORE(false, false);
     else GAML_LAUNCH_SCORE(true, false);
 #undef GAML_LAUNCH_SCORE
diff --git a/include/gaml_hip_debug.h b/include/gaml_hip_debug.h
--- a/include/gaml_hip_debug.h
+++ b/include/gaml_hip_debug.h
@@ -28,6 +28,7 @@
 int32_t gaml_hip_debug_block_partials(gaml_hip_ctx* ctx, int readset, int32_t set, double* sums, int32_t* zeros, int32_t cap, int32_t* layout8);
 
 int gaml_hip_debug_occ_route(gaml_hip_ctx* ctx, int readset, int64_t* out6);
+int gaml_hip_debug_occ_memo(gaml_hip_ctx* ctx, int readset, int64_t* out4);
 int gaml_hip_debug_occ_check(gaml_hip_ctx* ctx, int readset, int64_t* out4);
 
 #ifdef __cplusplus
```
